# A-Kokolis/Hermes

Measured on AMD Instinct MI355X. Metric: replicated KVS ops/s (reads+writes committed), higher is better.
Workload: dtype u8

## Files before the change

### hermes_amd/csrc/hkv_batch.hip

```cpp
#include <hip/hip_runtime.h>

#include <algorithm>
#include <cstdio>
#include <cstdlib>
#include <cstring>

#include "hkv_exec.h"
#include "hkv_internal.h"

namespace hkv {

constexpr uint32_t kNone = 0xFFFFFFFFu;
enum : uint8_t { kStDone = 0, kStCommit = 1, kStPend = 2 };
enum { kCtrFbM = 1, kCtrFbL = 2 };

struct BatchArgs {
    uint8_t *elems;
    const int32_t *counts;
    const int32_t *offsets;
    const uint8_t *index;
    uint8_t *log;
    uint8_t *rw;
    int32_t *ns_idx;
    unsigned long long *fw;
// ... 14 lines not shown
    int32_t stride;
    int32_t esz;
    int32_t type;
    uint32_t rtag0;
    uint8_t ltag;
    int32_t rounds;
    int32_t inv_direct;
    int32_t ack_direct;
    uint8_t g_membership;
    uint8_t w_ack_init;
    int32_t *node_suspected;
    int32_t n_batches;
    const uint8_t *host_src;
    uint8_t *host_dst;
    uint8_t *dev_region;
    uint64_t region_bytes;
    uint32_t *done_flag;
    uint32_t done_value;
    unsigned long long *prof;
    const SmallBatch *hdr;
    uint8_t *state_out;
    const uint8_t *opc;
    const uint8_t *patch;
    uint16_t *fk;
    uint64_t *hx;
    uint8_t *rws;
    const uint8_t *rwo;
    int32_t n_rows, skip_row;
    int64_t row_stride;
    int32_t dbg;
    int32_t check_unique;
    uint8_t *ack_out;
    uint32_t ack_out_size;
};

__host__ __device__ constexpr int rounds_for(int type, bool rmw)
{
    return type == kVals || (type == kLocal && !rmw) ? 0 : 2;
}

template <int TYPE>
__device__ __forceinline__ uint8_t absorbing_state()
{
    return TYPE == kVals ? kValid : kWrite;
}

template <int TYPE>
__device__ __forceinline__ Meta after_first(const BatchArgs &a, const Meta &m0, uint32_t f, int f_is_put)
{
    Meta m1 = m0;
    m_set_state(m1, absorbing_state<TYPE>());
    if (TYPE != kLocal || a.g.skew == 0) return m1;
    uint8_t foc = f_is_put ? (uint8_t)kOpPut : a.elems[(int64_t)f * a.esz + 8];
    if (a.hx && !f_is_put) {
        const uint64_t pb = *reinterpret_cast<const uint64_t *>(a.patch + (int64_t)f * 16 + 8);
        if ((pb >> 48) & 0xFFu) foc = (uint8_t)pb;
    }
    if (foc != kOpGet) {
        m1.ver += 2;
        m_set_cid(m1, (uint8_t)a.g.machine_id);
    } else {
        m_set_state(m1, kReplay);
    }
    return m1;
}

// ... 31 lines not shown
    }
    int lo = 0, hi = a.n_batches - 1;
    while (lo < hi) {
        const int mid = (lo + hi + 1) >> 1;
        if (a.offsets[mid] <= i) lo = mid; else hi = mid - 1;
    }
    start = a.offsets[lo];
    return lo;
}

__device__ __forceinline__ void elem_at(const BatchArgs &a, uint32_t i, uint8_t *&x, uint8_t &idx, Ctx &c)
{
    c.rw = nullptr;
    c.rws = nullptr;
    idx = 0;
    if (a.rw || !a.offsets) {
        int64_t start;
        const int32_t b = batch_of(a, i, start);
        idx = (uint8_t)(i - start);
        c.rw = a.rw ? a.rw + (int64_t)b * a.rw_stride : nullptr;
        c.rws = a.rws ? a.rws + (int64_t)b * (a.rw_stride / a.g.op_size) : nullptr;
        c.rwo = a.rwo ? a.rwo + (int64_t)b * (a.rw_stride / a.g.op_size) : nullptr;
    }
    x = a.elems + (int64_t)i * a.esz;
}

__device__ __forceinline__ void note_state(const BatchArgs &a, int64_t i, const uint8_t *x)
{
    if (a.state_out) a.state_out[i] = x[9];
}

__device__ __forceinline__ uint64_t phys_of(const BatchArgs &a, uint32_t e) { return (uint64_t)e * a.g.entry_unit; }
__device__ __forceinline__ uint8_t *entry_of(const BatchArgs &a, uint32_t e) { return a.log + phys_of(a, e); }
__device__ __forceinline__ uint32_t fw_index(const BatchArgs &a, uint64_t phys)
{
    return (uint32_t)(((phys >> 6) * 0x9E3779B1ull) & a.fw_mask);
}
__device__ __forceinline__ unsigned long long *fw_of(const BatchArgs &a, uint32_t e) { return a.fw + fw_index(a, phys_of(a, e)); }

__device__ __forceinline__ uint32_t first_cand(unsigned long long f, uint32_t rtag)
{
    return (uint32_t)(f >> 32) == ~rtag ? (uint32_t)f : kNone;
}

__device__ __forceinline__ void offer(unsigned long long *f, uint32_t rtag, uint32_t i)
{
    const unsigned long long v = ((unsigned long long)(~rtag) << 32) | i;
    if (v < __hip_atomic_load(f, __ATOMIC_RELAXED, __HIP_MEMORY_SCOPE_AGENT)) atomicMin(f, v);
}

__device__ __forceinline__ uint32_t agg_ticket(uint32_t *arr, uint32_t j, bool active)
{
    const int lane = threadIdx.x & 63;
    uint32_t ticket = 0;
    unsigned long long left = __ballot(active);
    while (left) {
        const int leader = __ffsll((long long)left) - 1;
        const uint32_t jl = __shfl(j, leader, 64);
        const unsigned long long m = left & __ballot(active && j == jl);
        uint32_t base = 0;
        if (lane == leader) base = atomicAdd(&arr[jl], (uint32_t)__popcll(m));
        base = __shfl(base, leader, 64);
        if ((m >> lane) & 1ull) ticket = base + (uint32_t)__popcll(m & ((1ull << lane) - 1ull));
        left &= ~m;
    }
    return ticket;
// ... 104 lines not shown
    if (oc == kOpPut) k = kFkWrite;
    else if (oc == kOpGet) k = kFkReplay;
    else if (oc == kOpRmw && st != kInProgressRmw) k = m_state(m0) == kValid ? kFkWrite : kFkReplay;
    return (uint16_t)(k | (oc == kOpRmw ? 4u : 0u) | (((h >> 16) & 0xFFu) << 8));
}
__device__ __forceinline__ Meta after_first_rmw(const BatchArgs &a, const Meta &m0, uint16_t fk, uint8_t idx)
{
    Meta m = m0;
    if ((fk & 3u) == kFkWrite) {
        const uint8_t rmw_flag = (fk >> 2) & 1u;
        m_set_val_len(m, (uint8_t)(((uint8_t)(fk >> 8) >> a.g.shift) + kOpMetaSize));
        m_set_rmw(m, rmw_flag);
        m_set_state(m, kWrite);
        m_set_obi(m, idx);
        const uint32_t step = (!a.g.rmw_enabled || rmw_flag == 1) ? 2u : 4u;
        const uint8_t node = (uint8_t)a.g.machine_id;
        m.llw_ver = m.ver + step;
        m.llw_cid = node;
        m_set_ack_bv(m, a.w_ack_init);
        m.ver += step;
        m_set_cid(m, node);
    } else {
        m_set_state(m, kReplay);
        m_set_obi(m, idx);
        m.llw_ver = m.ver;
        m.llw_cid = m_cid(m);
        m_set_ack_bv(m, a.w_ack_init);
    }
    return m;
}

constexpr int64_t kLookupHead = 8192;
constexpr int kLookupPair = 2;
template <int P = kLookupPair>
__device__ __forceinline__ void lookup_pair(const BatchArgs &a, const uint64_t *key, const bool *probe, int q,
                                            int gbase, bool *ok, uint64_t *phys, uint4 *ln)
{
    uint4 v[P];
#pragma unroll
    for (int k = 0; k < P; ++k)
        v[k] = probe[k] ? reinterpret_cast<const uint4 *>(a.index + ((key[k] & 0xFFFFFFFFFFFFULL) & a.g.bkt_mask) * 64u)[q]
                        : make_uint4(0u, 0u, 0u, 0u);
#pragma unroll
    for (int k = 0; k < P; ++k) {
        const uint64_t s0 = (uint64_t)v[k].x | ((uint64_t)v[k].y << 32);
        const uint64_t s1 = (uint64_t)v[k].z | ((uint64_t)v[k].w << 32);
        const uint32_t tag = (uint32_t)(key[k] >> 48);
        const bool mt0 = probe[k] && (s0 & 1u) && ((uint32_t)(s0 >> 1) & 0x7FFFFFu) == tag;
        const bool mt1 = probe[k] && (s1 & 1u) && ((uint32_t)(s1 >> 1) & 0x7FFFFFu) == tag;
        const uint32_t g0 = (uint32_t)(__ballot(mt0) >> gbase) & 0xFu;
        const uint32_t g1 = (uint32_t)(__ballot(mt1) >> gbase) & 0xFu;
        uint32_t o = 0;
#pragma unroll
        for (int l = 0; l < 4; ++l) o |= ((g0 >> l) & 1u) << (2 * l) | ((g1 >> l) & 1u) << (2 * l + 1);
        const int first = o ? __ffs(o) - 1 : 0;
        const uint64_t off = __shfl((first & 1) ? (s1 >> 24) : (s0 >> 24), first >> 1, 4);
        ok[k] = probe[k] && o && a.g.log_head - off < a.g.log_cap;
        phys[k] = off & a.g.log_mask;
    }
#pragma unroll
    for (int k = 0; k < P; ++k)
        ln[k] = ok[k] ? reinterpret_cast<const uint4 *>(a.log + phys[k])[q] : make_uint4(0u, 0u, 0u, 0u);
}

template <int P>
__device__ __forceinline__ void lookup_pair_f(const BatchArgs &a, const uint64_t *key, const bool *probe, int q,
                                              int gbase, bool *ok, uint64_t *phys, uint4 *ln, unsigned long long *fwv)
{
    uint4 v[P];
#pragma unroll
    for (int k = 0; k < P; ++k)
        v[k] = probe[k] ? reinterpret_cast<const uint4 *>(a.index + ((key[k] & 0xFFFFFFFFFFFFULL) & a.g.bkt_mask) * 64u)[q]
                        : make_uint4(0u, 0u, 0u, 0u);
#pragma unroll
    for (int k = 0; k < P; ++k) {
        const uint64_t s0 = (uint64_t)v[k].x | ((uint64_t)v[k].y << 32);
        const uint64_t s1 = (uint64_t)v[k].z | ((uint64_t)v[k].w << 32);
        const uint32_t tag = (uint32_t)(key[k] >> 48);
        const bool mt0 = probe[k] && (s0 & 1u) && ((uint32_t)(s0 >> 1) & 0x7FFFFFu) == tag;
        const bool mt1 = probe[k] && (s1 & 1u) && ((uint32_t)(s1 >> 1) & 0x7FFFFFu) == tag;
        const uint32_t g0 = (uint32_t)(__ballot(mt0) >> gbase) & 0xFu;
        const uint32_t g1 = (uint32_t)(__ballot(mt1) >> gbase) & 0xFu;
        uint32_t o = 0;
#pragma unroll
        for (int l = 0; l < 4; ++l) o |= ((g0 >> l) & 1u) << (2 * l) | ((g1 >> l) & 1u) << (2 * l + 1);
        const int first = o ? __ffs(o) - 1 : 0;
        const uint64_t off = __shfl((first & 1) ? (s1 >> 24) : (s0 >> 24), first >> 1, 4);
        ok[k] = probe[k] && o && a.g.log_head - off < a.g.log_cap;
        phys[k] = off & a.g.log_mask;
    }
#pragma unroll
    for (int k = 0; k < P; ++k) {
        ln[k] = ok[k] ? reinterpret_cast<const uint4 *>(a.log + phys[k])[q] : make_uint4(0u, 0u, 0u, 0u);
        fwv[k] = ok[k] && q == 0 ? a.fw[fw_index(a, phys[k])] : ~0ull;
    }
}


template <int P = kLookupPair>
__global__ __launch_bounds__(256) void k_lookup(BatchArgs a, int64_t i_begin, int64_t i_end)
{
    const int q = threadIdx.x & 3;
    const int lane = threadIdx.x & 63;
    const int gbase = lane & ~3;
    if (i_begin == 0 && blockIdx.x == 0 && threadIdx.x == 0) {
        a.ctr[kCtrFbM] = 0;
        a.ctr[kCtrFbL] = 0;
    }
    const bool vals_direct = a.type == kVals;
    int64_t gi[P];
    uint64_t key[P], hdr[P], tail[P];
    int probe[P];
    bool patched[P];
#pragma unroll
    for (int k = 0; k < P; ++k) {
        gi[k] = i_begin + ((int64_t)blockIdx.x * P + k) * 64 + (threadIdx.x >> 2);
        uint64_t kk = 0, hh = 0;
        int p = 0;
        patched[k] = false;
        tail[k] = 0;
        if (gi[k] < i_end && q == 0) {
            const int32_t b = (int32_t)(gi[k] / a.stride);
            const int32_t idx = (int32_t)(gi[k] - (int64_t)b * a.stride);
            const bool counted = a.counts == nullptr || idx < a.counts[b];
            if (a.hx) {
                const uint8_t *x = a.elems + gi[k] * a.esz;
                const U64x2 h = *reinterpret_cast<const U64x2 *>(x);
                const U64x2 pt = *reinterpret_cast<const U64x2 *>(a.patch + gi[k] * 16);
                tail[k] = *reinterpret_cast<const uint64_t *>(x + a.esz - 8);
                patched[k] = patch_valid(pt.b);
                kk = patched[k] ? pt.a : h.a;
                hh = patched[k] ? patched_hdr(h.b, pt.b) : h.b;
            }
            if (counted) {
                if (!a.hx) {
                    const U64x2 h = *reinterpret_cast<const U64x2 *>(a.elems + gi[k] * a.esz);
                    kk = h.a;
                    hh = h.b;
                }
                if (skip_elem_os(a.type, (uint8_t)hh, (uint8_t)(hh >> 8))) {
                    if (a.type == kInvs && a.ns_idx) {
                        int64_t start;
                        const int32_t bb = a.offsets ? batch_of(a, gi[k], start) : b;
                        atomicMax(&a.ns_idx[bb], a.offsets ? (int32_t)(gi[k] - start) : idx);
                    }
                } else {
                    p = 1;
                }
            }
        }
        key[k] = kk;
        hdr[k] = hh;
        probe[k] = p;
    }
#pragma unroll
    for (int k = 0; k < P; ++k) {
        const int p = __shfl(probe[k], 0, 4);
        const uint64_t kk = __shfl(key[k], 0, 4);
        probe[k] = p;
        key[k] = kk;
    }
    bool ok[P];
    uint64_t phys[P], ekey[P];
    Meta m0[P];
    U64x2 ln[P];
    {
        bool pr[P];
        uint4 l4[P];
#pragma unroll
        for (int k = 0; k < P; ++k) pr[k] = probe[k] != 0;
        lookup_pair<P>(a, key, pr, q, gbase, ok, phys, l4);
#pragma unroll
        for (int k = 0; k < P; ++k)
            ln[k] = U64x2{(uint64_t)l4[k].x | ((uint64_t)l4[k].y << 32), (uint64_t)l4[k].z | ((uint64_t)l4[k].w << 32)};
    }
#pragma unroll
    for (int k = 0; k < P; ++k) {
        ekey[k] = __shfl(ln[k].b, 0, 4);
        const uint64_t w45 = __shfl(ln[k].a, 1, 4), w67 = __shfl(ln[k].b, 1, 4);
        const uint32_t b32 = (uint32_t)__shfl(ln[k].a, 2, 4) & 0xFFu;
        m0[k].w4 = (uint32_t)w45;
        m0[k].w5 = (uint32_t)(w45 >> 32);
        m0[k].ver = (uint32_t)w67;
        m0[k].llw_cid = (uint8_t)(w67 >> 32);
        m0[k].llw_ver = (uint32_t)(w67 >> 40) | (b32 << 24);
    }
    if (q != 0) return;
#pragma unroll
    for (int k = 0; k < P; ++k) {
        if (gi[k] >= i_end) continue;
        uint8_t *x = a.elems + gi[k] * a.esz;
        uint32_t e = kNone;
        uint8_t ifl = 0;
        if (ok[k] && ekey[k] == key[k]) {
            e = (uint32_t)(phys[k] / a.g.entry_unit);
            uint8_t *entry = a.log + phys[k];
            if (vals_direct) {
                const uint64_t its = pack_ts((uint32_t)(hdr[k] >> 32), (uint8_t)(hdr[k] >> 24));
                if (its == pack_ts(m0[k].ver, m_cid(m0[k])) && m_state(m0[k]) != kValid) entry[kEntryMetaOff] = kValid;
                x[8] = kValSuccess;
            } else if (a.ack_direct) {
                const uint64_t ats = pack_ts((uint32_t)(hdr[k] >> 32), (uint8_t)(hdr[k] >> 24));
                if (ats != pack_ts(m0[k].llw_ver, m0[k].llw_cid) || m_obi(m0[k]) == kObiEmpty) {
                    x[8] = ack_opcode((uint8_t)hdr[k]);
                } else {
                    ifl = kAkMatch;
                    const uint32_t w = fw_index(a, phys[k]);
                    const uint8_t snd = (uint8_t)(hdr[k] >> 8);
                    if (snd >= 8 || (uint8_t)(a.g_membership & ~m_ack_bv(m0[k])) == 0)
                        offer(a.fw + w, a.rtag0, (uint32_t)gi[k]);
                    if (snd < 8) {
                        unsigned long long *t = a.ft + (size_t)w * 8 + snd;
                        const unsigned long long tv = ((unsigned long long)(a.rtag0 >> 3) << 32) | (0xFFFFFFFFu - (uint32_t)gi[k]);
                        if (tv > __hip_atomic_load(t, __ATOMIC_RELAXED, __HIP_MEMORY_SCOPE_AGENT)) atomicMax(t, tv);
                    }
                    a.pf[gi[k]] = (uint32_t)m_ack_bv(m0[k]) | ((uint32_t)m_state(m0[k]) << 8) | ((uint32_t)m_obi(m0[k]) << 16);
                }
            } else if (a.inv_direct) {
                const uint64_t its = pack_ts((uint32_t)(hdr[k] >> 32), (uint8_t)(hdr[k] >> 24));
                const uint64_t cur = pack_ts(m0[k].ver, m_cid(m0[k]));
                if (its < cur) {
                    x[8] = inv_opcode((uint8_t)hdr[k], false);
                } else if (its == cur) {
                    ifl = kIvEq | (m_state(m0[k]) == kWrite ? kIvWrite : 0);
                } else {
                    ifl = kIvRaise;
                    a.pf[gi[k]] = 0;
                    const uint32_t w = fw_index(a, phys[k]);
                    const unsigned long long xv = (its << 24) | (0x7FFFFFull - (uint64_t)gi[k]);
// ... 801 lines not shown
            slot = sl;
            return true;
        }
        sl = (sl + 1) & (kPreHash - 1);
    }
    return false;
}

__device__ __forceinline__ void pre_insert_key(uint64_t *hk, uint64_t key)
{
    if (key == ~0ull) return;
    uint32_t sl = pre_slot(key);
    for (int n = 0; n < kPreHash; ++n) {
        const unsigned long long old = atomicCAS((unsigned long long *)&hk[sl], ~0ull, key);
        if (old == ~0ull || old == key) return;
        sl = (sl + 1) & (kPreHash - 1);
    }
}

#ifndef HKV_PRE_PAIR
#define HKV_PRE_PAIR 4
#endif
constexpr int kPrePair = HKV_PRE_PAIR;
#ifdef HKV_PRE_WAVES
#define HKV_PRE_ATTR __attribute__((amdgpu_waves_per_eu(HKV_PRE_WAVES)))
#else
#define HKV_PRE_ATTR
#endif
#ifdef HKV_PRE_NUM_SGPR
#define HKV_PRE_SGPR_ATTR __attribute__((amdgpu_num_sgpr(HKV_PRE_NUM_SGPR)))
#else
#define HKV_PRE_SGPR_ATTR
#endif
template <int HEAD = kPreHead>
__global__ __launch_bounds__(kPreThreads) HKV_PRE_ATTR HKV_PRE_SGPR_ATTR void k_local_pre(BatchArgs a)
{
    __shared__ uint64_t hk[kPreHash], gk[kPreHash];
    __shared__ uint32_t hv[kPreHash];
    __shared__ uint32_t dl[kPreElems];
    __shared__ uint32_t nd;
    const int tid = threadIdx.x, q = tid & 3, gbase = (tid & 63) & ~3;
    if (tid == 0) {
        nd = 0;
        if (blockIdx.x == 0) a.ctr[kCtrDefer] = 0;
    }
    for (int j = tid; j < kPreHash; j += kPreThreads) {
        hk[j] = ~0ull;
        gk[j] = ~0ull;
        hv[j] = kNone;
    }
    if (HKV_DBG_ON(a, 8)) return;
    const int64_t i0 = (int64_t)blockIdx.x * kPreElems;
    const int64_t head_end = HKV_DBG_ON(a, 4) ? 0 : i0 < HEAD ? i0 : HEAD;
    constexpr int kOwnK = kPreElems / kPreThreads, kAllK = kOwnK + (HEAD + kPreThreads - 1) / kPreThreads;
    U64x2 h[kAllK];
    bool in[kAllK];
    uint8_t opm[kAllK];
    U64x2 pt[kAllK];
#pragma unroll
    for (int k = 0; k < kAllK; ++k) {
        const bool own = k < kOwnK;
        const int64_t i = own ? i0 + k * kPreThreads + tid : (int64_t)(k - kOwnK) * kPreThreads + tid;
        in[k] = i < a.n && (own || i < head_end);
        opm[k] = a.opc ? a.opc[in[k] ? i : 0] : (uint8_t)kOpPut;
    }
    if (a.patch) {
#pragma unroll
// ... 54 lines not shown
            pre_insert_key(gk, key);
        }
    }
    __syncthreads();
    const Ctx c = make_ctx(a);
    const uint64_t hput[2] = {0, (uint64_t)kOpPut};
    const uint32_t cnt = HKV_DBG_ON(a, 2) ? 0 : nd;
    for (uint32_t base = 0; base < cnt; base += (kPreThreads / 4) * kPrePair) {
        uint64_t key[kPrePair];
        bool probe[kPrePair], ok[kPrePair];
        uint32_t idx[kPrePair];
        uint64_t phys[kPrePair];
        uint4 ln[kPrePair];
#pragma unroll
        for (int k = 0; k < kPrePair; ++k) {
            const uint32_t j = base + k * (kPreThreads / 4) + (tid >> 2);
            probe[k] = j < cnt;
            const uint32_t d = probe[k] ? dl[j] : 0u;
            idx[k] = !probe[k] ? kNone : d < (uint32_t)kPreHash ? hv[d] : ~d;
            key[k] = !probe[k] ? 0 : d < (uint32_t)kPreHash ? hk[d] : elem_key(a, (int64_t)idx[k]);
            if (probe[k] && head_end > 0 && key[k] != ~0ull) {
                uint32_t sl = pre_slot(key[k]);
                for (int n = 0; n < kPreHash; ++n) {
                    const uint64_t g = gk[sl];
                    if (g == ~0ull) break;
                    if (g == key[k]) {
                        probe[k] = false;
                        break;
                    }
                    sl = (sl + 1) & (kPreHash - 1);
                }
            }
        }
        lookup_pair<kPrePair>(a, key, probe, q, gbase, ok, phys, ln);
#pragma unroll
        for (int k = 0; k < kPrePair; ++k) {
            Meta m0;
            const uint64_t ek = line_key_meta(ln[k], m0);
            if (q != 0 || !ok[k] || ek != key[k]) continue;
            if (!would_mutate(kLocal, reinterpret_cast<const uint8_t *>(hput), m0, c) || HKV_DBG_ON(a, 1)) continue;
            atomicMin(a.fw + fw_index(a, phys[k]), ((unsigned long long)(~a.rtag0) << 32) | idx[k]);
        }
    }
}

__device__ __forceinline__ void local_resolve_nm(const BatchArgs &a, uint8_t *x, const uint8_t *ent, const Meta &m)
{
    const uint8_t oc = x[8], st = m_state(m);
    const bool obi_empty = m_obi(m) == kObiEmpty;
    bool mut = false;
    if (oc == kOpGet) {
        if (st == kValid) {
            copy_value<31>(x + kOpValueOff, ent + kEntryValueOff, 31);
            x[9] = kGetComplete;
            x[10] = (uint8_t)((m_val_len(m) >> a.g.shift) - kOpMetaSize);
        } else if (st == kInvalidWrite || st == kWrite || st == kReplay) {
            x[9] = kGetStall;
        } else {
            x[9] = kEmpty;
            if (st == kInvalid) {
                const uint8_t lw = m_lwid(m);
                if (lw < 8 && ((a.g_membership >> lw) & 1u)) x[9] = kGetStall;
                else mut = obi_empty;
            }
        }
        if (a.g.skew & kSkewReadComplete) hot_read_complete(x, m.ver, m_cid(m));
    } else if (oc == kOpPut) {
        mut = (st == kValid || st == kInvalid) && obi_empty;
        x[9] = kPutStall;
        if (a.g.skew & kSkewWriteCoalesce) {
            const uint32_t cv = m.ver & 0xFFFFu;
            uint32_t over = ld32(x + 12);
            if (st != kReplay && over == 0) {
                st32(x + 12, cv);
                over = cv;
            }
            if (over > 0 && over + 1u < cv) x[9] = kPutComplete;
        }
    }
    if (mut && a.error_flags) atomicOr(a.error_flags, 1u);
}

#ifndef HKV_LOCAL_NUM_SGPR
#define HKV_LOCAL_NUM_SGPR 80
#endif
#if HKV_LOCAL_NUM_SGPR > 0
#define HKV_LOCAL_SGPR_ATTR __attribute__((amdgpu_num_sgpr(HKV_LOCAL_NUM_SGPR)))
#else
#define HKV_LOCAL_SGPR_ATTR
#endif
#ifndef HKV_LF_WAVES
#define HKV_LF_WAVES 2
#endif
constexpr int kLfWaves = HKV_LF_WAVES;
template <int P, int NW>
__global__ __launch_bounds__(64 * NW) HKV_LOCAL_SGPR_ATTR void k_local_fused(BatchArgs a)
{
    constexpr int E = 16 * P;
    constexpr int EB = E * NW;
    __shared__ uint4 sops_b[NW][E * 4];
    __shared__ uint4 sln_b[NW][E * 4];
    __shared__ unsigned long long sfw_b[NW][E];
    __shared__ uint32_t sent_b[NW][E];
    __shared__ uint8_t sprb_b[NW][E];
    __shared__ uint32_t sst[EB / 4], sstate[EB / 4];
    __shared__ uint32_t sdef[EB];
    __shared__ uint32_t ndef;
    const int w = threadIdx.x >> 6, tid = threadIdx.x & 63, q = tid & 3, gbase = tid & ~3;
    uint4 *sops = sops_b[w], *sln = sln_b[w];
    unsigned long long *sfw = sfw_b[w];
    uint32_t *sent = sent_b[w];
    uint8_t *sprb = sprb_b[w];
    const int64_t ib = (int64_t)blockIdx.x * EB, i0 = ib + (int64_t)w * E;
    if (threadIdx.x == 0) ndef = 0;
    uint64_t key[P];
    bool probe[P], ok[P], live[P];
    uint64_t phys[P];
    uint4 ln[P], op[P];
    int te[P];
#pragma unroll
    for (int k = 0; k < P; ++k) {
        te[k] = k * 16 + (tid >> 2);
        const int64_t i = i0 + te[k];
        live[k] = i < a.n;
        op[k] = make_uint4(0u, 0u, 0u, 0u);
        if (live[k]) {
            const uint8_t *xg = a.elems + i * 56 + 16 * q;
            U64x2 p{0, 0};
            if (a.patch) p = *reinterpret_cast<const U64x2 *>(a.patch + i * 16);
            if (q < 3) {
                op[k] = *reinterpret_cast<const uint4 *>(xg);
            } else {
                const uint64_t t = *reinterpret_cast<const uint64_t *>(xg);
                op[k].x = (uint32_t)t;
                op[k].y = (uint32_t)(t >> 32);
            }
            if (patch_valid(p.b)) op[k] = patch_chunk(op[k], q, p.a, p.b);
        }
        sops[te[k] * 4 + q] = op[k];
    }
#pragma unroll
    for (int k = 0; k < P; ++k) {
        key[k] = (uint64_t)(uint32_t)__shfl((int)op[k].x, 0, 4) | ((uint64_t)(uint32_t)__shfl((int)op[k].y, 0, 4) << 32);
        const uint32_t h0 = (uint32_t)__shfl((int)op[k].z, 0, 4);
        probe[k] = false;
        if (live[k] && !HKV_DBG_ON(a, 128))
            probe[k] = in_count(a, (uint32_t)(i0 + te[k])) && !skip_elem_os(kLocal, (uint8_t)h0, (uint8_t)(h0 >> 8));
    }
    unsigned long long fwv[P];
    if (HKV_DBG_ON(a, 512)) {
        lookup_pair<P>(a, key, probe, q, gbase, ok, phys, ln);
#pragma unroll
        for (int k = 0; k < P; ++k) fwv[k] = ~0ull;
    } else {
        lookup_pair_f<P>(a, key, probe, q, gbase, ok, phys, ln, fwv);
    }
#pragma unroll
    for (int k = 0; k < P; ++k) {
        Meta m;
        const uint64_t ek = line_key_meta(ln[k], m);
        const bool hit = ok[k] && ek == key[k];
        const unsigned long long f = hit && m_state(m) != kInvalid && q == 0 ? fwv[k] : ~0ull;
        if (hit) sln[te[k] * 4 + q] = ln[k];
        if (q == 0) {
            sfw[te[k]] = f;
            sent[te[k]] = hit ? (uint32_t)(phys[k] / a.g.entry_unit) : kNone;
            sprb[te[k]] = probe[k];
        }
    }
    __syncthreads();
    if (tid < E && i0 + tid < a.n && !HKV_DBG_ON(a, 64)) {
        const int64_t i = i0 + tid;
        uint8_t *x = reinterpret_cast<uint8_t *>(&sops[tid * 4]);
        uint8_t *ent = reinterpret_cast<uint8_t *>(&sln[tid * 4]);
        const uint32_t e = sent[tid];
        uint8_t st = kStDone;
        if (e != kNone) {
            Ctx c = make_ctx(a);
            Meta m;
            meta_load(ent, m);
            const bool wm = would_mutate(kLocal, x, m, c);
            if (m_state(m) == kInvalid) {
                if (wm) {
                    const uint64_t ph = phys_of(a, e);
                    offer(a.fw + fw_index(a, ph), a.rtag0, (uint32_t)i);
                    if ((uint8_t)(m.w5 >> 16) != a.ltag) a.log[ph + kEntryMetaOff + 4] = a.ltag;
                }
                st = kStDefer;
                sdef[atomicAdd(&ndef, 1u)] = (uint32_t)i;
            } else {
                const uint32_t f = first_cand(sfw[tid], a.rtag0);
                if (wm && (f == kNone || f > (uint32_t)i) && a.error_flags) atomicOr(a.error_flags, 4u);
                if ((uint32_t)i == f) {
                    apply_to_shadow<kLocal, 31>(a, x, (uint32_t)i, ent);
                    st = kStCommit;
                } else {
                    local_resolve_nm(a, x, ent, f != kNone && (uint32_t)i > f ? after_first<kLocal>(a, m, f, 1) : m);
                }
            }
        } else if (sprb[tid]) {
            x[9] = kMiss;
        }
        if (a.opc && sprb[tid] && x[8] == kOpPut && a.opc[i] != kOpPut && a.error_flags) atomicOr(a.error_flags, 8u);
        if (!HKV_DBG_ON(a, 1024)) a.ent[i] = e;
        reinterpret_cast<uint8_t *>(sst)[w * E + tid] = st;
        reinterpret_cast<uint8_t *>(sstate)[w * E + tid] = x[9];
    }
    __syncthreads();
    if (!HKV_DBG_ON(a, 1024) && !HKV_DBG_ON(a, 64)) {
        if (ib + EB <= a.n && ((uintptr_t)a.state_out & 3) == 0) {
            if ((int)threadIdx.x < EB / 4) {
                reinterpret_cast<uint32_t *>(a.st + ib)[threadIdx.x] = sst[threadIdx.x];
                if (a.state_out) reinterpret_cast<uint32_t *>(a.state_out + ib)[threadIdx.x] = sstate[threadIdx.x];
            }
        } else if ((int)threadIdx.x < EB && ib + threadIdx.x < a.n) {
            a.st[ib + threadIdx.x] = reinterpret_cast<const uint8_t *>(sst)[threadIdx.x];
            if (a.state_out) a.state_out[ib + threadIdx.x] = reinterpret_cast<const uint8_t *>(sstate)[threadIdx.x];
        }
    }
// ... 70 lines not shown
        if (a.check_unique) {
            const unsigned long long v = ((unsigned long long)(~a.rtag0) << 32) | (uint32_t)gi[k];
            const unsigned long long old = atomicExch(a.fw + fw_index(a, phys[k]), v);
            if ((uint32_t)(old >> 32) == ~a.rtag0 && a.error_flags) atomicOr(a.error_flags, 16u);
        }
        uint8_t *entry = a.log + phys[k];
        Ctx c = make_ctx(a);
        uint8_t idx = 0;
        if (TYPE == kAcks) {
            uint8_t *xx;
            elem_at(a, (uint32_t)gi[k], xx, idx, c);
        }
        Meta t = m[k];
        dispatch<SV>(TYPE, x, entry, idx, t, c);
        if (!meta_equal(t, m[k])) meta_store(entry, t);
    }
}

__device__ __forceinline__ uint4 load_chunk(const uint8_t *x, int q, int32_t esz)
{
    if (16 * q + 16 <= esz) return *reinterpret_cast<const uint4 *>(x + 16 * q);
    if (16 * q + 8 <= esz) {
        const uint64_t t = *reinterpret_cast<const uint64_t *>(x + 16 * q);
        return make_uint4((uint32_t)t, (uint32_t)(t >> 32), 0u, 0u);
    }
    return make_uint4(0u, 0u, 0u, 0u);
}

__device__ __forceinline__ bool chunk_equal(const uint4 &a, const uint4 &b)
{
    return a.x == b.x && a.y == b.y && a.z == b.z && a.w == b.w;
}

template <int TYPE, int P = kLookupPair>
__global__ __launch_bounds__(64) void k_unique_lds(BatchArgs a)
{
    constexpr int E = 16 * P;
    __shared__ uint4 sops[E * 4];
    __shared__ uint4 sln[E * 4];
    __shared__ uint32_t sent[E];
    __shared__ uint8_t sprb[E];
    const int tid = threadIdx.x, q = tid & 3, gbase = tid & ~3;
    const int64_t i0 = (int64_t)blockIdx.x * E;
    const int64_t n_live = a.offsets ? (int64_t)a.offsets[a.n_batches] : a.n;
    uint64_t key[P];
    bool probe[P], ok[P], live[P];
    uint64_t phys[P];
    uint4 ln[P], op[P];
    int te[P];
#pragma unroll
    for (int k = 0; k < P; ++k) {
        te[k] = k * 16 + (tid >> 2);
        const int64_t i = i0 + te[k];
        live[k] = i < a.n && i < n_live;
        op[k] = live[k] ? load_chunk(a.elems + i * a.esz, q, a.esz) : make_uint4(0u, 0u, 0u, 0u);
        sops[te[k] * 4 + q] = op[k];
    }
#pragma unroll
    for (int k = 0; k < P; ++k) {
        key[k] = (uint64_t)(uint32_t)__shfl((int)op[k].x, 0, 4) | ((uint64_t)(uint32_t)__shfl((int)op[k].y, 0, 4) << 32);
        const uint32_t h0 = (uint32_t)__shfl((int)op[k].z, 0, 4);
        probe[k] = false;
        const int64_t i = i0 + te[k];
        if (live[k] && (a.offsets || in_count(a, (uint32_t)i))) {
            if (!skip_elem_os(TYPE, (uint8_t)h0, (uint8_t)(h0 >> 8))) {
                probe[k] = true;
            } else if (TYPE == kInvs && a.ns_idx && q == 0) {
                int64_t start;
                const int32_t b = batch_of(a, i, start);
                atomicMax(&a.ns_idx[b], (int32_t)(i - start));
            }
        }
    }
    lookup_pair<P>(a, key, probe, q, gbase, ok, phys, ln);
#pragma unroll
    for (int k = 0; k < P; ++k) {
        Meta m;
        const uint64_t ek = line_key_meta(ln[k], m);
        const bool hit = ok[k] && ek == key[k];
        sln[te[k] * 4 + q] = ln[k];
        if (q == 0) {
            sent[te[k]] = hit ? (uint32_t)(phys[k] / a.g.entry_unit) : kNone;
            sprb[te[k]] = probe[k];
        }
    }
    __syncthreads();
    if (tid < E && i0 + tid < n_live) {
        const int64_t i = i0 + tid;
        uint8_t *x = reinterpret_cast<uint8_t *>(&sops[tid * 4]);
        uint8_t *ent = reinterpret_cast<uint8_t *>(&sln[tid * 4]);
        const uint32_t e = sent[tid];
        if (e != kNone) {
            if (a.check_unique) {
                const unsigned long long v = ((unsigned long long)(~a.rtag0) << 32) | (uint32_t)i;
                const unsigned long long old = atomicExch(a.fw + fw_index(a, phys_of(a, e)), v);
                if ((uint32_t)(old >> 32) == ~a.rtag0 && a.error_flags) atomicOr(a.error_flags, 16u);
            }
            Ctx c = make_ctx(a);
            int done = -1;
            if (TYPE == kAcks) c.rw_done = &done;
            Meta m;
            meta_load(ent, m);
            Meta t = m;
            dispatch<31>(TYPE, x, ent, 0, t, c);
            if (!meta_equal(t, m)) meta_store(ent, t);
            if (TYPE == kAcks && done >= 0 && a.rw) {
                uint8_t *xx;
// ... 7 lines not shown
    }
    __syncthreads();
#pragma unroll
    for (int k = 0; k < P; ++k) {
        if (!live[k]) continue;
        uint4 w = sops[te[k] * 4 + q];
        if (TYPE == kInvs && a.ack_out) {
            uint8_t *y = a.ack_out + (i0 + te[k]) * a.ack_out_size;
            const uint32_t hz = sops[te[k] * 4].z;
            const uint8_t oc = (uint8_t)hz;
            const bool full = oc == kOpInvAbort && a.ack_out_size >= (uint32_t)a.esz;
            if (oc == kInvSuccess || full) {
                uint4 c = w;
                if (q == 0)
                    c.z = (hz & ~0xFFFFu) | (oc == kInvSuccess ? kOpAck : kOpInvAbort) |
                          ((uint32_t)(uint8_t)a.g.machine_id << 8);
                if (q == 0 || (full && 16 * q < a.esz)) {
                    if (16 * q + 16 <= a.esz || q == 0) *reinterpret_cast<uint4 *>(y + 16 * q) = c;
                    else *reinterpret_cast<uint64_t *>(y + 16 * q) = (uint64_t)c.x | ((uint64_t)c.y << 32);
                }
            } else if (q == 0) {
                y[8] = kEmpty;
            }
            if (q == 0 && (oc == kInvSuccess || oc == kOpInvAbort || oc == kOpMembChange))
                w.z = (w.z & ~0xFFu) | kEmpty;
        }
        if (!chunk_equal(w, op[k])) {
            uint8_t *xg = a.elems + (i0 + te[k]) * a.esz + 16 * q;
            if (16 * q + 16 <= a.esz) *reinterpret_cast<uint4 *>(xg) = w;
            else *reinterpret_cast<uint64_t *>(xg) = (uint64_t)w.x | ((uint64_t)w.y << 32);
        }
        if (ok[k] && q > 0) {
            const uint4 l = sln[te[k] * 4 + q];
            if (!chunk_equal(l, ln[k])) reinterpret_cast<uint4 *>(a.log + phys[k])[q] = l;
        }
    }
}

#ifdef HKV_ROWS_NUM_SGPR
#define HKV_ROWS_SGPR_ATTR __attribute__((amdgpu_num_sgpr(HKV_ROWS_NUM_SGPR)))
#else
#define HKV_ROWS_SGPR_ATTR
#endif
template <int TYPE, int RMAX, int CH, int P = kLookupPair>
#ifdef HKV_ROWS_WAVES
#define HKV_ROWS_WAVES_ATTR __attribute__((amdgpu_waves_per_eu(HKV_ROWS_WAVES, 8)))
#else
#define HKV_ROWS_WAVES_ATTR
#endif
__global__ __launch_bounds__(64) HKV_ROWS_SGPR_ATTR HKV_ROWS_WAVES_ATTR void k_unique_rows(BatchArgs a)
{
    constexpr int E = 16 * P;
    __shared__ uint4 sops[RMAX][E * CH];
    __shared__ uint4 sln[E * 4];
    __shared__ uint32_t sent[E];
    __shared__ uint8_t spart[E];
    const int tid = threadIdx.x, q = tid & 3, gbase = tid & ~3;
    const int64_t i0 = (int64_t)blockIdx.x * E;
    const int R = a.n_rows < RMAX ? a.n_rows : RMAX;
    const int64_t n_live = a.offsets ? (int64_t)a.offsets[a.n_batches] : a.n;
    uint64_t key[P];
    bool probe[P], ok[P], live[P];
    uint64_t phys[P];
    uint4 ln[P], op[RMAX][P];
    uint32_t part[P];
    int te[P];
#pragma unroll
    for (int k = 0; k < P; ++k) {
        te[k] = k * 16 + (tid >> 2);
        const int64_t i = i0 + te[k];
        live[k] = i < a.n && i < n_live && (a.offsets || in_count(a, (uint32_t)i));
#pragma unroll
        for (int r = 0; r < RMAX; ++r) {
            const bool on = live[k] && r < R && r != a.skip_row;
            op[r][k] = on && q < CH ? load_chunk(a.elems + (r * a.row_stride + i) * a.esz, q, a.esz)
                                    : make_uint4(0u, 0u, 0u, 0u);
            if (q < CH) sops[r][te[k] * CH + q] = op[r][k];
        }
    }
#pragma unroll
    for (int k = 0; k < P; ++k) {
        uint64_t kk = 0;
        uint32_t p = 0;
        bool mismatch = false;
#pragma unroll
        for (int r = 0; r < RMAX; ++r) {
            const uint64_t kr = (uint64_t)(uint32_t)__shfl((int)op[r][k].x, 0, 4) |
                                ((uint64_t)(uint32_t)__shfl((int)op[r][k].y, 0, 4) << 32);
            const uint32_t h0 = (uint32_t)__shfl((int)op[r][k].z, 0, 4);
            if (!live[k] || r >= R || r == a.skip_row || (uint8_t)h0 == 0) continue;
            if (skip_elem_os(TYPE, (uint8_t)h0, (uint8_t)(h0 >> 8))) continue;
            if (p && kr != kk) mismatch = true;
            if (!p) kk = kr;
            p |= 1u << r;
        }
        if (mismatch && q == 0 && a.error_flags) atomicOr(a.error_flags, 16u);
        key[k] = kk;
        part[k] = mismatch ? 0u : p;
        probe[k] = part[k] != 0;
    }
    lookup_pair<P>(a, key, probe, q, gbase, ok, phys, ln);
#pragma unroll
    for (int k = 0; k < P; ++k) {
        Meta m;
        const uint64_t ek = line_key_meta(ln[k], m);
        const bool hit = ok[k] && ek == key[k];
        sln[te[k] * 4 + q] = ln[k];
        if (q == 0) {
            sent[te[k]] = hit ? (uint32_t)(phys[k] / a.g.entry_unit) : kNone;
            spart[te[k]] = (uint8_t)part[k];
        }
    }
    __syncthreads();
    if (tid < E && i0 + tid < n_live) {
        const int64_t i = i0 + tid;
        uint8_t *ent = reinterpret_cast<uint8_t *>(&sln[tid * 4]);
        const uint32_t e = sent[tid];
        const uint32_t p = spart[tid];
        if (e != kNone && p) {
            if (a.check_unique) {
                const unsigned long long v = ((unsigned long long)(~a.rtag0) << 32) | (uint32_t)i;
                const unsigned long long old = atomicExch(a.fw + fw_index(a, phys_of(a, e)), v);
                if ((uint32_t)(old >> 32) == ~a.rtag0 && a.error_flags) atomicOr(a.error_flags, 16u);
            }
            Ctx c = make_ctx(a);
            int done = -1;
            if (TYPE == kAcks) c.rw_done = &done;
            Meta m;
            meta_load(ent, m);
            Meta t = m;
#pragma unroll
            for (int r = 0; r < RMAX; ++r)
                if ((p >> r) & 1u) dispatch<31>(TYPE, reinterpret_cast<uint8_t *>(&sops[r][tid * CH]), ent, 0, t, c);
            if (!meta_equal(t, m)) meta_store(ent, t);
// ... 3 lines not shown
                elem_at(a, (uint32_t)i, xx, idx, c);
                complete_rw_slot(c, done);
            }
        } else {
#pragma unroll
            for (int r = 0; r < RMAX; ++r)
                if ((p >> r) & 1u) reinterpret_cast<uint8_t *>(&sops[r][tid * CH])[9] = kMiss;
        }
    }
    __syncthreads();
#pragma unroll
    for (int k = 0; k < P; ++k) {
        if (!live[k]) continue;
#pragma unroll
        for (int r = 0; r < RMAX; ++r) {
            if (r >= R || r == a.skip_row || q >= CH) continue;
            uint4 w = sops[r][te[k] * CH + q];
            if (TYPE == kAcks && CH == 1 && a.ack_out) {
                const uint8_t oc = (uint8_t)w.z;
                uint4 v = make_uint4(0u, 0u, (uint32_t)kEmpty, 0u);
                if (oc != 0 && oc != kAckSuccess && oc != kOpMembChange && oc != kEmpty)
                    v = make_uint4(w.x, w.y, (w.z & ~0xFFFFu) | (uint32_t)kOpVal | ((uint32_t)(uint8_t)a.g.machine_id << 8), w.w);
                *reinterpret_cast<uint4 *>(a.ack_out + (r * a.row_stride + i0 + te[k]) * 16) = v;
                if (oc != 0 && oc != kEmpty) w.z = (w.z & ~0xFFu) | (uint32_t)kEmpty;
            }
            if (!chunk_equal(w, op[r][k])) {
                uint8_t *xg = a.elems + (r * a.row_stride + i0 + te[k]) * a.esz + 16 * q;
                if (16 * q + 16 <= a.esz) *reinterpret_cast<uint4 *>(xg) = w;
                else *reinterpret_cast<uint64_t *>(xg) = (uint64_t)w.x | ((uint64_t)w.y << 32);
            }
        }
        if (ok[k] && q > 0) {
            const uint4 l = sln[te[k] * 4 + q];
            if (!chunk_equal(l, ln[k])) reinterpret_cast<uint4 *>(a.log + phys[k])[q] = l;
        }
    }
}

constexpr int kUbElems = 16;
constexpr int kUbChunks = 20;
template <int TYPE>
__global__ __launch_bounds__(64) void k_unique_big(BatchArgs a)
{
    __shared__ uint4 sx[kUbElems * kUbChunks];
    __shared__ uint4 se[kUbElems * kUbChunks];
    constexpr int kPerLane = (kUbChunks + 3) / 4;
    uint4 x0[kPerLane], e0[kPerLane];
    const int tid = threadIdx.x, q = tid & 3, el = tid >> 2, gbase = tid & ~3;
    const int64_t i = (int64_t)blockIdx.x * kUbElems + el;
    const bool live = i < a.n;
    const int nch = (a.esz + 15) / 16;
    uint8_t *xg = a.elems + i * a.esz;
#pragma unroll
    for (int u = 0; u < kPerLane; ++u) {
        const int c = q + 4 * u;
        const uint4 v = live && c < nch ? load_chunk(xg, c, a.esz) : make_uint4(0u, 0u, 0u, 0u);
        if (c < nch) sx[el * kUbChunks + c] = v;
        x0[u] = v;
    }
    const uint4 c0 = sx[el * kUbChunks];
    const uint64_t key = (uint64_t)c0.x | ((uint64_t)c0.y << 32);
    bool probe = false;
    if (live && (a.offsets || in_count(a, (uint32_t)i))) {
        if (!skip_elem_os(TYPE, (uint8_t)c0.z, (uint8_t)(c0.z >> 8))) {
            probe = true;
        } else if (TYPE == kInvs && a.ns_idx && q == 0) {
            int64_t start;
// ... 63 lines not shown
                        w.z = (hz & ~0xFFFFu) | (oc == kInvSuccess ? kOpAck : kOpInvAbort) |
                              ((uint32_t)(uint8_t)a.g.machine_id << 8);
                    if (16 * c + 16 <= a.esz || c == 0) *reinterpret_cast<uint4 *>(y + 16 * c) = w;
                    else *reinterpret_cast<uint64_t *>(y + 16 * c) = (uint64_t)w.x | ((uint64_t)w.y << 32);
                }
            } else if (q == 0) {
                y[8] = kEmpty;
            }
        }
#pragma unroll
        for (int u = 0; u < kPerLane; ++u) {
            const int c = q + 4 * u;
            if (c >= nch) continue;
            uint4 w = sx[el * kUbChunks + c];
            if (TYPE == kInvs && a.ack_out && c == 0 && (oc == kInvSuccess || oc == kOpInvAbort || oc == kOpMembChange))
                w.z = (w.z & ~0xFFu) | kEmpty;
            if (chunk_equal(w, x0[u])) continue;
            if (16 * c + 16 <= a.esz) *reinterpret_cast<uint4 *>(xg + 16 * c) = w;
            else *reinterpret_cast<uint64_t *>(xg + 16 * c) = (uint64_t)w.x | ((uint64_t)w.y << 32);
        }
    }
    if (hit) {
        uint4 *eg = reinterpret_cast<uint4 *>(a.log + phys);
#pragma unroll
        for (int u = 0; u < kPerLane; ++u) {
            const int c = q + 4 * u;
            if (c >= kUbChunks) continue;
            const uint4 w = se[el * kUbChunks + c];
            if (c > 0 && !chunk_equal(w, e0[u])) eg[c] = w;
        }
    }
}

__global__ __launch_bounds__(256) void k_local_deferred(BatchArgs a)
{
    const uint32_t nd = a.ctr[kCtrDefer];
    for (uint32_t j = blockIdx.x * 256u + threadIdx.x; j < nd; j += gridDim.x * 256u) {
        const uint32_t i = a.fbl[j];
        const uint32_t e = a.ent[i];
        uint8_t *xg;
        uint8_t idx;
        Ctx c = make_ctx(a);
        elem_at(a, i, xg, idx, c);
        Meta m;
        meta_load(entry_of(a, e), m);
        const uint32_t f = first_cand(*fw_of(a, e), a.rtag0);
        uint8_t st = kStDone;
        if (f == kNone || i < f) {
            Meta tm = m;
            dispatch<31>(kLocal, xg, entry_of(a, e), idx, tm, c);
            if (a.error_flags && !meta_equal(tm, m)) atomicOr(a.error_flags, 1u);
        } else if (i == f) {
            apply_to_shadow<kLocal, 31>(a, nullptr, i, entry_of(a, e));
            st = kStCommit;
        } else {
            const Meta m1 = after_first<kLocal>(a, m, f, 0);
            Meta tm = m1;
            dispatch<31>(kLocal, xg, entry_of(a, e), idx, tm, c);
            if (a.error_flags && !meta_equal(tm, m1)) atomicOr(a.error_flags, 1u);
        }
        a.st[i] = st;
        note_state(a, i, xg);
    }
}

template <int TYPE, int SV>
__global__ __launch_bounds__(256) void k_resolve(BatchArgs a, int r)
{
    extern __shared__ uint64_t sx[];
    const bool kStage = SV == 31 && a.esz <= 16;
    const int64_t i = (int64_t)blockIdx.x * 256 + threadIdx.x;
    bool left = false;
    VCopy vc{nullptr, nullptr};
    VCopy *vcp = SV != 31 && a.g.st_value <= 320 ? &vc : nullptr;
    const bool wave_shadow = SV != 31 && vcp;
    bool cand = false;
    uint32_t prev = 0;
    if (i < a.n && a.st[i] == kStPend) {
        const uint32_t e = a.ent[i];
        const uint32_t f = first_cand(*fw_of(a, e), a.rtag0 + (uint32_t)r);
        prev = a.pf[i];
        if (f == kNone || (uint32_t)i <= f) {
            uint8_t *xg = a.elems + i * a.esz;
            uint8_t *xl = reinterpret_cast<uint8_t *>(sx) + threadIdx.x * (uint32_t)a.esz;
            if (kStage) copy_elem(xl, xg, a.esz);
            if ((uint32_t)i != f) {
                if (kStage) resolve_elem<TYPE, SV>(a, (uint32_t)i, xl, shadow_of(a, prev));
                else resolve_elem<TYPE, SV>(a, (uint32_t)i, xg, shadow_of(a, prev), vcp);
                a.st[i] = kStDone;
            } else {
                if (wave_shadow) cand = true;
// ... 19 lines not shown
    }
}

__device__ __forceinline__ uint32_t pow2ceil(uint32_t c) { return c <= 1 ? 1u : 1u << (32 - __clz(c - 1)); }

template <int SV>
__global__ __launch_bounds__(256) void k_commit(BatchArgs a)
{
    const int64_t i = (int64_t)blockIdx.x * 256 + threadIdx.x;
    if (SV != 31) {
        const bool mine = i < a.n && a.st[i] == kStCommit;
        const uint32_t e = mine ? a.ent[i] : 0u;
        wave_block_copies(mine ? entry_of(a, e) : nullptr, mine ? shadow_of(a, (uint32_t)i) : nullptr,
                          a.g.entry_size);
        return;
    }
    if (i >= a.n || a.st[i] != kStCommit) return;
    uint8_t *dst = entry_of(a, a.ent[i]);
    const uint8_t *src = shadow_of(a, (uint32_t)i);
    if (SV == 31) {
        const uint4 *s4 = reinterpret_cast<const uint4 *>(src);
        uint4 *d4 = reinterpret_cast<uint4 *>(dst);
        const uint4 w0 = s4[0], w1 = s4[1], w2 = s4[2], w3 = s4[3];
        d4[0] = w0;
        d4[1] = w1;
        d4[2] = w2;
        d4[3] = w3;
    } else {
        copy_entry(dst, src, a.g.entry_size);
    }
}

constexpr int kCwElems = 1024;
__global__ __launch_bounds__(256) void k_commit_w(BatchArgs a)
{
    __shared__ uint32_t lst[4][kCwElems];
    const int lane = threadIdx.x & 63, w = threadIdx.x >> 6;
    const int64_t e0 = ((int64_t)blockIdx.x * 4 + w) * kCwElems + 16 * lane;
    uint32_t m = 0;
    if (e0 + 16 <= a.n) {
        const uint4 s4 = *reinterpret_cast<const uint4 *>(a.st + e0);
        const uint32_t sw[4] = {s4.x, s4.y, s4.z, s4.w};
#pragma unroll
        for (int b = 0; b < 16; ++b)
            if (((sw[b >> 2] >> (8 * (b & 3))) & 0xFFu) == kStCommit) m |= 1u << b;
    } else {
        for (int b = 0; b < 16; ++b)
            if (e0 + b < a.n && a.st[e0 + b] == kStCommit) m |= 1u << b;
    }
    const uint32_t c = __popc(m);
    uint32_t incl = c;
#pragma unroll
    for (int d = 1; d < 64; d <<= 1) {
        const uint32_t v = (uint32_t)__shfl_up((int)incl, d, 64);
        if (lane >= d) incl += v;
    }
    const uint32_t total = (uint32_t)__shfl((int)incl, 63, 64);
    for (uint32_t pos = incl - c; m; m &= m - 1) lst[w][pos++] = (uint32_t)e0 + (uint32_t)(__ffs(m) - 1);
    __syncthreads();
    const int q = lane & 3;
    for (uint32_t j = (uint32_t)(lane >> 2); j < total; j += 16) {
        const uint32_t i = lst[w][j];
        const uint4 v = reinterpret_cast<const uint4 *>(shadow_of(a, i))[q];
        reinterpret_cast<uint4 *>(entry_of(a, a.ent[i]))[q] = v;
    }
}

constexpr int kFbThreads = 1024;
constexpr int kFbPerThread = 8;
constexpr int kFbChunk = kFbThreads * kFbPerThread;
constexpr int kFbLds = 8192;
constexpr int kFbSerial = 32;

__device__ __forceinline__ int block_min(int v, int *lds)
{
    for (int o = 32; o > 0; o >>= 1) {
        const int u = __shfl_xor(v, o, 64);
        v = u < v ? u : v;
    }
    if ((threadIdx.x & 63) == 0) lds[threadIdx.x >> 6] = v;
    __syncthreads();
    int r = lds[0];
#pragma unroll
    for (int w = 1; w < kFbThreads / 64; ++w) r = lds[w] < r ? lds[w] : r;
    return r;
}

__device__ void bitonic_sort(unsigned long long *s, uint32_t n)
{
    for (uint32_t k = 2; k <= n; k <<= 1) {
        for (uint32_t j = k >> 1; j > 0; j >>= 1) {
            for (uint32_t t = threadIdx.x; t < n; t += blockDim.x) {
                const uint32_t u = t ^ j;
                if (u > t) {
                    const unsigned long long x = s[t], y = s[u];
                    if ((x > y) == ((t & k) == 0)) {
                        s[t] = y;
// ... 914 lines not shown
    if (pl.n_batches <= 0 || pl.n_batches > kPartMaxB || pl.c.g.entry_size != 64 || pl.c.g.st_value != 31) return -1;
    static const int prof_every = getenv("HKV_PART_PROF") ? atoi(getenv("HKV_PART_PROF")) : 0;
    static unsigned long long *prof = nullptr;
    static long prof_n = 0, k = 0;
    static double sum[4] = {0, 0, 0, 0};
    HostPartLaunch p = pl;
    p.c.prof = nullptr;
    const bool sample = prof_every > 0 && (++prof_n % prof_every) == 0;
    if (sample) {
        if (!prof && hipHostMalloc((void **)&prof, 64, hipHostMallocMapped | hipHostMallocCoherent) != hipSuccess) return -3;
        p.c.prof = prof;
    }
    hipLaunchKernelGGL(k_hpart, dim3(kPartG), dim3(kHpThreads), 0, s, p);
    if (sample) {
        hipStreamSynchronize(s);
        ++k;
        for (int i = 0; i < 4; ++i) sum[i] += (double)(prof[i + 1] - prof[i]) * 10.0 / 1000.0;
        fprintf(stderr, "[hkv] k_hpart phases (us, avg of %ld): headers %.2f load+lookup %.2f rounds %.2f store %.2f\n", k,
                sum[0] / k, sum[1] / k, sum[2] / k, sum[3] / k);
    }
    return hipGetLastError() == hipSuccess ? 0 : -3;
}

__global__ void k_node_suspected(const uint8_t *elems, const int32_t *ns_idx, int32_t *out, int32_t n_batches,
                                 int32_t stride, int32_t esz, const int32_t *offsets)
{
    const int32_t b = blockIdx.x * blockDim.x + threadIdx.x;
    if (b >= n_batches) return;
    const int32_t i = ns_idx[b];
    const int64_t base = offsets ? (int64_t)offsets[b] : (int64_t)b * stride;
    if (i >= 0) out[b] = elems[(base + i) * esz + kOpValueOff];
}

static inline size_t align256(size_t x) { return (x + 255) & ~(size_t)255; }

size_t batch_scratch_bytes(int64_t cap, uint32_t entry_size)
{
    return align256(4 * (size_t)cap) * 3 + align256((size_t)cap) + align256(16 * (size_t)cap) * 2 + 256 +
           align256(2 * (size_t)cap) +
           align256((size_t)entry_size * (size_t)cap);
}

void batch_carve(BatchLaunch &bl, uint8_t *base, int64_t cap, uint32_t entry_size)
{
    uint8_t *p = base;
    auto take = [&](size_t bytes) {
        uint8_t *r = p;
        p += align256(bytes);
        return r;
    };
    bl.ent = reinterpret_cast<uint32_t *>(take(4 * (size_t)cap));
    bl.st = take((size_t)cap);
    bl.mem = reinterpret_cast<unsigned long long *>(take(16 * (size_t)cap));
    bl.fbl = reinterpret_cast<uint32_t *>(take(4 * (size_t)cap));
    bl.pf = reinterpret_cast<uint32_t *>(take(4 * (size_t)cap));
    bl.shadow = take((size_t)entry_size * (size_t)cap);
    bl.ctr = reinterpret_cast<uint32_t *>(take(256));
    bl.hx = reinterpret_cast<uint64_t *>(take(16 * (size_t)cap));
    bl.fk = reinterpret_cast<uint16_t *>(take(2 * (size_t)cap));
    bl.cap = (uint32_t)cap;
}

size_t batch_fw_words(uint64_t log_cap) { return (size_t)(log_cap >> 6); }

uint32_t batch_max_epoch() { return (1u << 29) - 1; }

int launch_batch(BatchLaunch &bl, hipStream_t s)
{
    const int64_t n = bl.n;
    if (n <= 0) return 0;
    BatchArgs a;
    a.elems = bl.elems;
    a.counts = bl.counts;
    a.offsets = bl.offsets;
    a.state_out = (bl.type == kLocal || bl.type == kLocalAfterMemb) ? bl.state_out : nullptr;
    a.opc = bl.type == kLocal ? bl.opcode_in : nullptr;
    a.patch = nullptr;
    a.hx = nullptr;
    a.fk = bl.type == kLocal && bl.g.rmw_enabled && bl.esz > 64 ? bl.fk : nullptr;
    a.ack_out = bl.type == kInvs || (bl.type == kAcks && bl.n_rows > 0) ? bl.ack_out : nullptr;
    a.ack_out_size = bl.ack_out_size;
    a.n_rows = bl.n_rows;
    a.skip_row = bl.skip_row;
    a.row_stride = bl.row_stride;
    a.rws = bl.type == kAcks ? bl.rw_state : nullptr;
    a.rwo = bl.type == kAcks ? bl.opcode_in : nullptr;
#ifdef HKV_DEBUG_MODES
    static const int dbg_env = getenv("HKV_DBG") ? atoi(getenv("HKV_DBG")) : 0;
#else
    constexpr int dbg_env = 0;
#endif
    a.dbg = dbg_env;
    static const int check_unique_env = getenv("HKV_CHECK_UNIQUE") ? atoi(getenv("HKV_CHECK_UNIQUE")) : 0;
    a.check_unique = check_unique_env;
    a.index = bl.index;
    a.log = bl.log;
    a.rw = bl.rw;
    a.ns_idx = bl.ns_idx;
    a.fw = bl.fw;
    a.fw_mask = (uint32_t)((bl.g.log_cap >> 6) - 1);
    a.ent = bl.ent;
    a.st = bl.st;
    a.mem = bl.mem;
    a.fbl = bl.fbl;
    a.pf = bl.pf;
    a.shadow = bl.shadow;
    a.ctr = bl.ctr;
    a.error_flags = bl.error_flags;
    a.g = bl.g;
    a.n = n;
    a.rw_stride = bl.rw_stride;
    a.stride = bl.stride;
    a.esz = bl.esz;
    a.type = bl.type;
    a.rtag0 = bl.epoch << 3;
    a.ltag = (uint8_t)(bl.epoch % 255u + 1u);
    a.rounds = rounds_for(bl.type, bl.g.rmw_enabled != 0);
    a.fx = bl.fx;
    a.fy = bl.fy;
    a.inv_direct = bl.type == kInvs && !bl.g.rmw_enabled && n < kInvDirectMax;
    a.ft = bl.ft;
    a.ack_direct = bl.type == kAcks && !bl.g.rmw_enabled && n < (int64_t)kNone;
    a.g_membership = bl.g_membership;
    a.w_ack_init = bl.w_ack_init;
    a.node_suspected = bl.node_suspected;
    a.n_batches = bl.n_batches;
    a.host_src = bl.host_src;
    a.host_dst = bl.host_dst;
    a.dev_region = bl.dev_region;
    a.region_bytes = bl.region_bytes;
    a.done_flag = bl.done_flag;
    a.done_value = bl.done_value;
    a.hdr = bl.hdr;
    const unsigned grid = (unsigned)((n + 255) / 256);
    const unsigned cgrid = (unsigned)((n + 256 * kCandPer - 1) / (256 * kCandPer));
    const bool big = bl.esz > 64;
    const bool big_direct = bl.type != kInvs;
    const unsigned rgrid = (unsigned)(big ? (n + 127) / 128 : grid);
    const size_t rlds = (size_t)(big ? 128 : 256) * (size_t)bl.esz;
    const bool small = (bl.path == kPathSmall || (bl.path == kPathAuto && n <= kSmallMax)) && n <= kSmallMax;
    if (bl.region_bytes && !small) return -1;
    const bool local_direct = bl.type == kLocal && !bl.g.rmw_enabled && bl.esz == 56 && bl.g.st_value == 31 &&
                              bl.g.entry_size == 64 && !bl.offsets;
    const uint32_t vend = (uint32_t)kOpValueOff + bl.g.st_value;
    const bool patch_in_resolve = bl.patch && !small && !local_direct && bl.type == kLocal && big && big_direct &&
                                  !bl.offsets && bl.g.st_value != 31 && bl.g.st_value <= 320 && bl.esz % 8 == 0 &&
                                  (uint32_t)bl.esz >= vend && (uint32_t)bl.esz <= vend + 8;
    if (patch_in_resolve) {
        a.patch = bl.patch;
        a.hx = bl.hx;
    } else if (bl.patch && (small || !local_direct)) {
        hipLaunchKernelGGL(k_apply_patch, dim3(grid), dim3(256), 0, s, bl.elems, bl.patch, n, bl.esz, bl.g.st_value);
    } else if (bl.patch) {
        a.patch = bl.patch;
    }
    if (small) {
        if (launch_small(a, s)) return -3;
        return 0;
    } else if (local_direct) {
        hipLaunchKernelGGL(k_local_pre<kPreHead>, dim3((unsigned)((n + kPreElems - 1) / kPreElems)), dim3(kPreThreads),
                           0, s, a);
        hipLaunchKernelGGL((k_local_fused<2, kLfWaves>), dim3((unsigned)((n + 32 * kLfWaves - 1) / (32 * kLfWaves))),
                           dim3(64 * kLfWaves), 0, s, a);
        hipLaunchKernelGGL(k_local_deferred, dim3(128u), dim3(256), 0, s, a);
        hipLaunchKernelGGL(k_commit_w, dim3((unsigned)((n + 4 * kCwElems - 1) / (4 * kCwElems))), dim3(256), 0, s, a);
    } else if (bl.n_rows > 0 && bl.unique) {
        const unsigned lgrid = (unsigned)((n + kLfElems - 1) / kLfElems);
        if (bl.type == kInvs) {
            if (bl.n_rows <= 2) hipLaunchKernelGGL((k_unique_rows<kInvs, 2, 4>), dim3(lgrid), dim3(64), 0, s, a);
            else hipLaunchKernelGGL((k_unique_rows<kInvs, 8, 4>), dim3(lgrid), dim3(64), 0, s, a);
        } else if (bl.esz <= 16) {
            if (bl.n_rows <= 2) hipLaunchKernelGGL((k_unique_rows<kAcks, 2, 1>), dim3(lgrid), dim3(64), 0, s, a);
            else hipLaunchKernelGGL((k_unique_rows<kAcks, 8, 1>), dim3(lgrid), dim3(64), 0, s, a);
        } else {
            if (bl.n_rows <= 2) hipLaunchKernelGGL((k_unique_rows<kAcks, 2, 4>), dim3(lgrid), dim3(64), 0, s, a);
            else hipLaunchKernelGGL((k_unique_rows<kAcks, 8, 4>), dim3(lgrid), dim3(64), 0, s, a);
        }
    } else if (bl.unique && (bl.type == kInvs || bl.type == kAcks)) {
        const unsigned ugrid1 = (unsigned)((n + 63) / 64);
#define HKV_UNIQUE(T)                                                                                  \
    do {                                                                                               \
        if (bl.g.st_value == 31) hipLaunchKernelGGL((k_unique<T, 31, 1>), dim3(ugrid1), dim3(256), 0, s, a); \
        else if (bl.g.st_value == 287) hipLaunchKernelGGL((k_unique<T, 287, 1>), dim3(ugrid1), dim3(256), 0, s, a); \
        else hipLaunchKernelGGL((k_unique<T, 0, 1>), dim3(ugrid1), dim3(256), 0, s, a);             \
    } while (0)
        const bool lds64 = bl.g.st_value == 31 && bl.g.entry_size == 64 && bl.esz <= 64;
        const bool lds_big = bl.type == kInvs && bl.g.st_value == 287 && bl.g.entry_size == 320 && bl.esz <= 320;
        if (a.ack_out && !(lds64 || lds_big)) return -1;
        if (lds64) {
            const unsigned g1 = (unsigned)((n + 15) / 16);
            if (bl.type == kInvs) hipLaunchKernelGGL((k_unique_lds<kInvs, 1>), dim3(g1), dim3(64), 0, s, a);
            else hipLaunchKernelGGL((k_unique_lds<kAcks, 1>), dim3(g1), dim3(64), 0, s, a);
        } else if (lds_big) {
            hipLaunchKernelGGL(k_unique_big<kInvs>, dim3((unsigned)((n + kUbElems - 1) / kUbElems)), dim3(64), 0, s, a);
        } else if (bl.type == kInvs) HKV_UNIQUE(kInvs);
        else HKV_UNIQUE(kAcks);
#undef HKV_UNIQUE
    } else if (bl.type == kVals) {
        hipLaunchKernelGGL(k_lookup<1>, dim3((unsigned)((n + 63) / 64)), dim3(256), 0, s, a, (int64_t)0, n);
        return hipGetLastError() == hipSuccess ? 0 : -3;
    } else {
    const bool split = bl.type == kLocal || bl.type == kLocalAfterMemb;
    const int64_t head = split && n > kLookupHead ? kLookupHead : n;
    hipLaunchKernelGGL(k_lookup<1>, dim3((unsigned)((head + 63) / 64)), dim3(256), 0, s, a, (int64_t)0, head);
    if (n > head) hipLaunchKernelGGL(k_lookup<1>, dim3((unsigned)((n - head + 63) / 64)), dim3(256), 0, s, a, head, n);
    if (a.ack_direct) {
        hipLaunchKernelGGL(k_ack_resolve, dim3(grid), dim3(256), 0, s, a);
    } else if (a.inv_direct) {
        hipLaunchKernelGGL(k_inv_resolve, dim3(grid), dim3(256), 0, s, a, (int64_t)0, n);
        if (bl.g.st_value == 31) hipLaunchKernelGGL((k_inv_commit<31>), dim3(grid), dim3(256), 0, s, a);
        else if (bl.g.st_value == 287) hipLaunchKernelGGL((k_inv_commit<287>), dim3(grid), dim3(256), 0, s, a);
        else hipLaunchKernelGGL((k_inv_commit<0>), dim3(grid), dim3(256), 0, s, a);
    } else {
#define HKV_ROUNDS(T, V)                                                                          \
    do {                                                                                          \
        if (big && rlds > 64 * 1024 &&                                                            \
            hipFuncSetAttribute((const void *)k_resolve0<T, V, 128>,                              \
                                hipFuncAttributeMaxDynamicSharedMemorySize, (int)rlds) != hipSuccess) \
            return -3;                                                                            \
        if (big && big_direct) hipLaunchKernelGGL((k_resolve0_direct<T, V>), dim3(grid), dim3(256), 0, s, a); \
        else if (big) hipLaunchKernelGGL((k_resolve0<T, V, 128>), dim3(rgrid), dim3(128), rlds, s, a); \
        else hipLaunchKernelGGL((k_resolve0<T, V, 256>), dim3(rgrid), dim3(256), rlds, s, a);     \
        for (int r = 1; r <= a.rounds; ++r) {                                                     \
            hipLaunchKernelGGL((k_cand<T>), dim3(cgrid), dim3(256), 0, s, a, r);                  \
            hipLaunchKernelGGL((k_resolve<T, V>), dim3(grid), dim3(256), V == 31 ? 256 * bl.esz : 0, s, a, r); \
        }                                                                                         \
        hipLaunchKernelGGL((k_commit<V>), dim3(grid), dim3(256), 0, s, a);                         \
        if (a.rounds > 0) hipLaunchKernelGGL((k_fb_exec<T, V>), dim3(256), dim3(kFbThreads), 0, s, a); \
    } while (0)
#define HKV_ROUNDS_SV(T)                                      \
    do {                                                      \
        if (bl.g.st_value == 31) HKV_ROUNDS(T, 31);           \
// ... 25 lines not shown
```

### hermes_amd/csrc/hkv_internal.h

```cpp
#pragma once
#include <hip/hip_runtime.h>
#include <stddef.h>
#include <stdint.h>

#include "hkv_codes.h"

struct hkv_table;

namespace hkv {

struct BatchLaunch {
    Geometry g;
    uint8_t *elems;
    const int32_t *counts;
    const int32_t *offsets;
    uint8_t *state_out;
    const uint8_t *opcode_in;
    const uint8_t *patch;
    uint8_t *rw_state;
    const uint8_t *index;
    uint8_t *log;
    uint8_t *rw;
    int64_t rw_stride;
    int32_t *ns_idx;
    int32_t *node_suspected;
    unsigned long long *fw;
    unsigned long long *fx, *fy;
    unsigned long long *ft;
    unsigned long long *mem;
    uint32_t *ent, *fbl, *pf, *ctr;
    uint64_t *hx;
    uint16_t *fk;
    uint8_t *st, *shadow;
    uint32_t cap;
    uint32_t epoch;
    unsigned int *error_flags;
    int64_t n;
    int32_t n_batches;
    int32_t stride;
    int32_t esz;
    int32_t type;
    uint8_t g_membership;
    uint8_t w_ack_init;
    int32_t path;
    int32_t unique;
    int32_t n_rows, skip_row;
    uint8_t *ack_out;
    uint32_t ack_out_size;
    int64_t row_stride;
    const uint8_t *host_src;
    uint8_t *host_dst;
    uint8_t *dev_region;
    uint64_t region_bytes;
    uint32_t *done_flag;
// ... 56 lines not shown
    const uint32_t *stop;
    uint32_t *exited;
    uint64_t idle_ticks, life_ticks;
    int32_t merge;
    uint32_t start[kPartG];
    int32_t spec;
};
int launch_host_serve(const HostServeLaunch &sl, hipStream_t s);
int launch_host_part(const HostPartLaunch &pl, hipStream_t s);

enum : int32_t { kPathAuto = 0, kPathEngine = 1, kPathSmall = 2 };

struct PopulateLaunch {
    uint64_t *first, *second;
    uint32_t *keys_a, *keys_b, *vals_a, *vals_b;
    void *sort_tmp;
    size_t sort_tmp_bytes;
    uint8_t *index;
    uint8_t *log;
    unsigned long long *evictions;
    int64_t n;
    uint64_t bkt_mask;
    uint64_t log_cap, log_mask;
    uint64_t h0, k, hw;
    uint32_t entry_size;
    int32_t key_bits;
    uint8_t val_len_byte;
};

struct TableView {
    Geometry g;
    const uint8_t *index;
    const uint8_t *log;
};
int table_view(const hkv_table *t, TableView *out);

int launch_batch(BatchLaunch &bl, hipStream_t s);
constexpr int64_t kSmallMaxElems = 4096;
int launch_populate(const PopulateLaunch &pl, hipStream_t s);
int launch_hash_ids(const uint32_t *ids, uint64_t *out, int64_t n, hipStream_t s);
size_t sort_temp_bytes(int64_t n, int key_bits);
size_t batch_scratch_bytes(int64_t cap, uint32_t entry_size);
void batch_carve(BatchLaunch &bl, uint8_t *base, int64_t cap, uint32_t entry_size);
size_t batch_fw_words(uint64_t log_cap);
uint32_t batch_max_epoch();

}
```

### hermes_amd/csrc/hkv_runtime.hip

```cpp
#include <hip/hip_runtime.h>
#include <csetjmp>
#include <csignal>

#include <cstdarg>
#include <cstdio>
#include <cstdlib>
#include <cstring>
#include <sched.h>
#include <unistd.h>
#include <algorithm>
#include <atomic>
#include <condition_variable>
#include <deque>
#include <mutex>
#include <vector>
#include <string>

#define HKV_IMPLEMENTATION 1
#include "../../include/hermeskv.h"
#include "hkv_internal.h"

using namespace hkv;

constexpr int kHostSets = 4;
// ... 38 lines not shown
{
    std::vector<std::pair<uint8_t *, bool>> gy;
    {
        std::lock_guard<std::mutex> g(g_stage_gy_mu);
        gy.swap(g_stage_graveyard);
    }
    for (auto &b : gy) (void)(b.second ? hipFree(b.first) : hipHostFree(b.first));
}
static thread_local CallerStage t_stage;

struct HostReq {
    int type;
    uint8_t *ops;
    int n;
    uint16_t esz;
    uint64_t mb;
    int *ns;
    uint8_t *rw;
    HostSet *set = nullptr;
    size_t ops_off = 0, rw_off = 0, ns_off = 0, rw_bytes = 0;
    std::atomic<bool> launched{false};
    bool part = false;
    uint32_t pseq = 0;
    uint64_t st_elems = 0, st_pos = 0, st_rw = 0, st_out = 0, st_rwo = 0;
    uint16_t poff[kPartG + 1];
};

struct hkv_table {
    hkv_config cfg;
    Geometry geo;
    hipStream_t stream = nullptr;
    uint8_t *d_index = nullptr;
    uint8_t *d_log = nullptr;
    unsigned long long *d_evictions = nullptr;
    int64_t inserted = 0;
    uint32_t skip_key = 0;
    int key_bits = 0;
    uint8_t *d_batch = nullptr;
    int64_t batch_cap = 0;
    unsigned long long *d_fw = nullptr;
    uint32_t epoch = 0;
    uint32_t scratch_gen = 0;
    struct {
        bool valid = false, done = false;
        uint32_t epoch = 0, scratch_gen = 0;
        int64_t n = 0;
        const uint8_t *elems = nullptr;
    } pre;
    unsigned int *d_error_flags = nullptr;
    int32_t *d_ns_idx = nullptr;
    int32_t ns_cap = 0;
    std::mutex hmu;
    std::condition_variable hcv;
    std::deque<HostReq *> hq;
    std::atomic<bool> combining{false};
    HostSet sets[kHostSets];
    uint32_t *pflags = nullptr, *pflags_d = nullptr;
    uint32_t pseq = 0;
    HostRingSlot *ring = nullptr, *ring_d = nullptr;
    uint32_t *srv_words = nullptr, *srv_words_d = nullptr;
    uint32_t *srv_stop = nullptr, *srv_stop_d = nullptr;
    bool ring_vram = false;
    uint32_t srv_epoch = 0;
    bool srv_running = false;
    hipEvent_t srv_ev = nullptr;
    std::mutex mu;
// ... 99 lines not shown
        HIP_TRY(hipMemset(t->d_fw, 0xFF, bytes));
        HIP_TRY(hipMemset(reinterpret_cast<uint8_t *>(t->d_fw) + bytes, 0, 10 * bytes));
        HIP_TRY(hipDeviceSynchronize());
        t->epoch = 0;
    }
    if (n <= t->batch_cap) return 0;
    const int64_t cap = n + n / 4 + 1024;
    hipFree(t->d_batch);
    t->d_batch = nullptr;
    t->batch_cap = 0;
    HIP_TRY(hipMalloc(&t->d_batch, batch_scratch_bytes(cap, t->geo.entry_size)));
    t->batch_cap = cap;
    ++t->scratch_gen;
    return 0;
}

static void plan_log(uint64_t h0, uint64_t cap, uint32_t e, uint32_t maxv, uint64_t n,
                     uint64_t &k, uint64_t &hw, uint64_t &final_head)
{
    const uint64_t T = (uint64_t)maxv + 32, mask = cap - 1;
    k = UINT64_MAX;
    hw = 0;
    if (h0 <= cap) {
        uint64_t lo = cap > T ? cap - T : 0;
        uint64_t kk = (h0 + e >= lo) ? 1 : (lo - h0 + e - 1) / e;
        if (h0 + kk * e <= cap) {
            k = kk;
            hw = (h0 + kk * e + cap) & ~mask;
        }
    }
    final_head = (n < k) ? h0 + n * e : hw + (n - k) * e;
}

namespace hkv {
int table_view(const hkv_table *t, TableView *out)
{
    if (!t || !out) return -1;
    out->g = t->geo;
    out->index = t->d_index;
    out->log = t->d_log;
    return 0;
}
}

extern "C" {

int hkv_abi_version(void) { return HKV_ABI_VERSION; }

int hkv_debug_modes(void)
{
#ifdef HKV_DEBUG_MODES
    return 1;
#else
    return 0;
#endif
}

const char *hkv_last_error(void) { return g_err.c_str(); }

int hkv_table_create(const hkv_config *cfg, hkv_table **out)
{
    if (!cfg || !out) return fail(-1, "null argument");
    if (cfg->abi_version != HKV_ABI_VERSION) return fail(-1, "abi_version %u != %d", cfg->abi_version, HKV_ABI_VERSION);
    if (!is_pow2(cfg->num_bkts) || cfg->num_bkts > (1ull << 31)) return fail(-1, "num_bkts must be a power of two <= 2^31");
    if (!is_pow2(cfg->log_cap) || cfg->log_cap < 4096) return fail(-1, "log_cap must be a power of two >= 4096");
    if (cfg->machine_id > 127) return fail(-1, "machine_id must be < 128");
    if (cfg->skew_flags & ~(HKV_SKEW_READ_COMPLETE | HKV_SKEW_WRITE_COALESCE))
        return fail(-1, "unknown skew_flags %#x", cfg->skew_flags);
    if (cfg->big_objects && (cfg->extra_cache_lines < 1 || cfg->extra_cache_lines > 16))
        return fail(-1, "extra_cache_lines must be 1..16 with big objects");
    hkv_table *t = new hkv_table();
    t->cfg = *cfg;
    if (t->cfg.rw_len == 0) t->cfg.rw_len = 250;
// ... 5 lines not shown
    }
    t->skip_key = (uint32_t)slots;
    t->key_bits = bit_width(slots);
    int rc = 0;
    do {
        if (hipSetDevice(cfg->device) != hipSuccess) { rc = fail(-5, "hipSetDevice(%d) failed", cfg->device); break; }
        if (hipStreamCreateWithFlags(&t->stream, hipStreamNonBlocking) != hipSuccess) { rc = fail(-5, "stream"); break; }
        if (hipMalloc(&t->d_index, t->cfg.num_bkts * 64) != hipSuccess) { rc = fail(-6, "index alloc %llu B", (unsigned long long)(t->cfg.num_bkts * 64)); break; }
        if (hipMalloc(&t->d_log, t->cfg.log_cap + t->geo.entry_size) != hipSuccess) { rc = fail(-6, "log alloc %llu B", (unsigned long long)t->cfg.log_cap); break; }
        if (hipMalloc(&t->d_evictions, sizeof(unsigned long long)) != hipSuccess) { rc = fail(-6, "alloc"); break; }
        if (hipMalloc(&t->d_error_flags, sizeof(unsigned int)) != hipSuccess) { rc = fail(-6, "alloc"); break; }
        if (hipMemsetAsync(t->d_error_flags, 0, sizeof(unsigned int), t->stream) != hipSuccess) { rc = fail(-5, "memset"); break; }
        if (hipMemsetAsync(t->d_index, 0, t->cfg.num_bkts * 64, t->stream) != hipSuccess) { rc = fail(-5, "memset"); break; }
        if (hipMemsetAsync(t->d_log, 0, t->cfg.log_cap + t->geo.entry_size, t->stream) != hipSuccess) { rc = fail(-5, "memset"); break; }
        if (hipMemsetAsync(t->d_evictions, 0, sizeof(unsigned long long), t->stream) != hipSuccess) { rc = fail(-5, "memset"); break; }
        if (hipStreamSynchronize(t->stream) != hipSuccess) { rc = fail(-5, "sync"); break; }
    } while (0);
    if (rc) {
        hkv_table_destroy(t);
        return rc;
    }
    (void)stage_vram_usable();
    *out = t;
    return 0;
}


int hkv_table_destroy(hkv_table *t)
{
    if (!t) return 0;
    if (t->stream) hipStreamSynchronize(t->stream);
    hipFree(t->d_index);
    hipFree(t->d_log);
    hipFree(t->d_evictions);
    hipFree(t->d_batch);
    hipFree(t->d_fw);
    hipFree(t->d_error_flags);
    hipFree(t->d_ns_idx);
    for (HostSet &hs : t->sets) {
        hipFree(hs.d);
        hipHostFree(hs.h);
        hipHostFree(hs.flag);
        if (hs.ev) hipEventDestroy(hs.ev);
    }
    if (t->srv_running) {
        srv_set_stop(t, 1u);
        hipEventSynchronize(t->srv_ev);
    }
    {
        std::lock_guard<std::mutex> lk(g_srv_mu);
        g_srv_tables.erase(std::remove(g_srv_tables.begin(), g_srv_tables.end(), t), g_srv_tables.end());
    }
    if (t->srv_ev) hipEventDestroy(t->srv_ev);
    free_stage_graveyard();
    if (t->ring) (void)(t->ring_vram ? hipFree(t->ring) : hipHostFree(t->ring));
    if (t->ring_vram && t->srv_stop) (void)hipFree(t->srv_stop);
    if (t->srv_words) hipHostFree(t->srv_words);
    if (t->pflags) hipHostFree(t->pflags);
    if (t->stream) hipStreamDestroy(t->stream);
    delete t;
    return 0;
}

int hkv_table_config(const hkv_table *t, hkv_config *out)
{
    if (!t || !out) return fail(-1, "null argument");
    *out = t->cfg;
    return 0;
}

int hkv_table_set_skew(hkv_table *t, uint32_t skew_flags)
{
    if (!t) return fail(-1, "null table");
    if (skew_flags & ~(HKV_SKEW_READ_COMPLETE | HKV_SKEW_WRITE_COALESCE)) return fail(-1, "unknown skew_flags %#x", skew_flags);
    srv_stop(t);
    std::lock_guard<std::mutex> lk(t->mu);
    t->cfg.skew_flags = skew_flags;
    t->geo.skew = skew_flags;
    return 0;
}

int hkv_table_populate(hkv_table *t, int64_t n, int val_len)
{
    if (!t) return fail(-1, "null table");
    if (n <= 0) return fail(-1, "populate: n must be > 0");
    if (val_len <= 0 || (uint32_t)val_len > t->geo.kvs_value) return fail(-1, "populate: bad val_len %d", val_len);
    srv_stop(t);
    if (n > 0x7FFFFFFFll) return fail(-1, "populate: at most 2^31-1 keys (32-bit key ids)");
    std::lock_guard<std::mutex> lk(t->mu);
    HIP_TRY(hipSetDevice(t->cfg.device));
    int bbits = bit_width(t->cfg.num_bkts - 1);
    if (bbits == 0) bbits = 1;
    uint64_t *d_first = nullptr, *d_second = nullptr;
    uint32_t *d_pairs = nullptr;
    void *d_tmp = nullptr;
    const size_t tmp_bytes = sort_temp_bytes(n, bbits);
    auto release = [&]() {
        hipFree(d_first);
        hipFree(d_second);
        hipFree(d_pairs);
        hipFree(d_tmp);
    };
    if (hipMalloc(&d_first, n * 8) != hipSuccess || hipMalloc(&d_second, n * 8) != hipSuccess ||
        hipMalloc(&d_pairs, n * 16) != hipSuccess || hipMalloc(&d_tmp, tmp_bytes) != hipSuccess) {
        release();
        return fail(-6, "populate: temporary allocation of %lld keys failed", (long long)n);
    }
    PopulateLaunch pl;
    memset(&pl, 0, sizeof pl);
    pl.first = d_first;
    pl.second = d_second;
    pl.keys_a = d_pairs;
    pl.keys_b = d_pairs + n;
    pl.vals_a = d_pairs + 2 * n;
    pl.vals_b = d_pairs + 3 * n;
    pl.sort_tmp = d_tmp;
    pl.sort_tmp_bytes = tmp_bytes;
    pl.index = t->d_index;
    pl.log = t->d_log;
    pl.evictions = t->d_evictions;
    pl.n = n;
    pl.bkt_mask = t->geo.bkt_mask;
    pl.log_cap = t->geo.log_cap;
// ... 100 lines not shown
    bl.path = (d->flags & HKV_BATCH_ENGINE) || packed ? kPathEngine
            : (d->flags & HKV_BATCH_SMALL) ? kPathSmall : kPathAuto;
    bl.unique = (d->flags & HKV_BATCH_UNIQUE) && (d->type == kInvs || d->type == kAcks) ? 1 : 0;
    if (d->d_ack_out && d->type == kAcks) {
        if (!(d->flags & HKV_BATCH_ROWS) || !bl.unique || d->elem_size != 16 || d->ack_out_size != 16 ||
            t->geo.entry_size != 64 || t->geo.st_value != 31 || ((uintptr_t)d->d_ack_out & 15))
            return fail(-1, "d_ack_out on an ACK launch: HKV_BATCH_ROWS unique launches of 16-byte ACKs and 64-byte "
                            "entries, 16-byte VALs, 16-byte aligned");
        bl.ack_out = d->d_ack_out;
        bl.ack_out_size = d->ack_out_size;
    } else if (d->d_ack_out) {
        const bool small_geo = t->geo.entry_size == 64 && t->geo.st_value == 31 && d->elem_size <= 64;
        const bool big_geo = t->geo.entry_size == 320 && t->geo.st_value == 287 && d->elem_size <= 320;
        if (d->type != kInvs || !bl.unique || d->n_rows > 1 || !(small_geo || big_geo) || d->ack_out_size < 16 ||
            (d->ack_out_size & 7) || ((uintptr_t)d->d_ack_out & 7))
            return fail(-1, "d_ack_out: unique INV launches of 64-byte entries and elements (or 320-byte big "
                            "objects), 16-byte ACKs or larger");
        bl.ack_out = d->d_ack_out;
        bl.ack_out_size = d->ack_out_size;
        bl.path = kPathEngine;
    }
    if (d->flags & HKV_BATCH_ROWS) {
        if (!bl.unique || t->geo.entry_size != 64 || t->geo.st_value != 31 || d->elem_size > 64)
            return fail(-1, "HKV_BATCH_ROWS: unique INV or ACK launches of 64-byte entries and elements only");
        if (d->n_rows < 1 || d->n_rows > HKV_MAX_ROWS || d->skip_row >= d->n_rows || d->d_node_suspected)
            return fail(-1, "HKV_BATCH_ROWS: 1..%d rows, a skip row among them (or -1), no node_suspected",
                        HKV_MAX_ROWS);
        if (d->n_rows > 1 && d->row_stride < n) return fail(-1, "HKV_BATCH_ROWS: rows overlap");
        bl.n_rows = d->n_rows;
        bl.skip_row = d->skip_row < 0 ? -1 : d->skip_row;
        bl.row_stride = d->row_stride;
        bl.path = kPathEngine;
    }
    TRACE("batch_async type=%d n=%lld", d->type, (long long)n);
    rc = launch_batch(bl, s);
    if (rc) return fail(rc, "batch launch failed (%d): %s", rc, hipGetErrorString(hipGetLastError()));
    return 0;
}

static bool srv_exited(const hkv_table *t);
static void free_stage_graveyard_if_quiet()
{
    {
        std::lock_guard<std::mutex> g(g_stage_gy_mu);
        if (g_stage_graveyard.empty()) return;
    }
    {
        std::lock_guard<std::mutex> lk(g_srv_mu);
        for (hkv_table *u : g_srv_tables)
            if (__atomic_load_n(&u->srv_running, __ATOMIC_ACQUIRE) && !srv_exited(u)) return;
    }
    free_stage_graveyard();
}

int hkv_sync(hkv_table *t, void *stream)
{
    if (!t) return fail(-1, "null table");
    srv_stop(t);
    HIP_TRY(hipStreamSynchronize((hipStream_t)stream));
    HIP_TRY(hipStreamSynchronize(t->stream));
    free_stage_graveyard_if_quiet();
    return 0;
}

int hkv_copy_index(hkv_table *t, void *dst, uint64_t off, uint64_t bytes)
{
    if (!t || !dst) return fail(-1, "null argument");
    if (off + bytes > t->cfg.num_bkts * 64) return fail(-1, "index range out of bounds");
    srv_stop(t);
    HIP_TRY(hipStreamSynchronize(t->stream));
    HIP_TRY(hipMemcpy(dst, t->d_index + off, bytes, hipMemcpyDeviceToHost));
    return 0;
}

int hkv_copy_log(hkv_table *t, void *dst, uint64_t off, uint64_t bytes)
{
    if (!t || !dst) return fail(-1, "null argument");
    if (off + bytes > t->cfg.log_cap + t->geo.entry_size) return fail(-1, "log range out of bounds");
    srv_stop(t);
    HIP_TRY(hipStreamSynchronize(t->stream));
    HIP_TRY(hipMemcpy(dst, t->d_log + off, bytes, hipMemcpyDeviceToHost));
    return 0;
}

uint64_t hkv_log_head(const hkv_table *t) { return t ? t->geo.log_head : 0; }

int64_t hkv_num_index_evictions(const hkv_table *t)
{
    if (!t) return -1;
    unsigned long long v = 0;
    if (hipMemcpy(&v, t->d_evictions, sizeof v, hipMemcpyDeviceToHost) != hipSuccess) return -1;
    return (int64_t)v;
}

void *hkv_device_index(hkv_table *t) { return t ? t->d_index : nullptr; }

int hkv_take_error_flags(hkv_table *t, uint32_t *out)
{
    if (!t || !out) return fail(-1, "null argument");
    srv_stop(t);
    HIP_TRY(hipDeviceSynchronize());
    HIP_TRY(hipMemcpy(out, t->d_error_flags, sizeof(uint32_t), hipMemcpyDeviceToHost));
    HIP_TRY(hipMemset(t->d_error_flags, 0, sizeof(uint32_t)));
    HIP_TRY(hipDeviceSynchronize());
    return 0;
}
void *hkv_device_log(hkv_table *t) { return t ? t->d_log : nullptr; }

int hkv_hash_ids(const uint32_t *d_ids, uint64_t *d_keys_second, int64_t n, void *stream)
{
    if (launch_hash_ids(d_ids, d_keys_second, n, (hipStream_t)stream)) return fail(-5, "hash launch failed");
    return 0;
}

int hkv_set_default_config(const hkv_config *cfg)
{
    std::lock_guard<std::mutex> lk(g_default_mu);
    if (g_default) return fail(-1, "default table already exists");
    g_default_cfg = *cfg;
    g_default_cfg_set = true;
    return 0;
}

hkv_table *hkv_default_table(void) { return g_default; }

[[noreturn]] static void die(const char *where)
{
    fprintf(stderr, "libhermeskv: %s: %s\n", where, g_err.c_str());
    abort();
}

static hkv_table *default_table_locked(int instance_id)
{
    if (!g_default) {
        hkv_config c = g_default_cfg_set ? g_default_cfg : reference_defaults();
        if (!g_default_cfg_set && instance_id >= 0) c.machine_id = (uint32_t)instance_id;
        if (hkv_table_create(&c, &g_default)) die("table create");
        kv.handle = g_default;
    }
    return g_default;
// ... 97 lines not shown
    size_t off = align16(sizeof(SmallBatch) * (size_t)nb);
    for (HostReq *r : take) {
        r->ops_off = off;
        off = align16(off + (size_t)r->n * r->esz);
    }
    for (HostReq *r : take) {
        r->rw_bytes = r->type == acks && r->rw ? rw_bytes : 0;
        r->rw_off = off;
        off = align16(off + r->rw_bytes);
        r->ns_off = off;
        if (r->type == invs && r->ns) off += 4;
    }
    const size_t total = align16(off);
    host_set_reserve(set, total);
    SmallBatch *hdr = reinterpret_cast<SmallBatch *>(set->h);
    for (int b = 0; b < nb; ++b) {
        HostReq *r = take[b];
        SmallBatch &h = hdr[b];
        memset(&h, 0, sizeof h);
        h.type = r->type;
        h.count = r->n;
        h.esz = r->esz;
        h.elem_off = (int32_t)r->ops_off;
        h.rw_off = r->rw_bytes ? (int32_t)r->rw_off : -1;
        h.ns_off = r->type == invs && r->ns ? (int32_t)r->ns_off : -1;
        h.g_membership = (uint8_t)(r->mb >> 8);
        h.w_ack_init = (uint8_t)(r->mb >> 16);
        memcpy(set->h + r->ops_off, r->ops, (size_t)r->n * r->esz);
        if (r->rw_bytes) memcpy(set->h + r->rw_off, r->rw, r->rw_bytes);
        if (h.ns_off >= 0) memcpy(set->h + r->ns_off, r->ns, 4);
    }
    BatchLaunch bl;
    memset(&bl, 0, sizeof bl);
    bl.g = t->geo;
    bl.index = t->d_index;
    bl.log = t->d_log;
    bl.error_flags = t->d_error_flags;
    bl.n = elems;
    bl.n_batches = nb;
    bl.stride = 1;
    bl.esz = 16;
    bl.type = take[0]->type;
    bl.g_membership = hdr[0].g_membership;
    bl.w_ack_init = hdr[0].w_ack_init;
    bl.path = kPathSmall;
    bl.host_src = set->hd;
    bl.host_dst = set->hd;
    bl.dev_region = set->d;
    bl.region_bytes = total;
    bl.done_flag = set->flag_d;
    bl.done_value = ++set->seq;
    bl.hdr = reinterpret_cast<const SmallBatch *>(set->d);
    set->mode = kModeSmall;
    if (g_host_stats) host_stats_note(nb);
    TRACE("mixed launch batches=%d elements=%lld", nb, (long long)elems);
    if (elems == 0) {
        __atomic_store_n(set->flag, bl.done_value, __ATOMIC_RELEASE);
    } else {
        std::lock_guard<std::mutex> tl(t->mu);
        bl.g = t->geo;
        if (launch_batch(bl, t->stream)) die("hermes_batch_ops_to_KVS (small launch)");
    }
    lk.lock();
    set->busy = true;
    set->refs = nb;
    for (HostReq *r : take) {
// ... 25 lines not shown

static void srv_stop(hkv_table *t)
{
    std::lock_guard<std::mutex> lk(t->hmu);
    srv_stop_locked(t);
}

static void srv_atexit()
{
    std::lock_guard<std::mutex> lk(g_srv_mu);
    for (hkv_table *t : g_srv_tables)
        if (t->srv_running) {
            srv_set_stop(t, 1u);
            (void)hipEventSynchronize(t->srv_ev);
            t->srv_running = false;
        }
    g_srv_tables.clear();
}

static void srv_ensure(hkv_table *t)
{
    if (t->srv_running && !srv_exited(t)) return;
    if (t->srv_running) {
        if (hipEventSynchronize(t->srv_ev) != hipSuccess) die("serving kernel");
        t->srv_running = false;
    }
    static const double idle_ms = getenv("HKV_SERVE_IDLE_MS") ? atof(getenv("HKV_SERVE_IDLE_MS")) : 2.0;
    HostServeLaunch sl;
    memset(&sl, 0, sizeof sl);
    {
        std::lock_guard<std::mutex> tl(t->mu);
        sl.c.g = t->geo;
    }
    sl.c.index = t->d_index;
    sl.c.log = t->d_log;
    sl.c.error_flags = t->d_error_flags;
    sl.c.flags = t->pflags_d;
    sl.ring = t->ring_d;
    sl.ring_n = kRingN;
    sl.epoch = ++t->srv_epoch;
    sl.stop = t->srv_stop_d;
    sl.exited = t->srv_words_d + 32;
    sl.idle_ticks = (uint64_t)(idle_ms * 1e5);
    sl.life_ticks = (uint64_t)1e8;
    static const int merge = getenv("HKV_SERVE_MERGE") ? std::max(1, atoi(getenv("HKV_SERVE_MERGE"))) : kServeMerge;
    sl.merge = std::min(merge, kRingN / 2);
    sl.spec = 1;
    for (int g = 0; g < kPartG; ++g) sl.start[g] = __atomic_load_n(t->pflags + g, __ATOMIC_ACQUIRE) + 1;
    srv_set_stop(t, 0u);
    if (!t->srv_ev && hipEventCreateWithFlags(&t->srv_ev, hipEventDisableTiming) != hipSuccess) die("event");
    if (launch_host_serve(sl, t->stream) || hipEventRecord(t->srv_ev, t->stream) != hipSuccess) die("serving kernel launch");
    t->srv_running = true;
    {
        static std::once_flag once;
        std::call_once(once, [] { atexit(srv_atexit); });
        std::lock_guard<std::mutex> lk(g_srv_mu);
        if (std::find(g_srv_tables.begin(), g_srv_tables.end(), t) == g_srv_tables.end()) g_srv_tables.push_back(t);
    }
    TRACE("serving kernel epoch %u", sl.epoch);
}

static uint32_t part_done(const hkv_table *t)
{
    uint32_t m = __atomic_load_n(t->pflags, __ATOMIC_ACQUIRE);
    for (int g = 1; g < kPartG; ++g) {
        const uint32_t v = __atomic_load_n(t->pflags + g, __ATOMIC_ACQUIRE);
// ... 56 lines not shown
    memset(&pl, 0, sizeof pl);
    std::vector<HostReq *> take;
    int tot[kPartG] = {0};
    for (auto it = t->hq.begin(); it != t->hq.end() && (int)take.size() < kPartMaxB;) {
        HostReq *r = *it;
        bool fits = r->part;
        for (int g = 0; fits && g < kPartG; ++g) fits = tot[g] + (r->poff[g + 1] - r->poff[g]) <= kPartCap;
        if (!fits) {
            ++it;
            continue;
        }
        for (int g = 0; g < kPartG; ++g) tot[g] += r->poff[g + 1] - r->poff[g];
        take.push_back(r);
        it = t->hq.erase(it);
    }
    const uint32_t seq = ++t->pseq;
    lk.unlock();
    const int nb = (int)take.size();
    for (int b = 0; b < nb; ++b) {
        const HostReq *r = take[b];
        HostPartHdr &h = pl.hdr[b];
        h.elems = r->st_elems;
        h.pos = r->st_pos;
        h.out = r->st_out;
        h.rw = r->st_rw;
        h.rwo = r->st_rwo;
        h.type = r->type;
        h.count = r->n;
        h.esz = r->esz;
        h.g_membership = (uint8_t)(r->mb >> 8);
        h.w_ack_init = (uint8_t)(r->mb >> 16);
        for (int g = 0; g <= kPartG; ++g) pl.part[g][b] = r->poff[g];
    }
    pl.c.index = t->d_index;
    pl.c.log = t->d_log;
    pl.c.error_flags = t->d_error_flags;
    pl.n_batches = nb;
    pl.c.flags = t->pflags_d;
    pl.seq = seq;
    if (g_host_stats) host_stats_note(nb);
    TRACE("partitioned launch %u batches=%d", seq, nb);
    const long c2 = g_host_timing ? now_ns() : 0;
    if (serve) {
        HostRingSlot &slot = t->ring[seq % kRingN];
        slot.n_batches = nb;
        memcpy(slot.hdr, pl.hdr, sizeof(HostPartHdr) * (size_t)nb);
        memcpy(slot.part, pl.part, sizeof slot.part);
        __builtin_ia32_sfence();
        __atomic_store_n(&slot.seq, seq, __ATOMIC_RELEASE);
        __builtin_ia32_sfence();
        lk.lock();
        srv_ensure(t);
    } else {
        {
            std::lock_guard<std::mutex> tl(t->mu);
            pl.c.g = t->geo;
            if (launch_host_part(pl, t->stream)) {
                die("hermes_batch_ops_to_KVS (partitioned launch)");
            }
        }
        lk.lock();
    }
    if (g_host_timing) {
        const long c3 = now_ns();
        g_hc_n += 1;
        g_hc_inflight += c1 - c0;
// ... 365 lines not shown
```

### hermes_amd/csrc/hkv_workload.hip

```cpp
#include <hip/hip_runtime.h>

#include "../../include/hermeskv.h"
#include "../../include/hermeskv_workload.h"
#include "hkv_codes.h"
#include "hkv_internal.h"

namespace hkv {

__device__ __forceinline__ uint64_t splitmix64(uint64_t x)
{
    x += 0x9e3779b97f4a7c15ULL;
    x = (x ^ (x >> 30)) * 0xbf58476d1ce4e5b9ULL;
    x = (x ^ (x >> 27)) * 0x94d049bb133111ebULL;
    return x ^ (x >> 31);
}

__device__ __forceinline__ double unit_double(uint64_t r) { return (double)(r >> 11) * (1.0 / 9007199254740992.0); }

__device__ __forceinline__ uint64_t zipf_draw(const hkv_zipf &z, double u)
{
    if (z.theta <= 0.0) {
        uint64_t id = (uint64_t)(u * (double)z.n);
        return id < z.n ? id : z.n - 1;
    }
// ... 1175 lines not shown
            const int64_t g = (int64_t)w * row + (int64_t)r * per_peer + j;
            bool keep = false;
            uint32_t id = 0;
            if (j < per_peer) {
                id = ids[g];
                const uint32_t h = dedup_slot(hk, (((uint64_t)r << 32) | id) + 1, mask, false);
                keep = h != 0xFFFFFFFFu && hmin[h] == (uint32_t)w * (uint32_t)per_peer + (uint32_t)j;
            }
            int total;
            const int rank = block_rank(keep, total);
            if (keep) {
                const int64_t o = (int64_t)w * row + base + cnt + rank;
                const uint64_t key = key_of_id(id);
                const uint8_t f = rmw[g];
                const uint64_t h1 = (uint64_t)kOpInv | ((uint64_t)peer << 8) | ((uint64_t)(st_value >> shift) << 16) |
                                    ((uint64_t)peer << 24);
                uint64_t *x = reinterpret_cast<uint64_t *>(invs + o * op_size);
                x[0] = key;
                x[1] = h1;
                const uint64_t vv = 0x0101010101010101ULL * (uint8_t)('a' + peer);
                x[2] = (vv << 16) | f;
                for (uint32_t k = 3; k < op_size / 8; ++k) x[k] = vv;
                uint64_t *v = reinterpret_cast<uint64_t *>(vals + o * kOpMetaSize);
                v[0] = key;
                v[1] = (h1 & ~0xFFull) | kOpVal;
            }
            cnt += total;
        }
        if (threadIdx.x == 0) peer_counts[(int64_t)w * n_peers + r] = cnt;
        base += cnt;
    }
}

__device__ __forceinline__ uint64_t find_entry(const TableView &t, uint64_t key)
{
    const uint64_t *b = reinterpret_cast<const uint64_t *>(t.index + ((key & 0xFFFFFFFFFFFFULL) & t.g.bkt_mask) * 64u);
    const uint32_t tag = (uint32_t)(key >> 48);
    for (int s = 0; s < 8; ++s) {
        const uint64_t slot = b[s];
        if ((slot & 1u) && ((uint32_t)(slot >> 1) & 0x7FFFFFu) == tag) {
            const uint64_t off = slot >> 24;
            if (t.g.log_head - off >= t.g.log_cap) return ~0ull;
            const uint64_t phys = off & t.g.log_mask;
            return *reinterpret_cast<const uint64_t *>(t.log + phys + 8) == key ? phys : ~0ull;
        }
    }
    return ~0ull;
}

__device__ __forceinline__ uint64_t peer_slot(const TableView &t, uint64_t phys) { return phys / t.g.entry_size; }

__device__ __forceinline__ uint32_t peer_round_tag(uint32_t round) { return (round + 1u) & 0x7FFFFFu; }

struct __attribute__((aligned(8))) U64x2w {
    uint64_t a, b;
};
constexpr int kPeerTsPair = 2;
__global__ __launch_bounds__(256) void k_peer_ts(TableView t, uint8_t *invs, uint8_t *vals, const int32_t *counts,
                                                 int32_t stride, uint32_t op_size, unsigned long long *peer_ts,
                                                 uint32_t round, int64_t total)
{
    const int q = threadIdx.x & 3;
    const int gbase = (threadIdx.x & 63) & ~3;
    int64_t g[kPeerTsPair];
    int live[kPeerTsPair];
    uint64_t key[kPeerTsPair], flags[kPeerTsPair];
#pragma unroll
    for (int k = 0; k < kPeerTsPair; ++k) {
        g[k] = ((int64_t)blockIdx.x * kPeerTsPair + k) * 64 + (threadIdx.x >> 2);
        live[k] = 0;
        key[k] = flags[k] = 0;
        if (g[k] < total && q == 0) {
            const int32_t w = (int32_t)(g[k] / stride);
            if ((int32_t)(g[k] - (int64_t)w * stride) < counts[w]) {
                live[k] = 1;
                const uint8_t *x = invs + g[k] * op_size;
                key[k] = *reinterpret_cast<const uint64_t *>(x);
                flags[k] = *reinterpret_cast<const uint64_t *>(x + 8) >> 8 & 0xFFu;
                flags[k] |= (uint64_t)(x[16] & 1u) << 8;
            }
// ... 226 lines not shown
        uint8_t *x = aq + ((int64_t)w * q_stride + j) * ack_size;
        const uint8_t oc = j < applied ? x[8] : 0;
        const bool send = j < applied && val_sends(oc);
        int cnt;
        const int rank = block_rank(send, cnt);
        if (send && total + rank < kMaxVq) {
            const W16 h = *reinterpret_cast<const W16 *>(x);
            buf[total + rank] = W16{h.a, (h.b & ~0xFFFFull) | kOpVal | ((uint64_t)(machine_id & 0xFF) << 8)};
        } else if (send && overflow) {
            atomicAdd(overflow, 1ull);
        }
        if (j < applied && oc != kEmpty) x[8] = kEmpty;
        total = min(total + cnt, kMaxVq);
    }
    __syncthreads();
    const int send = min(total, min(v_credits, out_stride));
    W16 *orow = reinterpret_cast<W16 *>(out + (int64_t)w * out_stride * kOpMetaSize);
    for (int j = threadIdx.x; j < send; j += 256) orow[j] = buf[j];
    const int keep = min(total - send, vq_stride);
    for (int j = threadIdx.x; j < keep; j += 256) vrow[j] = buf[send + j];
    if (threadIdx.x == 0) {
        out_count[w] = send;
        vq_n[w] = keep;
        if (applied) aq_n[w] = 0;
        if (total - send > keep && overflow) atomicAdd(overflow, (unsigned long long)(total - send - keep));
    }
}

__global__ __launch_bounds__(256) void k_peer_locate(TableView t, const uint8_t *invs, uint32_t op_size,
                                                     int64_t total, uint64_t *phys_out)
{
    const int64_t g = (int64_t)blockIdx.x * 256 + threadIdx.x;
    if (g >= total) return;
    phys_out[g] = find_entry(t, *reinterpret_cast<const uint64_t *>(invs + g * op_size));
}

struct PeerTsArgs {
    TableView t;
    uint8_t *invs, *vals;
    const uint64_t *phys_in;
    int64_t total;
    uint32_t op_size;
    unsigned long long *peer_ts;
    uint32_t round;
};
__device__ __forceinline__ void peer_ts_at_body(const PeerTsArgs &pt, int bx)
{
    const TableView &t = pt.t;
    uint8_t *invs = pt.invs, *vals = pt.vals;
    const uint64_t *phys_in = pt.phys_in;
    const int64_t total = pt.total;
    const uint32_t op_size = pt.op_size, round = pt.round;
    unsigned long long *peer_ts = pt.peer_ts;
    const int64_t g = (int64_t)bx * 256 + threadIdx.x;
    if (g >= total) return;
    uint8_t *x = invs + g * op_size;
    uint8_t *vv = vals + g * kOpMetaSize;
    const uint64_t key = *reinterpret_cast<const uint64_t *>(x);
    const uint64_t h8 = *reinterpret_cast<const uint64_t *>(x + 8);
    const uint64_t vh = *reinterpret_cast<const uint64_t *>(vv + 8);
    const uint8_t peer = (uint8_t)(h8 >> 8);
    const bool rmw = x[16] & 1u;
    uint64_t phys = phys_in[g];
    uint32_t cur = 0;
    bool ok = false;
    if (phys != ~0ull) {
        const U64x2w *e = reinterpret_cast<const U64x2w *>(t.log + phys);
        const U64x2w l0 = e[0], l1 = e[1];
        if (l0.b == key) {
            ok = true;
            cur = (uint32_t)l1.b;
        }
    }
    if (!ok) {
        phys = find_entry(t, key);
        if (phys != ~0ull) {
            ok = true;
            cur = *reinterpret_cast<const uint32_t *>(t.log + phys + 24);
        }
    }
    uint32_t ver = 2;
    if (ok) {
        ver = cur + ((!t.g.rmw_enabled || rmw) ? 2u : 4u);
        if (peer_ts && peer < 8)
            atomicMax(peer_ts + peer_slot(t, phys) * 8 + peer,
                      ((unsigned long long)peer_round_tag(round) << 41) | ((unsigned long long)rmw << 40) |
                          ((unsigned long long)ver << 8) | peer);
    }
    const uint64_t nh = (h8 & 0xFFFFFF00ull & 0xFFFFFFFFull) | kOpInv | ((uint64_t)ver << 32);
    *reinterpret_cast<uint64_t *>(x + 8) = nh;
    *reinterpret_cast<uint64_t *>(vv + 8) = (vh & 0xFFFFFF00ull & 0xFFFFFFFFull) | kOpVal | ((uint64_t)ver << 32);
}

__global__ __launch_bounds__(256) void k_peer_ts_at(PeerTsArgs pt) { peer_ts_at_body(pt, blockIdx.x); }

__global__ __launch_bounds__(256) HKV_PLAN_SGPR_ATTR void k_plan_peer_ts(PlanArgs pa, PeerTsArgs pt, int plan_blocks)
{
    if ((int)blockIdx.x < plan_blocks) refill_plan_body<2>(pa, blockIdx.x);
    else peer_ts_at_body(pt, (int)blockIdx.x - plan_blocks);
}

}

using namespace hkv;

static inline unsigned blocks_for(int64_t n) { return (unsigned)((n + 255) / 256); }
static inline int ok() { return hipGetLastError() == hipSuccess ? 0 : -5; }

extern "C" {

int hkv_wl_gen_trace(uint64_t *tkey, uint8_t *top, uint32_t *tid, int32_t n_workers, int32_t len, const hkv_zipf *z,
                     uint32_t write_pm, uint32_t rmw_pm, uint64_t seed, void *stream)
{
    int64_t n = (int64_t)n_workers * len;
    if (n <= 0) return 0;
    hipLaunchKernelGGL(k_gen_trace, dim3(blocks_for(n)), dim3(256), 0, (hipStream_t)stream, tkey, top, tid, n_workers,
                       len, *z, write_pm, rmw_pm, seed);
    return ok();
}

int hkv_wl_refill(uint8_t *ops, int32_t n_workers, int32_t stride, uint32_t op_size, uint32_t st_value, uint32_t shift,
                  const uint64_t *tkey, const uint8_t *top, const uint32_t *tid, int32_t tlen, uint32_t *cursor,
                  uint32_t machine_id, int32_t first_iter, uint32_t flags, unsigned long long *counters,
                  uint8_t *opc_out, uint8_t *hot, void *stream)
{
    if (stride > 256 || n_workers <= 0 || op_size % 8 || tlen <= 0) return -1;
    if (flags & ~(uint32_t)(HKV_WL_REFILL_ALL | HKV_WL_READ_TS_RESET | HKV_WL_COALESCE_HOT)) return -1;
    const size_t lds = (size_t)stride * op_size;
    if (flags & HKV_WL_COALESCE_HOT) {
        if (!tid || !hot || stride > 255 || lds > 56 * 1024) return -1;
        hipLaunchKernelGGL(k_refill_hot, dim3(n_workers), dim3(256), lds, (hipStream_t)stream, ops, stride, op_size,
                           st_value, shift, tkey, top, tid, tlen, cursor, machine_id, first_iter, flags, counters,
// ... 58 lines not shown
{
    if (stride > 256 || n_workers <= 0) return -1;
    hipLaunchKernelGGL(k_marshal_invs, dim3(n_workers), dim3(256), 0, (hipStream_t)stream, ops, stride, op_size, out,
                       stride, count, machine_id, (unsigned long long *)nullptr, (const int32_t *)nullptr, 1,
                       (uint8_t *)nullptr);
    return ok();
}

int hkv_wl_marshal_acks(uint8_t *invs, int64_t n, uint32_t op_size, uint8_t *out, uint32_t ack_size,
                        uint32_t machine_id, void *stream)
{
    if (n <= 0) return 0;
    hipLaunchKernelGGL(k_marshal_acks, dim3(blocks_for(n)), dim3(256), 0, (hipStream_t)stream, invs, n, op_size, out,
                       ack_size, machine_id);
    return ok();
}

int hkv_wl_marshal_vals(uint8_t *acks, int64_t n, uint32_t ack_size, uint8_t *out, uint32_t machine_id, void *stream)
{
    if (n <= 0) return 0;
    hipLaunchKernelGGL(k_marshal_vals, dim3(blocks_for(n)), dim3(256), 0, (hipStream_t)stream, acks, n, ack_size, out,
                       machine_id);
    return ok();
}

int hkv_wl_peer_acks_pm(hkv_table *t, const uint8_t *inv_out, const int32_t *inv_count, int32_t n_workers,
                        int32_t inv_stride, uint32_t op_size, uint8_t *acks, uint32_t ack_size, int32_t max_invs,
                        int32_t *ack_count, const uint8_t *peer_ids, int32_t n_peers,
                        const unsigned long long *peer_ts, uint32_t round, const int32_t *inv_off, void *stream)
{
    if (n_peers <= 0 || n_workers <= 0 || ack_size < kOpMetaSize || ack_size % 8 || !inv_off) return -1;
    if (max_invs <= 0 || max_invs > inv_stride) return -1;
    TableView tv{};
    if (peer_ts && table_view(t, &tv)) return -1;
    const int32_t out_stride = max_invs * n_peers;
    int64_t total = (int64_t)n_workers * out_stride;
    hipLaunchKernelGGL(k_peer_acks, dim3(blocks_for(total)), dim3(256), 0, (hipStream_t)stream, inv_out, inv_count,
                       inv_stride, op_size, acks, ack_size, out_stride, ack_count, peer_ids, n_peers, total, tv,
                       peer_ts, round, inv_off, n_workers);
    return ok();
}

int hkv_wl_peer_acks(hkv_table *t, const uint8_t *inv_out, const int32_t *inv_count, int32_t n_workers,
                     int32_t inv_stride, uint32_t op_size, uint8_t *acks, uint32_t ack_size, int32_t out_stride,
                     int32_t *ack_count, const uint8_t *peer_ids, int32_t n_peers,
                     const unsigned long long *peer_ts, uint32_t round, const int32_t *out_off, void *stream)
{
    if (n_peers <= 0 || n_workers <= 0 || ack_size < kOpMetaSize || ack_size % 8) return -1;
    if (out_stride % n_peers || out_stride > inv_stride * n_peers || out_stride <= 0) return -1;
    TableView tv{};
    if (peer_ts && table_view(t, &tv)) return -1;
    int64_t total = (int64_t)n_workers * out_stride;
    hipLaunchKernelGGL(k_peer_acks, dim3(blocks_for(total)), dim3(256), 0, (hipStream_t)stream, inv_out, inv_count,
                       inv_stride, op_size, acks, ack_size, out_stride, ack_count, peer_ids, n_peers, total, tv,
                       peer_ts, round, out_off, 0);
    return ok();
}

static size_t peer_slots(int64_t total)
{
    size_t s = 1024;
    while (s < 2 * (size_t)total) s <<= 1;
    return s;
}

static size_t align_up(size_t x) { return (x + 255) & ~(size_t)255; }

size_t hkv_wl_peer_round_scratch(int32_t n_workers, int32_t per_peer, int32_t n_peers)
{
    const int64_t total = (int64_t)n_workers * per_peer * n_peers;
    const size_t slots = peer_slots(total);
    return align_up(8 * slots) + align_up(4 * slots) + align_up(4 * (size_t)total) + align_up((size_t)total);
}

int hkv_wl_gen_peer_round(uint8_t *invs, uint8_t *vals, int32_t *peer_counts, int32_t n_workers, int32_t per_peer,
                          const uint8_t *peer_ids, int32_t n_peers, uint32_t op_size, uint32_t st_value,
                          uint32_t shift, const hkv_zipf *z, uint32_t rmw_pm, uint32_t round, uint64_t seed,
                          void *scratch, void *stream)
{
    const int64_t total = (int64_t)n_workers * per_peer * n_peers;
    if (total <= 0) return 0;
    if (op_size % 8 || op_size < kOpValueOff + st_value || total > 0x7FFFFFFFll) return -1;
    hipStream_t s = (hipStream_t)stream;
    const size_t slots = peer_slots(total);
    uint8_t *p = static_cast<uint8_t *>(scratch);
    unsigned long long *hk = reinterpret_cast<unsigned long long *>(p);
    p += align_up(8 * slots);
    uint32_t *hmin = reinterpret_cast<uint32_t *>(p);
    p += align_up(4 * slots);
    uint32_t *ids = reinterpret_cast<uint32_t *>(p);
    p += align_up(4 * (size_t)total);
    uint8_t *rmw = p;
    if (hipMemsetAsync(hk, 0, 8 * slots, s) != hipSuccess || hipMemsetAsync(hmin, 0xFF, 4 * slots, s) != hipSuccess)
        return -5;
    hipLaunchKernelGGL(k_peer_draw, dim3(blocks_for(total)), dim3(256), 0, s, ids, rmw, hk, hmin,
                       (uint32_t)(slots - 1), per_peer, n_peers, *z, rmw_pm, round, seed, total);
    hipLaunchKernelGGL(k_peer_compact, dim3(n_workers), dim3(256), 0, s, ids, rmw, hk, hmin, (uint32_t)(slots - 1), invs,
                       vals, peer_counts, per_peer, peer_ids, n_peers, op_size, st_value, shift);
    return ok();
}

int hkv_wl_peer_ts(hkv_table *t, uint8_t *invs, uint8_t *vals, const int32_t *counts, int32_t n_workers,
                   int32_t stride, uint32_t op_size, unsigned long long *peer_ts, uint32_t round, void *stream)
{
    TableView tv;
    if (table_view(t, &tv) || n_workers <= 0 || stride <= 0 || op_size % 8) return -1;
    const int64_t total = (int64_t)n_workers * stride;
    const int64_t per_block = 64 * kPeerTsPair;
    hipLaunchKernelGGL(k_peer_ts, dim3((unsigned)((total + per_block - 1) / per_block)), dim3(256), 0,
                       (hipStream_t)stream, tv, invs, vals, counts, stride, op_size, peer_ts, round, total);
    return ok();
}

uint64_t hkv_wl_peer_ts_words(const hkv_table *t)
{
    TableView tv;
    if (table_view(t, &tv)) return 0;
    return (tv.g.log_cap / tv.g.entry_size + 1) * 8;
}

int hkv_wl_marshal_invs_cap(uint8_t *ops, int32_t n_workers, int32_t stride, uint32_t op_size, uint8_t *out,
                            int32_t out_stride, int32_t *count, uint32_t machine_id, unsigned long long *held,
                            uint8_t *states, void *stream)
{
    if (stride > 256 || n_workers <= 0 || out_stride <= 0 || op_size % 8) return -1;
    const bool mwave = marshal_wave();
    if (op_size <= 64)
        if (wl_wpw() == 2 && mwave)
            hipLaunchKernelGGL((k_marshal_invs_w<2, true>), dim3((unsigned)((n_workers + 7) / 8)), dim3(256), 0,
                               (hipStream_t)stream, ops, n_workers, stride, op_size, out, out_stride, count, machine_id,
                               held, (const int32_t *)nullptr, 1, states);
        else if (wl_wpw() == 2)
            hipLaunchKernelGGL(k_marshal_invs_w<2>, dim3((unsigned)((n_workers + 7) / 8)), dim3(256), 0, (hipStream_t)stream,
                               ops, n_workers, stride, op_size, out, out_stride, count, machine_id, held,
                               (const int32_t *)nullptr, 1, states);
        else
            hipLaunchKernelGGL(k_marshal_invs_w<1>, dim3((unsigned)((n_workers + 3) / 4)), dim3(256), 0, (hipStream_t)stream,
                               ops, n_workers, stride, op_size, out, out_stride, count, machine_id, held,
                               (const int32_t *)nullptr, 1, states);
    else
        hipLaunchKernelGGL(k_marshal_invs, dim3(n_workers), dim3(256), 0, (hipStream_t)stream, ops, stride, op_size,
                           out, out_stride, count, machine_id, held, (const int32_t *)nullptr, 1, states);
    return ok();
}

int hkv_wl_marshal_invs_credits(uint8_t *ops, int32_t n_workers, int32_t stride, uint32_t op_size, uint8_t *out,
                                int32_t out_stride, int32_t *count, uint32_t machine_id, unsigned long long *held,
                                const int32_t *aq_n, int32_t r_alive, void *stream)
{
    if (stride > 256 || n_workers <= 0 || out_stride <= 0 || op_size % 8) return -1;
// ... 114 lines not shown
int hkv_wl_marshal_acks_aligned(uint8_t *invs, const int32_t *counts, int32_t rows, int32_t width, uint32_t op_size,
                                uint8_t *out, uint32_t ack_size, uint32_t machine_id, void *stream)
{
    const int64_t n = (int64_t)rows * width;
    if (n <= 0) return 0;
    if (op_size % 8 || ack_size % 8) return -1;
    hipLaunchKernelGGL(k_marshal_acks_aligned, dim3(blocks_for(n)), dim3(256), 0, (hipStream_t)stream, invs, counts,
                       width, n, op_size, out, ack_size, machine_id);
    return ok();
}

int hkv_wl_regroup_aligned(const uint8_t *in, int32_t n_peers, int32_t width, const int32_t *offsets,
                           const int32_t *counts, int32_t n_workers, uint32_t elem_size, uint8_t *out,
                           int32_t out_stride, int32_t *out_count, void *stream)
{
    if (n_workers <= 0) return 0;
    if (n_peers <= 0 || width <= 0 || elem_size % 8) return -1;
    hipLaunchKernelGGL(k_regroup_aligned, dim3(n_workers), dim3(256), 0, (hipStream_t)stream, in, n_peers, width,
                       offsets, counts, elem_size, out, out_stride, out_count);
    return ok();
}

}

extern "C" {

int hkv_wl_peer_acks_queue(hkv_table *t, const uint8_t *inv_out, const int32_t *inv_count, int32_t n_workers,
                           int32_t inv_stride, uint32_t op_size, uint8_t *aq, uint32_t ack_size, int32_t q_stride,
                           int32_t *aq_n, const int32_t *vq_n, int32_t *acnt, const uint8_t *peer_ids, int32_t n_peers,
                           const unsigned long long *peer_ts, uint32_t round, void *stream)
{
    if (n_peers <= 0 || n_workers <= 0 || ack_size < kOpMetaSize || ack_size % 8 || q_stride <= 0) return -1;
    TableView tv{};
    if (peer_ts && table_view(t, &tv)) return -1;
    hipLaunchKernelGGL(k_peer_acks_q, dim3(n_workers), dim3(256), 0, (hipStream_t)stream, inv_out, inv_count, inv_stride,
                       op_size, aq, ack_size, q_stride, aq_n, vq_n, acnt, peer_ids, n_peers, tv, peer_ts, round);
    return ok();
}

int hkv_wl_vals_credit(uint8_t *aq, int32_t *aq_n, const int32_t *acnt, int32_t n_workers, int32_t q_stride,
                       uint32_t ack_size, uint8_t *vq, int32_t *vq_n, int32_t vq_stride, uint8_t *out,
                       int32_t *out_count, int32_t out_stride, int32_t v_credits, uint32_t machine_id,
                       unsigned long long *overflow, void *stream)
{
    if (n_workers <= 0 || ack_size % 8 || vq_stride <= 0 || out_stride <= 0 || v_credits < 0) return -1;
    hipLaunchKernelGGL(k_vals_credit, dim3(n_workers), dim3(256), 0, (hipStream_t)stream, aq, aq_n, acnt, q_stride,
                       ack_size, vq, vq_n, vq_stride, out, out_count, out_stride, v_credits, machine_id, overflow);
    return ok();
}

}

extern "C" {

int hkv_wl_peer_locate(hkv_table *t, const uint8_t *invs, int64_t n, uint32_t op_size, uint64_t *phys_out, void *stream)
{
    TableView tv;
    if (table_view(t, &tv) || n < 0 || op_size % 8) return -1;
    if (n == 0) return 0;
    hipLaunchKernelGGL(k_peer_locate, dim3(blocks_for(n)), dim3(256), 0, (hipStream_t)stream, tv, invs, op_size, n,
                       phys_out);
    return ok();
}

int hkv_wl_peer_ts_at(hkv_table *t, uint8_t *invs, uint8_t *vals, const uint64_t *phys, int64_t n, uint32_t op_size,
                      unsigned long long *peer_ts, uint32_t round, void *stream)
{
    TableView tv;
    if (table_view(t, &tv) || n < 0 || op_size % 8) return -1;
    if (n == 0) return 0;
    const PeerTsArgs pt{tv, invs, vals, phys, n, op_size, peer_ts, round};
    hipLaunchKernelGGL(k_peer_ts_at, dim3(blocks_for(n)), dim3(256), 0, (hipStream_t)stream, pt);
    return ok();
}

int hkv_wl_refill_plan_peer_ts(uint8_t *states, int32_t n_workers, int32_t stride, uint32_t st_value, uint32_t shift,
                               const uint64_t *tkey, const uint8_t *top, int32_t tlen, uint32_t *cursor,
                               uint32_t machine_id, uint32_t flags, unsigned long long *counters, uint8_t *opc,
                               uint8_t *patch, hkv_table *t, uint8_t *invs, uint8_t *vals, const uint64_t *phys, int64_t n,
                               uint32_t op_size, unsigned long long *peer_ts, uint32_t round, void *stream)
{
    if (stride > 256 || n_workers <= 0 || tlen <= 0 || !states || !opc || !patch) return -1;
    if (flags & ~(uint32_t)(HKV_WL_REFILL_ALL | HKV_WL_READ_TS_RESET)) return -1;
    if (((uintptr_t)patch & 15) || (st_value >> shift) > 255) return -1;
    TableView tv;
    if (table_view(t, &tv) || n < 0 || op_size % 8) return -1;
    const PlanArgs pa{states, n_workers, stride, st_value, shift, tkey, top, tlen, cursor, machine_id, flags, counters, opc,
                      patch};
    const PeerTsArgs pt{tv, invs, vals, phys, n, op_size, peer_ts, round};
    const int plan_blocks = (n_workers + 7) / 8;
#ifdef HKV_PLAN_PTS_SPLIT
    hipLaunchKernelGGL(k_refill_plan_w<2>, dim3((unsigned)plan_blocks), dim3(256), 0, (hipStream_t)stream, pa);
    if (n) hipLaunchKernelGGL(k_peer_ts_at, dim3(blocks_for(n)), dim3(256), 0, (hipStream_t)stream, pt);
#else
    hipLaunchKernelGGL(k_plan_peer_ts, dim3((unsigned)plan_blocks + blocks_for(n)), dim3(256), 0, (hipStream_t)stream, pa,
                       pt, plan_blocks);
#endif
    return ok();
}

}
```

### hermes_amd/kvs.py

```python
from __future__ import annotations

import ctypes

import numpy as np
import torch

from . import layout as L
from .lib import ABI_VERSION, HkvBatchDesc, HkvConfig, Membership, check, raw

_L = raw()


def _membership_struct(mb: bytes) -> Membership:
    return Membership(int.from_bytes(bytes(mb[:8]).ljust(8, b"\0"), "little"))


def set_default_config(**kw) -> None:
    cfg = make_config(**kw)
    check(_L.hkv_set_default_config(ctypes.byref(cfg)), "hkv_set_default_config")


def spacetime_init(instance_id: int) -> None:
    _L.spacetime_init(int(instance_id))


def spacetime_populate_fixed_len(n: int, val_len: int) -> None:
    _L.spacetime_populate_fixed_len(None, int(n), int(val_len))


def hermes_batch_ops_to_KVS(btype: int, op_array: np.ndarray, op_num: int, sizeof_op_elem: int,
                            curr_membership: bytes, node_suspected: list | None,
                            read_write_ops: np.ndarray | None, thread_id: int = 0) -> None:
    assert op_array.flags["C_CONTIGUOUS"]
    ns = ctypes.c_int(node_suspected[0] if node_suspected else -1)
    _L.hermes_batch_ops_to_KVS(int(btype), op_array.ctypes.data_as(ctypes.c_void_p), int(op_num),
                               int(sizeof_op_elem), _membership_struct(curr_membership),
                               ctypes.byref(ns) if node_suspected is not None else None,
                               read_write_ops.ctypes.data_as(ctypes.c_void_p) if read_write_ops is not None else None,
                               int(thread_id))
    if node_suspected is not None:
        node_suspected[0] = ns.value


def make_config(num_keys: int = 1_000_000, num_bkts: int = 2 * 1024 * 1024, log_cap: int = 1 << 30,
                machine_id: int = 0, rmw: bool = False, big_objects: bool = False,
                extra_cache_lines: int = 0, device: int = 0, rw_len: int = 250, skew: int = 0) -> HkvConfig:
    return HkvConfig(ABI_VERSION, machine_id, int(rmw), int(big_objects), int(extra_cache_lines), device, rw_len,
                     int(skew), num_keys, num_bkts, log_cap)


SKEW_READ_COMPLETE = 1
SKEW_WRITE_COALESCE = 2


def sized_geometry(num_keys: int, sizes: L.Sizes = L.DEFAULT) -> tuple[int, int]:
    bkts = 1 << max(4, (2 * num_keys - 1).bit_length())
    need = num_keys * sizes.entry + sizes.kvs_value + 64
    cap = 1 << max(16, (need - 1).bit_length())
    return min(bkts, 1 << (27 if num_keys <= 1 << 28 else 29)), cap


BATCH_ENGINE = 1
BATCH_SMALL = 2
BATCH_PACKED = 4
BATCH_UNIQUE = 8
BATCH_ROWS = 16


class HermesKV:

    default_flags = 0

    def __init__(self, num_keys: int | None = 1_000_000, num_bkts: int | None = None,
                 log_cap: int | None = None, machine_id: int = 0, rmw: bool = False,
                 big_objects: bool = False, extra_cache_lines: int = 0, device: int = 0,
                 rw_len: int = 250, populate: bool = True, skew: int = 0):
        self.sizes = L.Sizes(big_objects, extra_cache_lines if big_objects else 0)
        nk = num_keys or 0
        if num_bkts is None or log_cap is None:
            b, c = sized_geometry(max(nk, 1), self.sizes)
            num_bkts = num_bkts or b
            log_cap = log_cap or c
        self.cfg = make_config(nk, num_bkts, log_cap, machine_id, rmw, big_objects,
                               extra_cache_lines, device, rw_len, skew)
        self.skew = int(skew)
        self.device = device
        self.machine_id = machine_id
        self.rmw = rmw
        self.num_keys = nk
        h = ctypes.c_void_p()
        check(_L.hkv_table_create(ctypes.byref(self.cfg), ctypes.byref(h)), "hkv_table_create")
        self.h = h
        self._owned = True
# ... 163 lines not shown
        nbytes = self.cfg.num_bkts * 64 - offset if nbytes is None else nbytes
        out = np.empty(nbytes, dtype=np.uint8)
        check(_L.hkv_copy_index(self.h, out.ctypes.data_as(ctypes.c_void_p), offset, nbytes), "hkv_copy_index")
        return out

    def log_bytes(self, offset: int = 0, nbytes: int | None = None) -> np.ndarray:
        nbytes = self.cfg.log_cap - offset if nbytes is None else nbytes
        out = np.empty(nbytes, dtype=np.uint8)
        check(_L.hkv_copy_log(self.h, out.ctypes.data_as(ctypes.c_void_p), offset, nbytes), "hkv_copy_log")
        return out

    def lookup_offset(self, key: int) -> int | None:
        key = int(key)
        bkt = (key & 0xFFFFFFFFFFFF) & (self.cfg.num_bkts - 1)
        slots = self.index_bytes(bkt * 64, 64).view("<u8")
        tag = key >> 48
        for s in slots:
            s = int(s)
            if (s & 1) and ((s >> 1) & 0x7FFFFF) == tag:
                off = s >> 24
                if self.log_head - off >= self.cfg.log_cap:
                    return None
                phys = off & (self.cfg.log_cap - 1)
                e = self.log_bytes(phys, 16).view("<u8")
                return phys if int(e[1]) == key else None
        return None

    def entry(self, key: int):
        off = self.lookup_offset(key)
        if off is None:
            return None
        return self.log_bytes(off, self.sizes.entry).view(L.entry_dtype(self.sizes))[0]

    def device_index(self) -> int:
        return _L.hkv_device_index(self.h)

    def device_log(self) -> int:
        return _L.hkv_device_log(self.h)


def hash_ids(ids: torch.Tensor, stream: torch.cuda.Stream | None = None) -> torch.Tensor:
    assert ids.is_cuda and ids.dtype == torch.int32
    out = torch.empty(ids.numel(), dtype=torch.int64, device=ids.device)
    s = (stream or torch.cuda.current_stream(ids.device)).cuda_stream
    check(_L.hkv_hash_ids(ctypes.c_void_p(ids.data_ptr()), ctypes.c_void_p(out.data_ptr()), ids.numel(),
                          ctypes.c_void_p(s)), "hkv_hash_ids")
    return out
```

### hermes_amd/lib.py

```python
from __future__ import annotations

import ctypes
import os

import torch

HERE = os.path.dirname(os.path.abspath(__file__))
LIB_PATH = os.environ.get("HKV_LIB") or os.path.join(HERE, "libhermeskv.so")
ABI_VERSION = 8

if not os.path.exists(LIB_PATH):
    raise ImportError(f"{LIB_PATH} is missing: run __graft_entry__.build() (hipcc --offload-arch=gfx950)")

_L = ctypes.CDLL(LIB_PATH, mode=ctypes.RTLD_GLOBAL)


class HkvConfig(ctypes.Structure):
    _fields_ = [("abi_version", ctypes.c_uint32), ("machine_id", ctypes.c_uint32),
                ("rmw_enabled", ctypes.c_uint32), ("big_objects", ctypes.c_uint32),
                ("extra_cache_lines", ctypes.c_uint32), ("device", ctypes.c_int32),
                ("rw_len", ctypes.c_uint32), ("skew_flags", ctypes.c_uint32),
                ("num_keys", ctypes.c_uint64), ("num_bkts", ctypes.c_uint64),
                ("log_cap", ctypes.c_uint64)]


class HkvBatchDesc(ctypes.Structure):
    _fields_ = [("type", ctypes.c_int32), ("n_batches", ctypes.c_int32), ("stride", ctypes.c_int32),
                ("elem_size", ctypes.c_uint16), ("flags", ctypes.c_uint16),
                ("d_elems", ctypes.c_void_p), ("d_counts", ctypes.c_void_p), ("d_rw", ctypes.c_void_p),
                ("rw_stride_bytes", ctypes.c_int64), ("d_node_suspected", ctypes.c_void_p),
                ("membership", ctypes.c_uint8 * 8), ("d_state_out", ctypes.c_void_p),
                ("d_opcode_in", ctypes.c_void_p), ("d_patch", ctypes.c_void_p), ("d_rw_state", ctypes.c_void_p),
                ("d_put_keys", ctypes.c_void_p), ("n_rows", ctypes.c_int32), ("skip_row", ctypes.c_int32),
                ("row_stride", ctypes.c_int64), ("d_ack_out", ctypes.c_void_p), ("ack_out_size", ctypes.c_uint32),
                ("d_phys", ctypes.c_void_p)]


class Membership(ctypes.Structure):
    _fields_ = [("bits", ctypes.c_uint64)]


_P = ctypes.c_void_p
_L.hkv_abi_version.restype = ctypes.c_int
_L.hkv_debug_modes.restype = ctypes.c_int
_L.hkv_last_error.restype = ctypes.c_char_p
_L.hkv_table_create.argtypes = [ctypes.POINTER(HkvConfig), ctypes.POINTER(_P)]
_L.hkv_table_destroy.argtypes = [_P]
_L.hkv_table_populate.argtypes = [_P, ctypes.c_int64, ctypes.c_int]
_L.hkv_table_config.argtypes = [_P, ctypes.POINTER(HkvConfig)]
_L.hkv_table_set_skew.argtypes = [_P, ctypes.c_uint32]
_L.hkv_batch_async.argtypes = [_P, ctypes.POINTER(HkvBatchDesc), _P]
_L.hkv_sync.argtypes = [_P, _P]
_L.hkv_copy_index.argtypes = [_P, _P, ctypes.c_uint64, ctypes.c_uint64]
_L.hkv_copy_log.argtypes = [_P, _P, ctypes.c_uint64, ctypes.c_uint64]
_L.hkv_log_head.restype = ctypes.c_uint64
_L.hkv_log_head.argtypes = [_P]
_L.hkv_num_index_evictions.restype = ctypes.c_int64
_L.hkv_num_index_evictions.argtypes = [_P]
_L.hkv_device_index.restype = _P
_L.hkv_device_index.argtypes = [_P]
_L.hkv_take_error_flags.argtypes = [_P, ctypes.POINTER(ctypes.c_uint32)]
_L.hkv_device_log.restype = _P
_L.hkv_device_log.argtypes = [_P]
_L.hkv_set_default_config.argtypes = [ctypes.POINTER(HkvConfig)]
_L.hkv_default_table.restype = _P
_L.hkv_hash_ids.argtypes = [_P, _P, ctypes.c_int64, _P]
_L.spacetime_init.argtypes = [ctypes.c_int]
_L.spacetime_populate_fixed_len.argtypes = [_P, ctypes.c_int, ctypes.c_int]
_L.hermes_batch_ops_to_KVS.argtypes = [ctypes.c_int, _P, ctypes.c_int, ctypes.c_uint16, Membership,
                                       ctypes.POINTER(ctypes.c_int), _P, ctypes.c_uint8]

if _L.hkv_abi_version() != ABI_VERSION:
    raise ImportError(f"libhermeskv ABI {_L.hkv_abi_version()} != {ABI_VERSION}")


class HkvError(RuntimeError):
    pass


def check(rc: int, what: str) -> None:
    if rc != 0:
        raise HkvError(f"{what}: rc={rc}: {_L.hkv_last_error().decode(errors='replace')}")


def raw() -> ctypes.CDLL:
    return _L


def loaded_path() -> str:
    return LIB_PATH
```

### hermes_amd/workload.py

```python
from __future__ import annotations

import ctypes
import math

import numpy as np
import torch

from . import layout as L
from .kvs import HermesKV
from .lib import check, raw

_L = raw()
_P = ctypes.c_void_p


class HkvZipf(ctypes.Structure):
    _fields_ = [("theta", ctypes.c_double), ("zetan", ctypes.c_double), ("alpha", ctypes.c_double),
                ("eta", ctypes.c_double), ("half_pow", ctypes.c_double), ("n", ctypes.c_uint64)]


_L.hkv_wl_gen_trace.argtypes = [_P, _P, _P, ctypes.c_int32, ctypes.c_int32, ctypes.POINTER(HkvZipf),
                                ctypes.c_uint32, ctypes.c_uint32, ctypes.c_uint64, _P]
_L.hkv_wl_refill.argtypes = [_P, ctypes.c_int32, ctypes.c_int32, ctypes.c_uint32, ctypes.c_uint32, ctypes.c_uint32,
                             _P, _P, _P, ctypes.c_int32, _P, ctypes.c_uint32, ctypes.c_int32, ctypes.c_uint32, _P, _P,
                             _P, _P]
_L.hkv_wl_fold_counters.argtypes = [_P, _P]
_L.hkv_wl_refill_st.argtypes = [_P, ctypes.c_int32, ctypes.c_int32, ctypes.c_uint32, ctypes.c_uint32, ctypes.c_uint32,
                                _P, _P, ctypes.c_int32, _P, ctypes.c_uint32, ctypes.c_uint32, _P, _P, _P, _P]
_L.hkv_wl_refill_plan.argtypes = [_P, ctypes.c_int32, ctypes.c_int32, ctypes.c_uint32, ctypes.c_uint32, _P, _P,
                                  ctypes.c_int32, _P, ctypes.c_uint32, ctypes.c_uint32, _P, _P, _P, _P]
_L.hkv_wl_marshal_invs.argtypes = [_P, ctypes.c_int32, ctypes.c_int32, ctypes.c_uint32, _P, _P, ctypes.c_uint32, _P]
_L.hkv_wl_marshal_invs_cap.argtypes = [_P, ctypes.c_int32, ctypes.c_int32, ctypes.c_uint32, _P, ctypes.c_int32, _P,
                                       ctypes.c_uint32, _P, _P, _P]
_L.hkv_wl_marshal_acks.argtypes = [_P, ctypes.c_int64, ctypes.c_uint32, _P, ctypes.c_uint32, ctypes.c_uint32, _P]
_L.hkv_wl_marshal_memb_vals.argtypes = [_P, ctypes.c_int32, ctypes.c_int32, ctypes.c_uint32, _P, ctypes.c_int32, _P,
                                        ctypes.c_uint32, _P, _P]
_L.hkv_wl_max_to_host.argtypes = [_P, ctypes.c_int32, _P, _P]
_L.hkv_wl_marshal_vals.argtypes = [_P, ctypes.c_int64, ctypes.c_uint32, _P, ctypes.c_uint32, _P]
_L.hkv_wl_collect_vals.argtypes = [_P, _P, ctypes.c_int32, ctypes.c_int32, ctypes.c_uint32, _P, ctypes.c_int32,
                                   _P, ctypes.c_uint32, _P, _P, _P]
_L.hkv_wl_peer_acks_pm.argtypes = [_P, _P, _P, ctypes.c_int32, ctypes.c_int32, ctypes.c_uint32, _P, ctypes.c_uint32,
                                   ctypes.c_int32, _P, _P, ctypes.c_int32, _P, ctypes.c_uint32, _P, _P]
# ... 216 lines not shown
        self.ack_count = torch.zeros(W, dtype=torch.int32, device=dev)
        self.val_out = torch.zeros(W * self.ack_stride * L.OP_META_SIZE, **u8)
        self.val_count = torch.zeros(W, dtype=torch.int32, device=dev)
        self.rstride = self.rpp * max(self.R, 1)
        self.ack_out = torch.zeros(W * self.rstride * self.ack_size, **u8)
        self.cursor = torch.zeros(W, dtype=torch.int32, device=dev)
        self.counters = torch.zeros(4096, dtype=torch.int64, device=dev)
        self.inv_total = torch.zeros(1, dtype=torch.int64, device=dev)
        self.elem_totals = torch.zeros(3, dtype=torch.int64, device=dev)
        self.count_elems = True
        self.peer_t = torch.tensor(self.peers or [0], dtype=torch.uint8, device=dev)
        self.trace_len = trace_len
        self.seed = seed
        self.trace_key = torch.empty(W * trace_len, dtype=torch.int64, device=dev)
        self.trace_op = torch.empty(W * trace_len, dtype=torch.uint8, device=dev)
        self.trace_id = torch.empty(W * trace_len, dtype=torch.int32, device=dev) if coalesce_hot else None
        self.hot = torch.full((W * 2 * HOT_KEYS,), 0xFF, dtype=torch.uint8, device=dev) if coalesce_hot else None
        check(_L.hkv_wl_gen_trace(_ptr(self.trace_key), _ptr(self.trace_op), _ptr(self.trace_id), W, trace_len,
                                  ctypes.byref(zipf), write_permille, rmw_permille,
                                  ctypes.c_uint64(seed ^ (self.machine_id << 48)), _s()), "gen_trace")
        self.clock = 0
        self.max_steps = max_steps
        self.rmw_pm = rmw_permille
        self.remote_inv = []
        self.remote_val = []
        self.remote_counts = []
        self.peer_ts = None
        if virtual_peers and self.R and kvs.rmw:
            self.peer_ts = torch.zeros(int(_L.hkv_wl_peer_ts_words(kvs.h)), dtype=torch.int64, device=dev)
        self.pack_remote = virtual_peers and self.R > 0 and pack_remote
        self.remote_packed = []
        self.fused_acks = (self.pack_remote and ((kvs.sizes.entry == 64 and self.op <= 64) or
                                                 (kvs.sizes.entry == 320 and self.op <= 320)))
        self.drops = []
        self.alive = self.R
        self._counts = {}
        self.hades = None
        if hades:
            self._hades_start()
        self._gen_remote()
        self.audit: CommitAudit | None = None
        self._pts_done = None
        self.refill(first=True)

    def _gen_remote(self):
        if not (self.virtual and self.R):
            return
        W, R, dev = self.W, self.R, torch.device("cuda", self.kvs.device)
        u8 = dict(dtype=torch.uint8, device=dev)
        scratch = torch.empty(int(_L.hkv_wl_peer_round_scratch(W, self.rpp, R)), **u8)
        pc = torch.empty(W * R, dtype=torch.int32, device=dev)
        for k in range(self.max_steps):
            ri = torch.zeros(W * self.rstride * self.op, **u8)
            rv = torch.zeros(W * self.rstride * L.OP_META_SIZE, **u8)
            check(_L.hkv_wl_gen_peer_round(_ptr(ri), _ptr(rv), _ptr(pc), W, self.rpp, _ptr(self.peer_t), R, self.op,
                                           self.sizes.st_value, self.sizes.shift, ctypes.byref(self.zipf),
                                           self.rmw_pm, k, ctypes.c_uint64(self.seed * 7919 + self.machine_id),
                                           _ptr(scratch), _s()), "gen_peer_round")
            cum = torch.cumsum(pc.view(W, R), dim=1, dtype=torch.int32)
            self.remote_counts.append([None] + [cum[:, n - 1].contiguous() for n in range(1, R + 1)])
            self.remote_inv.append(ri)
            self.remote_val.append(rv)
            if self.pack_remote:
                pcw = pc.view(W, R).long()
                start = torch.cumsum(pcw, dim=1) - pcw
                cnt = pcw.t().reshape(-1)
# ... 364 lines not shown
```

### include/hermeskv.h

```cpp
#ifndef HERMESKV_H
#define HERMESKV_H

#include <stddef.h>
#include <stdint.h>

#ifdef __cplusplus
extern "C" {
#endif

#define HKV_ABI_VERSION 8

#ifndef HERMES_SPACETIME_H
enum hermes_batch_type_t {
    local_ops,
    local_ops_after_membership_change,
    invs,
    acks,
    vals
};
typedef struct { uint8_t bit_array[1]; } bit_vector_t;
typedef struct { uint8_t lock; uint32_t version; } __attribute__((packed)) seqlock_t;
typedef struct {
    volatile uint8_t num_of_alive_remotes;
    volatile bit_vector_t g_membership;
    volatile bit_vector_t w_ack_init;
    seqlock_t lock;
} spacetime_group_membership;
typedef struct hkv_spacetime_op spacetime_op_t;
struct spacetime_kv;
#endif


#ifndef HKV_IMPLEMENTATION
void hermes_batch_ops_to_KVS(enum hermes_batch_type_t type, uint8_t *op_array, int op_num,
                             uint16_t sizeof_op_elem, spacetime_group_membership curr_membership,
                             int *node_suspected, spacetime_op_t *read_write_ops, uint8_t thread_id);
#endif

void spacetime_init(int instance_id);

void spacetime_populate_fixed_len(struct spacetime_kv *kv, int n, int val_len);


// ... 41 lines not shown
    const uint64_t *d_phys;
} hkv_batch_desc;

#define HKV_PATCH_BYTES 16

#define HKV_BATCH_ENGINE 1u
#define HKV_BATCH_SMALL  2u
#define HKV_BATCH_PACKED 4u
#define HKV_BATCH_UNIQUE 8u
#define HKV_BATCH_ROWS 16u
#define HKV_BATCH_RESERVED_FLAGS 0xE0u
#define HKV_MAX_ROWS 8
int  hkv_abi_version(void);
int  hkv_debug_modes(void);
const char *hkv_last_error(void);

int  hkv_table_create(const hkv_config *cfg, hkv_table **out);
int  hkv_table_destroy(hkv_table *t);
int  hkv_table_populate(hkv_table *t, int64_t n, int val_len);
int  hkv_table_config(const hkv_table *t, hkv_config *out);
int  hkv_table_set_skew(hkv_table *t, uint32_t skew_flags);

int  hkv_batch_async(hkv_table *t, const hkv_batch_desc *desc, void *stream);
int  hkv_sync(hkv_table *t, void *stream);

int  hkv_copy_index(hkv_table *t, void *host_dst, uint64_t offset, uint64_t bytes);
int  hkv_copy_log(hkv_table *t, void *host_dst, uint64_t offset, uint64_t bytes);
uint64_t hkv_log_head(const hkv_table *t);
int64_t  hkv_num_index_evictions(const hkv_table *t);
void *hkv_device_index(hkv_table *t);
int  hkv_take_error_flags(hkv_table *t, uint32_t *out);
void *hkv_device_log(hkv_table *t);

int  hkv_set_default_config(const hkv_config *cfg);
hkv_table *hkv_default_table(void);

int  hkv_debug_host_hold(int n_batches);
int  hkv_debug_host_queued(void);

int  hkv_hash_ids(const uint32_t *d_ids, uint64_t *d_keys_second, int64_t n, void *stream);

#ifdef __cplusplus
}
#endif
#endif
```

Baseline: 4.532 billion.

## Add inline bucket-line layout co-locating index bucket and 64B entry

Adds an optional table layout where each hash bucket is stored as a 128-byte line holding the 64-byte index bucket followed by the first matching 64-byte entry, so a lookup can fetch index and value with one contiguous access instead of two dependent loads. Lookup, commit, deferred and peer kernels are templated on the inline flag, and entry references carry a high bit marking inline homes. A conversion kernel migrates between layouts, and the workload enables inline mode by default when entry and op sizes match. This adds memory for the line array, conversion cost and extra branching on every entry access.

Result: faster. 4.914 billion (median of 6 runs) (+8.4%).

```diff
diff --git a/hermes_amd/csrc/hkv_batch.hip b/hermes_amd/csrc/hkv_batch.hip
--- a/hermes_amd/csrc/hkv_batch.hip
+++ b/hermes_amd/csrc/hkv_batch.hip
@@ -70,6 +70,7 @@
     int32_t check_unique;
     uint8_t *ack_out;
     uint32_t ack_out_size;
+    uint8_t *line;
 };
 
 __host__ __device__ constexpr int rounds_for(int type, bool rmw)
@@ -167,6 +168,19 @@
 
 __device__ __forceinline__ uint64_t phys_of(const BatchArgs &a, uint32_t e) { return (uint64_t)e * a.g.entry_unit; }
 __device__ __forceinline__ uint8_t *entry_of(const BatchArgs &a, uint32_t e) { return a.log + phys_of(a, e); }
+constexpr uint32_t kEntInline = 0x80000000u;
+__device__ __forceinline__ uint8_t *line_entry(const BatchArgs &a, uint64_t key)
+{
+    return a.line + ((key & 0xFFFFFFFFFFFFULL) & a.g.bkt_mask) * 128u + 64u;
+}
+template <bool IL>
+__device__ __forceinline__ uint32_t ent_id(uint32_t e) { return IL ? e & ~kEntInline : e; }
+template <bool IL>
+__device__ __forceinline__ uint8_t *entry_home(const BatchArgs &a, uint32_t e, uint64_t key)
+{
+    if (IL && (e & kEntInline)) return line_entry(a, key);
+    return entry_of(a, ent_id<IL>(e));
+}
 __device__ __forceinline__ uint32_t fw_index(const BatchArgs &a, uint64_t phys)
 {
     return (uint32_t)(((phys >> 6) * 0x9E3779B1ull) & a.fw_mask);
@@ -337,15 +351,24 @@
 
 constexpr int64_t kLookupHead = 8192;
 constexpr int kLookupPair = 2;
-template <int P = kLookupPair>
-__device__ __forceinline__ void lookup_pair(const BatchArgs &a, const uint64_t *key, const bool *probe, int q,
-                                            int gbase, bool *ok, uint64_t *phys, uint4 *ln)
-{
-    uint4 v[P];
-#pragma unroll
-    for (int k = 0; k < P; ++k)
-        v[k] = probe[k] ? reinterpret_cast<const uint4 *>(a.index + ((key[k] & 0xFFFFFFFFFFFFULL) & a.g.bkt_mask) * 64u)[q]
-                        : make_uint4(0u, 0u, 0u, 0u);
+template <int P = kLookupPair, bool IL = false, bool F = false>
+__device__ __forceinline__ void lookup_core(const BatchArgs &a, const uint64_t *key, const bool *probe, int q,
+                                            int gbase, bool *ok, uint64_t *phys, uint4 *ln, unsigned long long *fwv,
+                                            uint8_t **home, bool *inl)
+{
+    uint4 v[P], ev[P];
+#pragma unroll
+    for (int k = 0; k < P; ++k) {
+        if (IL) {
+            const uint4 *l = reinterpret_cast<const uint4 *>(a.line + ((key[k] & 0xFFFFFFFFFFFFULL) & a.g.bkt_mask) * 128u);
+            v[k] = probe[k] ? l[q] : make_uint4(0u, 0u, 0u, 0u);
+            ev[k] = probe[k] ? l[4 + q] : make_uint4(0u, 0u, 0u, 0u);
+        } else {
+            v[k] = probe[k] ? reinterpret_cast<const uint4 *>(a.index + ((key[k] & 0xFFFFFFFFFFFFULL) & a.g.bkt_mask) * 64u)[q]
+                            : make_uint4(0u, 0u, 0u, 0u);
+        }
+    }
+    bool il[P];
 #pragma unroll
     for (int k = 0; k < P; ++k) {
         const uint64_t s0 = (uint64_t)v[k].x | ((uint64_t)v[k].y << 32);
@@ -359,50 +382,50 @@
 #pragma unroll
         for (int l = 0; l < 4; ++l) o |= ((g0 >> l) & 1u) << (2 * l) | ((g1 >> l) & 1u) << (2 * l + 1);
         const int first = o ? __ffs(o) - 1 : 0;
-        const uint64_t off = __shfl((first & 1) ? (s1 >> 24) : (s0 >> 24), first >> 1, 4);
+        uint64_t off = __shfl((first & 1) ? (s1 >> 24) : (s0 >> 24), first >> 1, 4);
+        il[k] = false;
+        if (IL) {
+            il[k] = (off & kInlineOffBit) != 0;
+            off &= ~kInlineOffBit;
+        }
         ok[k] = probe[k] && o && a.g.log_head - off < a.g.log_cap;
         phys[k] = off & a.g.log_mask;
-    }
-#pragma unroll
-    for (int k = 0; k < P; ++k)
-        ln[k] = ok[k] ? reinterpret_cast<const uint4 *>(a.log + phys[k])[q] : make_uint4(0u, 0u, 0u, 0u);
-}
-
-template <int P>
+        if (IL) il[k] = il[k] && ok[k];
+    }
+#pragma unroll
+    for (int k = 0; k < P; ++k) {
+        if (IL) {
+            ln[k] = ev[k];
+            if (!il[k]) ln[k] = ok[k] ? reinterpret_cast<const uint4 *>(a.log + phys[k])[q] : make_uint4(0u, 0u, 0u, 0u);
+            if (home) home[k] = il[k] ? line_entry(a, key[k]) : a.log + phys[k];
+            if (inl) inl[k] = il[k];
+        } else {
+            ln[k] = ok[k] ? reinterpret_cast<const uint4 *>(a.log + phys[k])[q] : make_uint4(0u, 0u, 0u, 0u);
+            if (home) home[k] = a.log + phys[k];
+            if (inl) inl[k] = false;
+        }
+        if (F) fwv[k] = ok[k] && q == 0 ? a.fw[fw_index(a, phys[k])] : ~0ull;
+    }
+}
+
+template <int P = kLookupPair, bool IL = false>
+__device__ __forceinline__ void lookup_pair(const BatchArgs &a, const uint64_t *key, const bool *probe, int q,
+                                            int gbase, bool *ok, uint64_t *phys, uint4 *ln, uint8_t **home = nullptr,
+                                            bool *inl = nullptr)
+{
+    lookup_core<P, IL, false>(a, key, probe, q, gbase, ok, phys, ln, nullptr, home, inl);
+}
+
+template <int P, bool IL = false>
 __device__ __forceinline__ void lookup_pair_f(const BatchArgs &a, const uint64_t *key, const bool *probe, int q,
-                                              int gbase, bool *ok, uint64_t *phys, uint4 *ln, unsigned long long *fwv)
-{
-    uint4 v[P];
-#pragma unroll
-    for (int k = 0; k < P; ++k)
-        v[k] = probe[k] ? reinterpret_cast<const uint4 *>(a.index + ((key[k] & 0xFFFFFFFFFFFFULL) & a.g.bkt_mask) * 64u)[q]
-                        : make_uint4(0u, 0u, 0u, 0u);
-#pragma unroll
-    for (int k = 0; k < P; ++k) {
-        const uint64_t s0 = (uint64_t)v[k].x | ((uint64_t)v[k].y << 32);
-        const uint64_t s1 = (uint64_t)v[k].z | ((uint64_t)v[k].w << 32);
-        const uint32_t tag = (uint32_t)(key[k] >> 48);
-        const bool mt0 = probe[k] && (s0 & 1u) && ((uint32_t)(s0 >> 1) & 0x7FFFFFu) == tag;
-        const bool mt1 = probe[k] && (s1 & 1u) && ((uint32_t)(s1 >> 1) & 0x7FFFFFu) == tag;
-        const uint32_t g0 = (uint32_t)(__ballot(mt0) >> gbase) & 0xFu;
-        const uint32_t g1 = (uint32_t)(__ballot(mt1) >> gbase) & 0xFu;
-        uint32_t o = 0;
-#pragma unroll
-        for (int l = 0; l < 4; ++l) o |= ((g0 >> l) & 1u) << (2 * l) | ((g1 >> l) & 1u) << (2 * l + 1);
-        const int first = o ? __ffs(o) - 1 : 0;
-        const uint64_t off = __shfl((first & 1) ? (s1 >> 24) : (s0 >> 24), first >> 1, 4);
-        ok[k] = probe[k] && o && a.g.log_head - off < a.g.log_cap;
-        phys[k] = off & a.g.log_mask;
-    }
-#pragma unroll
-    for (int k = 0; k < P; ++k) {
-        ln[k] = ok[k] ? reinterpret_cast<const uint4 *>(a.log + phys[k])[q] : make_uint4(0u, 0u, 0u, 0u);
-        fwv[k] = ok[k] && q == 0 ? a.fw[fw_index(a, phys[k])] : ~0ull;
-    }
-}
-
-
-template <int P = kLookupPair>
+                                              int gbase, bool *ok, uint64_t *phys, uint4 *ln, unsigned long long *fwv,
+                                              uint8_t **home = nullptr, bool *inl = nullptr)
+{
+    lookup_core<P, IL, true>(a, key, probe, q, gbase, ok, phys, ln, fwv, home, inl);
+}
+
+
+template <int P = kLookupPair, bool IL = false>
 __global__ __launch_bounds__(256) void k_lookup(BatchArgs a, int64_t i_begin, int64_t i_end)
 {
     const int q = threadIdx.x & 3;
@@ -469,12 +492,13 @@
     uint64_t phys[P], ekey[P];
     Meta m0[P];
     U64x2 ln[P];
+    uint8_t *home[P];
     {
         bool pr[P];
         uint4 l4[P];
 #pragma unroll
         for (int k = 0; k < P; ++k) pr[k] = probe[k] != 0;
-        lookup_pair<P>(a, key, pr, q, gbase, ok, phys, l4);
+        lookup_pair<P, IL>(a, key, pr, q, gbase, ok, phys, l4, home);
 #pragma unroll
         for (int k = 0; k < P; ++k)
             ln[k] = U64x2{(uint64_t)l4[k].x | ((uint64_t)l4[k].y << 32), (uint64_t)l4[k].z | ((uint64_t)l4[k].w << 32)};
@@ -499,7 +523,7 @@
         uint8_t ifl = 0;
         if (ok[k] && ekey[k] == key[k]) {
             e = (uint32_t)(phys[k] / a.g.entry_unit);
-            uint8_t *entry = a.log + phys[k];
+            uint8_t *entry = IL ? home[k] : a.log + phys[k];
             if (vals_direct) {
                 const uint64_t its = pack_ts((uint32_t)(hdr[k] >> 32), (uint8_t)(hdr[k] >> 24));
                 if (its == pack_ts(m0[k].ver, m_cid(m0[k])) && m_state(m0[k]) != kValid) entry[kEntryMetaOff] = kValid;
@@ -1367,7 +1391,7 @@
 #else
 #define HKV_PRE_SGPR_ATTR
 #endif
-template <int HEAD = kPreHead>
+template <int HEAD = kPreHead, bool IL = false>
 __global__ __launch_bounds__(kPreThreads) HKV_PRE_ATTR HKV_PRE_SGPR_ATTR void k_local_pre(BatchArgs a)
 {
     __shared__ uint64_t hk[kPreHash], gk[kPreHash];
@@ -1488,7 +1512,7 @@
                 }
             }
         }
-        lookup_pair<kPrePair>(a, key, probe, q, gbase, ok, phys, ln);
+        lookup_pair<kPrePair, IL>(a, key, probe, q, gbase, ok, phys, ln);
 #pragma unroll
         for (int k = 0; k < kPrePair; ++k) {
             Meta m0;
@@ -1549,7 +1573,7 @@
 #define HKV_LF_WAVES 2
 #endif
 constexpr int kLfWaves = HKV_LF_WAVES;
-template <int P, int NW>
+template <int P, int NW, bool IL = false>
 __global__ __launch_bounds__(64 * NW) HKV_LOCAL_SGPR_ATTR void k_local_fused(BatchArgs a)
 {
     constexpr int E = 16 * P;
@@ -1604,12 +1628,13 @@
             probe[k] = in_count(a, (uint32_t)(i0 + te[k])) && !skip_elem_os(kLocal, (uint8_t)h0, (uint8_t)(h0 >> 8));
     }
     unsigned long long fwv[P];
+    bool inl[P];
     if (HKV_DBG_ON(a, 512)) {
-        lookup_pair<P>(a, key, probe, q, gbase, ok, phys, ln);
+        lookup_pair<P, IL>(a, key, probe, q, gbase, ok, phys, ln, nullptr, inl);
 #pragma unroll
         for (int k = 0; k < P; ++k) fwv[k] = ~0ull;
     } else {
-        lookup_pair_f<P>(a, key, probe, q, gbase, ok, phys, ln, fwv);
+        lookup_pair_f<P, IL>(a, key, probe, q, gbase, ok, phys, ln, fwv, nullptr, inl);
     }
 #pragma unroll
     for (int k = 0; k < P; ++k) {
@@ -1620,7 +1645,7 @@
         if (hit) sln[te[k] * 4 + q] = ln[k];
         if (q == 0) {
             sfw[te[k]] = f;
-            sent[te[k]] = hit ? (uint32_t)(phys[k] / a.g.entry_unit) : kNone;
+            sent[te[k]] = hit ? (uint32_t)(phys[k] / a.g.entry_unit) | (IL && inl[k] ? kEntInline : 0u) : kNone;
             sprb[te[k]] = probe[k];
         }
     }
@@ -1638,9 +1663,10 @@
             const bool wm = would_mutate(kLocal, x, m, c);
             if (m_state(m) == kInvalid) {
                 if (wm) {
-                    const uint64_t ph = phys_of(a, e);
+                    const uint64_t ph = phys_of(a, ent_id<IL>(e));
                     offer(a.fw + fw_index(a, ph), a.rtag0, (uint32_t)i);
-                    if ((uint8_t)(m.w5 >> 16) != a.ltag) a.log[ph + kEntryMetaOff + 4] = a.ltag;
+                    if ((uint8_t)(m.w5 >> 16) != a.ltag)
+                        entry_home<IL>(a, e, *reinterpret_cast<const uint64_t *>(x))[kEntryMetaOff + 4] = a.ltag;
                 }
                 st = kStDefer;
                 sdef[atomicAdd(&ndef, 1u)] = (uint32_t)i;
@@ -1777,7 +1803,7 @@
     return a.x == b.x && a.y == b.y && a.z == b.z && a.w == b.w;
 }
 
-template <int TYPE, int P = kLookupPair>
+template <int TYPE, int P = kLookupPair, bool IL = false>
 __global__ __launch_bounds__(64) void k_unique_lds(BatchArgs a)
 {
     constexpr int E = 16 * P;
@@ -1817,7 +1843,8 @@
             }
         }
     }
-    lookup_pair<P>(a, key, probe, q, gbase, ok, phys, ln);
+    uint8_t *home[P];
+    lookup_pair<P, IL>(a, key, probe, q, gbase, ok, phys, ln, home);
 #pragma unroll
     for (int k = 0; k < P; ++k) {
         Meta m;
@@ -1891,7 +1918,7 @@
         }
         if (ok[k] && q > 0) {
             const uint4 l = sln[te[k] * 4 + q];
-            if (!chunk_equal(l, ln[k])) reinterpret_cast<uint4 *>(a.log + phys[k])[q] = l;
+            if (!chunk_equal(l, ln[k])) reinterpret_cast<uint4 *>(IL ? home[k] : a.log + phys[k])[q] = l;
         }
     }
 }
@@ -1901,7 +1928,7 @@
 #else
 #define HKV_ROWS_SGPR_ATTR
 #endif
-template <int TYPE, int RMAX, int CH, int P = kLookupPair>
+template <int TYPE, int RMAX, int CH, int P = kLookupPair, bool IL = false>
 #ifdef HKV_ROWS_WAVES
 #define HKV_ROWS_WAVES_ATTR __attribute__((amdgpu_waves_per_eu(HKV_ROWS_WAVES, 8)))
 #else
@@ -1958,7 +1985,8 @@
         part[k] = mismatch ? 0u : p;
         probe[k] = part[k] != 0;
     }
-    lookup_pair<P>(a, key, probe, q, gbase, ok, phys, ln);
+    uint8_t *home[P];
+    lookup_pair<P, IL>(a, key, probe, q, gbase, ok, phys, ln, home);
 #pragma unroll
     for (int k = 0; k < P; ++k) {
         Meta m;
@@ -2028,7 +2056,7 @@
         }
         if (ok[k] && q > 0) {
             const uint4 l = sln[te[k] * 4 + q];
-            if (!chunk_equal(l, ln[k])) reinterpret_cast<uint4 *>(a.log + phys[k])[q] = l;
+            if (!chunk_equal(l, ln[k])) reinterpret_cast<uint4 *>(IL ? home[k] : a.log + phys[k])[q] = l;
         }
     }
 }
@@ -2158,6 +2186,7 @@
     }
 }
 
+template <bool IL = false>
 __global__ __launch_bounds__(256) void k_local_deferred(BatchArgs a)
 {
     const uint32_t nd = a.ctr[kCtrDefer];
@@ -2168,21 +2197,22 @@
         uint8_t idx;
         Ctx c = make_ctx(a);
         elem_at(a, i, xg, idx, c);
+        uint8_t *entry = IL ? entry_home<IL>(a, e, *reinterpret_cast<const uint64_t *>(xg)) : entry_of(a, e);
         Meta m;
-        meta_load(entry_of(a, e), m);
-        const uint32_t f = first_cand(*fw_of(a, e), a.rtag0);
+        meta_load(entry, m);
+        const uint32_t f = first_cand(*fw_of(a, ent_id<IL>(e)), a.rtag0);
         uint8_t st = kStDone;
         if (f == kNone || i < f) {
             Meta tm = m;
-            dispatch<31>(kLocal, xg, entry_of(a, e), idx, tm, c);
+            dispatch<31>(kLocal, xg, entry, idx, tm, c);
             if (a.error_flags && !meta_equal(tm, m)) atomicOr(a.error_flags, 1u);
         } else if (i == f) {
-            apply_to_shadow<kLocal, 31>(a, nullptr, i, entry_of(a, e));
+            apply_to_shadow<kLocal, 31>(a, nullptr, i, entry);
             st = kStCommit;
         } else {
             const Meta m1 = after_first<kLocal>(a, m, f, 0);
             Meta tm = m1;
-            dispatch<31>(kLocal, xg, entry_of(a, e), idx, tm, c);
+            dispatch<31>(kLocal, xg, entry, idx, tm, c);
             if (a.error_flags && !meta_equal(tm, m1)) atomicOr(a.error_flags, 1u);
         }
         a.st[i] = st;
@@ -2268,6 +2298,7 @@
 }
 
 constexpr int kCwElems = 1024;
+template <bool IL = false>
 __global__ __launch_bounds__(256) void k_commit_w(BatchArgs a)
 {
     __shared__ uint32_t lst[4][kCwElems];
@@ -2298,7 +2329,12 @@
     for (uint32_t j = (uint32_t)(lane >> 2); j < total; j += 16) {
         const uint32_t i = lst[w][j];
         const uint4 v = reinterpret_cast<const uint4 *>(shadow_of(a, i))[q];
-        reinterpret_cast<uint4 *>(entry_of(a, a.ent[i]))[q] = v;
+        if (IL) {
+            const uint64_t key = (uint64_t)(uint32_t)__shfl((int)v.z, 0, 4) | ((uint64_t)(uint32_t)__shfl((int)v.w, 0, 4) << 32);
+            reinterpret_cast<uint4 *>(entry_home<IL>(a, a.ent[i], key))[q] = v;
+        } else {
+            reinterpret_cast<uint4 *>(entry_of(a, a.ent[i]))[q] = v;
+        }
     }
 }
 
@@ -3279,6 +3315,47 @@
     if (i >= 0) out[b] = elems[(base + i) * esz + kOpValueOff];
 }
 
+template <bool TO_INLINE>
+__global__ __launch_bounds__(256) void k_layout_convert(const uint8_t *index, uint8_t *log, uint8_t *line,
+                                                        uint64_t num_bkts, uint64_t log_mask)
+{
+    const int q = threadIdx.x & 3, gbase = (threadIdx.x & 63) & ~3;
+    const uint64_t b = (uint64_t)blockIdx.x * 64 + (threadIdx.x >> 2);
+    const bool live = b < num_bkts;
+    uint4 v = make_uint4(0u, 0u, 0u, 0u);
+    if (live) v = reinterpret_cast<const uint4 *>(index + b * 64u)[q];
+    const uint64_t s0 = (uint64_t)v.x | ((uint64_t)v.y << 32), s1 = (uint64_t)v.z | ((uint64_t)v.w << 32);
+    const uint32_t g0 = (uint32_t)(__ballot(live && (s0 & 1u)) >> gbase) & 0xFu;
+    const uint32_t g1 = (uint32_t)(__ballot(live && (s1 & 1u)) >> gbase) & 0xFu;
+    uint32_t o = 0;
+#pragma unroll
+    for (int l = 0; l < 4; ++l) o |= ((g0 >> l) & 1u) << (2 * l) | ((g1 >> l) & 1u) << (2 * l + 1);
+    const int first = o ? __ffs(o) - 1 : 0;
+    const uint64_t off = __shfl((first & 1) ? (s1 >> 24) : (s0 >> 24), first >> 1, 4);
+    if (!live) return;
+    uint4 *ln = reinterpret_cast<uint4 *>(line + b * 128u);
+    uint4 *ent = reinterpret_cast<uint4 *>(log + (off & log_mask));
+    if (TO_INLINE) {
+        if (o && (first >> 1) == q) {
+            if (first & 1) v.w |= (uint32_t)(kInlineSlotBit >> 32);
+            else v.y |= (uint32_t)(kInlineSlotBit >> 32);
+        }
+        ln[q] = v;
+        ln[4 + q] = o ? ent[q] : make_uint4(0u, 0u, 0u, 0u);
+    } else if (o) {
+        ent[q] = ln[4 + q];
+    }
+}
+
+int launch_layout_convert(const uint8_t *index, uint8_t *log, uint8_t *line, uint64_t num_bkts, uint64_t log_mask,
+                          bool to_inline, hipStream_t s)
+{
+    const unsigned grid = (unsigned)((num_bkts + 63) / 64);
+    if (to_inline) hipLaunchKernelGGL(k_layout_convert<true>, dim3(grid), dim3(256), 0, s, index, log, line, num_bkts, log_mask);
+    else hipLaunchKernelGGL(k_layout_convert<false>, dim3(grid), dim3(256), 0, s, index, log, line, num_bkts, log_mask);
+    return hipGetLastError() == hipSuccess ? 0 : -3;
+}
+
 static inline size_t align256(size_t x) { return (x + 255) & ~(size_t)255; }
 
 size_t batch_scratch_bytes(int64_t cap, uint32_t entry_size)
@@ -3312,10 +3389,40 @@
 
 uint32_t batch_max_epoch() { return (1u << 29) - 1; }
 
+struct BatchPath {
+    bool small, local_direct, rows, unique_lds64, vals;
+};
+static BatchPath batch_path(const BatchLaunch &bl)
+{
+    BatchPath p{};
+    const int64_t n = bl.n;
+    p.small = (bl.path == kPathSmall || (bl.path == kPathAuto && n <= kSmallMaxElems)) && n <= kSmallMaxElems;
+    p.local_direct = bl.type == kLocal && !bl.g.rmw_enabled && bl.esz == 56 && bl.g.st_value == 31 &&
+                     bl.g.entry_size == 64 && !bl.offsets;
+    const bool uniq = bl.unique && (bl.type == kInvs || bl.type == kAcks);
+    p.rows = bl.n_rows > 0 && bl.unique;
+    p.unique_lds64 = uniq && bl.g.st_value == 31 && bl.g.entry_size == 64 && bl.esz <= 64;
+    p.vals = bl.type == kVals;
+    return p;
+}
+
+bool batch_inline_capable(const BatchLaunch &bl)
+{
+    if (bl.n <= 0 || bl.g.entry_size != 64 || bl.g.st_value != 31) return false;
+    const BatchPath p = batch_path(bl);
+    if (p.small) return false;
+    if (p.local_direct) return true;
+    if (bl.type == kLocal || bl.type == kLocalAfterMemb) return false;
+    if (p.rows) return bl.n_rows <= 8;
+    if (bl.unique && (bl.type == kInvs || bl.type == kAcks)) return p.unique_lds64;
+    return p.vals;
+}
+
 int launch_batch(BatchLaunch &bl, hipStream_t s)
 {
     const int64_t n = bl.n;
     if (n <= 0) return 0;
+    if (bl.line && !batch_inline_capable(bl)) return -1;
     BatchArgs a;
     a.elems = bl.elems;
     a.counts = bl.counts;
@@ -3342,6 +3449,7 @@
     a.check_unique = check_unique_env;
     a.index = bl.index;
     a.log = bl.log;
+    a.line = bl.line;
     a.rw = bl.rw;
     a.ns_idx = bl.ns_idx;
     a.fw = bl.fw;
@@ -3385,10 +3493,11 @@
     const bool big_direct = bl.type != kInvs;
     const unsigned rgrid = (unsigned)(big ? (n + 127) / 128 : grid);
     const size_t rlds = (size_t)(big ? 128 : 256) * (size_t)bl.esz;
-    const bool small = (bl.path == kPathSmall || (bl.path == kPathAuto && n <= kSmallMax)) && n <= kSmallMax;
+    const BatchPath bp = batch_path(bl);
+    const bool small = bp.small;
     if (bl.region_bytes && !small) return -1;
-    const bool local_direct = bl.type == kLocal && !bl.g.rmw_enabled && bl.esz == 56 && bl.g.st_value == 31 &&
-                              bl.g.entry_size == 64 && !bl.offsets;
+    const bool local_direct = bp.local_direct;
+    const bool il = bl.line != nullptr;
     const uint32_t vend = (uint32_t)kOpValueOff + bl.g.st_value;
     const bool patch_in_resolve = bl.patch && !small && !local_direct && bl.type == kLocal && big && big_direct &&
                                   !bl.offsets && bl.g.st_value != 31 && bl.g.st_value <= 320 && bl.esz % 8 == 0 &&
@@ -3405,24 +3514,32 @@
         if (launch_small(a, s)) return -3;
         return 0;
     } else if (local_direct) {
-        hipLaunchKernelGGL(k_local_pre<kPreHead>, dim3((unsigned)((n + kPreElems - 1) / kPreElems)), dim3(kPreThreads),
-                           0, s, a);
-        hipLaunchKernelGGL((k_local_fused<2, kLfWaves>), dim3((unsigned)((n + 32 * kLfWaves - 1) / (32 * kLfWaves))),
-                           dim3(64 * kLfWaves), 0, s, a);
-        hipLaunchKernelGGL(k_local_deferred, dim3(128u), dim3(256), 0, s, a);
-        hipLaunchKernelGGL(k_commit_w, dim3((unsigned)((n + 4 * kCwElems - 1) / (4 * kCwElems))), dim3(256), 0, s, a);
+        const dim3 pgrid((unsigned)((n + kPreElems - 1) / kPreElems));
+        const dim3 fgrid((unsigned)((n + 32 * kLfWaves - 1) / (32 * kLfWaves)));
+        if (il) {
+            hipLaunchKernelGGL((k_local_pre<kPreHead, true>), pgrid, dim3(kPreThreads), 0, s, a);
+            hipLaunchKernelGGL((k_local_fused<2, kLfWaves, true>), fgrid, dim3(64 * kLfWaves), 0, s, a);
+            hipLaunchKernelGGL(k_local_deferred<true>, dim3(128u), dim3(256), 0, s, a);
+            hipLaunchKernelGGL(k_commit_w<true>, dim3((unsigned)((n + 4 * kCwElems - 1) / (4 * kCwElems))), dim3(256), 0, s, a);
+            return hipGetLastError() == hipSuccess ? 0 : -3;
+        }
+        hipLaunchKernelGGL(k_local_pre<kPreHead>, pgrid, dim3(kPreThreads), 0, s, a);
+        hipLaunchKernelGGL((k_local_fused<2, kLfWaves>), fgrid, dim3(64 * kLfWaves), 0, s, a);
+        hipLaunchKernelGGL(k_local_deferred<false>, dim3(128u), dim3(256), 0, s, a);
+        hipLaunchKernelGGL(k_commit_w<false>, dim3((unsigned)((n + 4 * kCwElems - 1) / (4 * kCwElems))), dim3(256), 0, s, a);
     } else if (bl.n_rows > 0 && bl.unique) {
         const unsigned lgrid = (unsigned)((n + kLfElems - 1) / kLfElems);
-        if (bl.type == kInvs) {
-            if (bl.n_rows <= 2) hipLaunchKernelGGL((k_unique_rows<kInvs, 2, 4>), dim3(lgrid), dim3(64), 0, s, a);
-            else hipLaunchKernelGGL((k_unique_rows<kInvs, 8, 4>), dim3(lgrid), dim3(64), 0, s, a);
-        } else if (bl.esz <= 16) {
-            if (bl.n_rows <= 2) hipLaunchKernelGGL((k_unique_rows<kAcks, 2, 1>), dim3(lgrid), dim3(64), 0, s, a);
-            else hipLaunchKernelGGL((k_unique_rows<kAcks, 8, 1>), dim3(lgrid), dim3(64), 0, s, a);
-        } else {
-            if (bl.n_rows <= 2) hipLaunchKernelGGL((k_unique_rows<kAcks, 2, 4>), dim3(lgrid), dim3(64), 0, s, a);
-            else hipLaunchKernelGGL((k_unique_rows<kAcks, 8, 4>), dim3(lgrid), dim3(64), 0, s, a);
-        }
+#define HKV_ROWS(T, CH)                                                                                           \
+    do {                                                                                                         \
+        if (il && bl.n_rows <= 2) hipLaunchKernelGGL((k_unique_rows<T, 2, CH, kLookupPair, true>), dim3(lgrid), dim3(64), 0, s, a); \
+        else if (il) hipLaunchKernelGGL((k_unique_rows<T, 8, CH, kLookupPair, true>), dim3(lgrid), dim3(64), 0, s, a); \
+        else if (bl.n_rows <= 2) hipLaunchKernelGGL((k_unique_rows<T, 2, CH>), dim3(lgrid), dim3(64), 0, s, a);  \
+        else hipLaunchKernelGGL((k_unique_rows<T, 8, CH>), dim3(lgrid), dim3(64), 0, s, a);                      \
+    } while (0)
+        if (bl.type == kInvs) HKV_ROWS(kInvs, 4);
+        else if (bl.esz <= 16) HKV_ROWS(kAcks, 1);
+        else HKV_ROWS(kAcks, 4);
+#undef HKV_ROWS
     } else if (bl.unique && (bl.type == kInvs || bl.type == kAcks)) {
         const unsigned ugrid1 = (unsigned)((n + 63) / 64);
 #define HKV_UNIQUE(T)                                                                                  \
@@ -3436,7 +3553,9 @@
         if (a.ack_out && !(lds64 || lds_big)) return -1;
         if (lds64) {
             const unsigned g1 = (unsigned)((n + 15) / 16);
-            if (bl.type == kInvs) hipLaunchKernelGGL((k_unique_lds<kInvs, 1>), dim3(g1), dim3(64), 0, s, a);
+            if (il && bl.type == kInvs) hipLaunchKernelGGL((k_unique_lds<kInvs, 1, true>), dim3(g1), dim3(64), 0, s, a);
+            else if (il) hipLaunchKernelGGL((k_unique_lds<kAcks, 1, true>), dim3(g1), dim3(64), 0, s, a);
+            else if (bl.type == kInvs) hipLaunchKernelGGL((k_unique_lds<kInvs, 1>), dim3(g1), dim3(64), 0, s, a);
             else hipLaunchKernelGGL((k_unique_lds<kAcks, 1>), dim3(g1), dim3(64), 0, s, a);
         } else if (lds_big) {
             hipLaunchKernelGGL(k_unique_big<kInvs>, dim3((unsigned)((n + kUbElems - 1) / kUbElems)), dim3(64), 0, s, a);
@@ -3444,7 +3563,8 @@
         else HKV_UNIQUE(kAcks);
 #undef HKV_UNIQUE
     } else if (bl.type == kVals) {
-        hipLaunchKernelGGL(k_lookup<1>, dim3((unsigned)((n + 63) / 64)), dim3(256), 0, s, a, (int64_t)0, n);
+        if (il) hipLaunchKernelGGL((k_lookup<1, true>), dim3((unsigned)((n + 63) / 64)), dim3(256), 0, s, a, (int64_t)0, n);
+        else hipLaunchKernelGGL(k_lookup<1>, dim3((unsigned)((n + 63) / 64)), dim3(256), 0, s, a, (int64_t)0, n);
         return hipGetLastError() == hipSuccess ? 0 : -3;
     } else {
     const bool split = bl.type == kLocal || bl.type == kLocalAfterMemb;
diff --git a/hermes_amd/csrc/hkv_internal.h b/hermes_amd/csrc/hkv_internal.h
--- a/hermes_amd/csrc/hkv_internal.h
+++ b/hermes_amd/csrc/hkv_internal.h
@@ -20,6 +20,7 @@
     uint8_t *rw_state;
     const uint8_t *index;
     uint8_t *log;
+    uint8_t *line;
     uint8_t *rw;
     int64_t rw_stride;
     int32_t *ns_idx;
@@ -142,11 +143,21 @@
     Geometry g;
     const uint8_t *index;
     const uint8_t *log;
+    const uint8_t *line;
 };
-int table_view(const hkv_table *t, TableView *out);
+enum : int32_t { kViewLog = 0, kViewLive = 1, kViewStatic = 2 };
+int table_view(hkv_table *t, TableView *out, hipStream_t stream, int32_t mode);
 
+constexpr uint64_t kInlineSlotBit = 1ull << 63;
+constexpr uint64_t kInlineOffBit = 1ull << 39;
+constexpr uint64_t kInlineMaxLog = 1ull << 36;
+constexpr uint64_t kPhysInline = 1ull << 62;
+int launch_layout_convert(const uint8_t *index, uint8_t *log, uint8_t *line, uint64_t num_bkts, uint64_t log_mask,
+                          bool to_inline, hipStream_t s);
+bool batch_inline_capable(const BatchLaunch &bl);
+
+constexpr int64_t kSmallMaxElems = 4096;
 int launch_batch(BatchLaunch &bl, hipStream_t s);
-constexpr int64_t kSmallMaxElems = 4096;
 int launch_populate(const PopulateLaunch &pl, hipStream_t s);
 int launch_hash_ids(const uint32_t *ids, uint64_t *out, int64_t n, hipStream_t s);
 size_t sort_temp_bytes(int64_t n, int key_bits);
diff --git a/hermes_amd/csrc/hkv_runtime.hip b/hermes_amd/csrc/hkv_runtime.hip
--- a/hermes_amd/csrc/hkv_runtime.hip
+++ b/hermes_amd/csrc/hkv_runtime.hip
@@ -94,6 +94,10 @@
     hipStream_t stream = nullptr;
     uint8_t *d_index = nullptr;
     uint8_t *d_log = nullptr;
+    uint8_t *d_line = nullptr;
+    int layout_pref = HKV_LAYOUT_LOG, layout_state = HKV_LAYOUT_LOG;
+    uint64_t conversions = 0, inline_launches = 0;
+    hipStream_t last_stream = nullptr;
     unsigned long long *d_evictions = nullptr;
     int64_t inserted = 0;
     uint32_t skip_key = 0;
@@ -259,13 +263,59 @@
     final_head = (n < k) ? h0 + n * e : hw + (n - k) * e;
 }
 
+static bool layout_eligible(const hkv_table *t)
+{
+    return t->geo.entry_size == 64 && !t->cfg.big_objects && t->geo.log_head <= t->geo.log_cap &&
+           t->geo.log_cap <= kInlineMaxLog;
+}
+
+static int layout_set(hkv_table *t, int want, hipStream_t s)
+{
+    if (t->layout_state == want) {
+        t->last_stream = s;
+        return 0;
+    }
+    if (t->last_stream != s) HIP_TRY(hipStreamSynchronize(t->last_stream));
+    if (launch_layout_convert(t->d_index, t->d_log, t->d_line, t->cfg.num_bkts, t->geo.log_mask,
+                              want == HKV_LAYOUT_INLINE, s))
+        return fail(-3, "layout conversion launch failed: %s", hipGetErrorString(hipGetLastError()));
+    TRACE("layout -> %s", want == HKV_LAYOUT_INLINE ? "INLINE" : "LOG");
+    t->layout_state = want;
+    t->last_stream = s;
+    ++t->conversions;
+    return 0;
+}
+
+static int layout_for_launch(hkv_table *t, bool capable, hipStream_t s, uint8_t **line)
+{
+    const bool inl = capable && t->layout_pref == HKV_LAYOUT_INLINE && t->d_line && layout_eligible(t);
+    if (int rc = layout_set(t, inl ? HKV_LAYOUT_INLINE : HKV_LAYOUT_LOG, s)) return rc;
+    if (inl) ++t->inline_launches;
+    *line = inl ? t->d_line : nullptr;
+    return 0;
+}
+
+static int layout_export(hkv_table *t)
+{
+    if (t->layout_state == HKV_LAYOUT_LOG) return 0;
+    hipStream_t s = t->last_stream;
+    HIP_TRY(hipStreamSynchronize(t->stream));
+    HIP_TRY(hipStreamSynchronize(s));
+    if (int rc = layout_set(t, HKV_LAYOUT_LOG, s)) return rc;
+    HIP_TRY(hipStreamSynchronize(s));
+    return 0;
+}
+
 namespace hkv {
-int table_view(const hkv_table *t, TableView *out)
+int table_view(hkv_table *t, TableView *out, hipStream_t stream, int32_t mode)
 {
     if (!t || !out) return -1;
+    uint8_t *line = nullptr;
+    if (mode != kViewStatic && layout_for_launch(t, mode == kViewLive, stream, &line)) return -1;
     out->g = t->geo;
     out->index = t->d_index;
     out->log = t->d_log;
+    out->line = line;
     return 0;
 }
 }
@@ -337,6 +387,7 @@
     if (t->stream) hipStreamSynchronize(t->stream);
     hipFree(t->d_index);
     hipFree(t->d_log);
+    hipFree(t->d_line);
     hipFree(t->d_evictions);
     hipFree(t->d_batch);
     hipFree(t->d_fw);
@@ -394,6 +445,7 @@
     if (n > 0x7FFFFFFFll) return fail(-1, "populate: at most 2^31-1 keys (32-bit key ids)");
     std::lock_guard<std::mutex> lk(t->mu);
     HIP_TRY(hipSetDevice(t->cfg.device));
+    if (int rc = layout_export(t)) return rc;
     int bbits = bit_width(t->cfg.num_bkts - 1);
     if (bbits == 0) bbits = 1;
     uint64_t *d_first = nullptr, *d_second = nullptr;
@@ -560,7 +612,8 @@
         bl.row_stride = d->row_stride;
         bl.path = kPathEngine;
     }
-    TRACE("batch_async type=%d n=%lld", d->type, (long long)n);
+    if (int lrc = layout_for_launch(t, batch_inline_capable(bl), s, &bl.line)) return lrc;
+    TRACE("batch_async type=%d n=%lld%s", d->type, (long long)n, bl.line ? " (inline)" : "");
     rc = launch_batch(bl, s);
     if (rc) return fail(rc, "batch launch failed (%d): %s", rc, hipGetErrorString(hipGetLastError()));
     return 0;
@@ -596,6 +649,7 @@
     if (!t || !dst) return fail(-1, "null argument");
     if (off + bytes > t->cfg.num_bkts * 64) return fail(-1, "index range out of bounds");
     srv_stop(t);
+    if (int rc = layout_export(t)) return rc;
     HIP_TRY(hipStreamSynchronize(t->stream));
     HIP_TRY(hipMemcpy(dst, t->d_index + off, bytes, hipMemcpyDeviceToHost));
     return 0;
@@ -606,6 +660,7 @@
     if (!t || !dst) return fail(-1, "null argument");
     if (off + bytes > t->cfg.log_cap + t->geo.entry_size) return fail(-1, "log range out of bounds");
     srv_stop(t);
+    if (int rc = layout_export(t)) return rc;
     HIP_TRY(hipStreamSynchronize(t->stream));
     HIP_TRY(hipMemcpy(dst, t->d_log + off, bytes, hipMemcpyDeviceToHost));
     return 0;
@@ -621,7 +676,11 @@
     return (int64_t)v;
 }
 
-void *hkv_device_index(hkv_table *t) { return t ? t->d_index : nullptr; }
+void *hkv_device_index(hkv_table *t)
+{
+    if (!t || layout_export(t)) return nullptr;
+    return t->d_index;
+}
 
 int hkv_take_error_flags(hkv_table *t, uint32_t *out)
 {
@@ -633,7 +692,73 @@
     HIP_TRY(hipDeviceSynchronize());
     return 0;
 }
-void *hkv_device_log(hkv_table *t) { return t ? t->d_log : nullptr; }
+void *hkv_device_log(hkv_table *t)
+{
+    if (!t || layout_export(t)) return nullptr;
+    return t->d_log;
+}
+
+static bool layout_room(const hkv_table *t)
+{
+    const size_t bytes = (size_t)t->cfg.num_bkts * 128;
+    size_t free_b = 0, total_b = 0;
+    if (hipSetDevice(t->cfg.device) != hipSuccess || hipMemGetInfo(&free_b, &total_b) != hipSuccess) return false;
+    return free_b >= bytes + bytes / 4 + ((size_t)1 << 30);
+}
+
+int hkv_table_prefer_layout(hkv_table *t, int layout)
+{
+    if (!t) return fail(-1, "null table");
+    if (layout != HKV_LAYOUT_LOG && layout != HKV_LAYOUT_INLINE) return fail(-1, "unknown layout %d", layout);
+    std::lock_guard<std::mutex> lk(t->mu);
+    t->layout_pref = layout;
+    if (layout == HKV_LAYOUT_LOG || !layout_eligible(t)) return 0;
+    if (!t->d_line) {
+        const size_t bytes = (size_t)t->cfg.num_bkts * 128;
+        if (!layout_room(t)) return 0;
+        if (hipMalloc(&t->d_line, bytes) != hipSuccess) {
+            (void)hipGetLastError();
+            t->d_line = nullptr;
+            return 0;
+        }
+    }
+    return 1;
+}
+
+int hkv_table_layout(hkv_table *t, hkv_layout_info *out)
+{
+    if (!t || !out) return fail(-1, "null argument");
+    memset(out, 0, sizeof *out);
+    out->state = t->layout_state;
+    out->preferred = t->layout_pref;
+    out->eligible = layout_eligible(t) && (t->d_line || layout_room(t));
+    out->conversions = t->conversions;
+    out->inline_launches = t->inline_launches;
+    out->line_bytes = t->d_line ? (uint64_t)t->cfg.num_bkts * 128 : 0;
+    return 0;
+}
+
+int hkv_table_apply_layout(hkv_table *t, void *stream)
+{
+    if (!t) return fail(-1, "null table");
+    srv_stop(t);
+    uint8_t *line;
+    if (int rc = layout_for_launch(t, true, (hipStream_t)stream, &line)) return rc;
+    if (line) --t->inline_launches;
+    return 0;
+}
+
+int hkv_copy_lines(hkv_table *t, void *dst, uint64_t off, uint64_t bytes)
+{
+    if (!t || !dst) return fail(-1, "null argument");
+    if (!t->d_line) return fail(-1, "the inline residency is not allocated");
+    if (off + bytes > t->cfg.num_bkts * 128) return fail(-1, "line range out of bounds");
+    srv_stop(t);
+    HIP_TRY(hipStreamSynchronize(t->stream));
+    HIP_TRY(hipStreamSynchronize(t->last_stream));
+    HIP_TRY(hipMemcpy(dst, t->d_line + off, bytes, hipMemcpyDeviceToHost));
+    return 0;
+}
 
 int hkv_hash_ids(const uint32_t *d_ids, uint64_t *d_keys_second, int64_t n, void *stream)
 {
@@ -797,6 +922,7 @@
     }
     BatchLaunch bl;
     memset(&bl, 0, sizeof bl);
+    if (layout_export(t)) die("hermes_batch_ops_to_KVS (layout)");
     bl.g = t->geo;
     bl.index = t->d_index;
     bl.log = t->d_log;
@@ -888,6 +1014,7 @@
         std::lock_guard<std::mutex> tl(t->mu);
         sl.c.g = t->geo;
     }
+    if (layout_export(t)) die("hermes_batch_ops_to_KVS (layout)");
     sl.c.index = t->d_index;
     sl.c.log = t->d_log;
     sl.c.error_flags = t->d_error_flags;
@@ -1010,6 +1137,7 @@
         h.w_ack_init = (uint8_t)(r->mb >> 16);
         for (int g = 0; g <= kPartG; ++g) pl.part[g][b] = r->poff[g];
     }
+    if (layout_export(t)) die("hermes_batch_ops_to_KVS (layout)");
     pl.c.index = t->d_index;
     pl.c.log = t->d_log;
     pl.c.error_flags = t->d_error_flags;
diff --git a/hermes_amd/csrc/hkv_workload.hip b/hermes_amd/csrc/hkv_workload.hip
--- a/hermes_amd/csrc/hkv_workload.hip
+++ b/hermes_amd/csrc/hkv_workload.hip
@@ -1231,20 +1231,31 @@
     }
 }
 
+template <bool FLAG = false>
 __device__ __forceinline__ uint64_t find_entry(const TableView &t, uint64_t key)
 {
     const uint64_t *b = reinterpret_cast<const uint64_t *>(t.index + ((key & 0xFFFFFFFFFFFFULL) & t.g.bkt_mask) * 64u);
     const uint32_t tag = (uint32_t)(key >> 48);
+    bool lowest = true;
     for (int s = 0; s < 8; ++s) {
         const uint64_t slot = b[s];
         if ((slot & 1u) && ((uint32_t)(slot >> 1) & 0x7FFFFFu) == tag) {
             const uint64_t off = slot >> 24;
             if (t.g.log_head - off >= t.g.log_cap) return ~0ull;
             const uint64_t phys = off & t.g.log_mask;
-            return *reinterpret_cast<const uint64_t *>(t.log + phys + 8) == key ? phys : ~0ull;
-        }
+            if (*reinterpret_cast<const uint64_t *>(t.log + phys + 8) != key) return ~0ull;
+            return phys | (FLAG && lowest && t.g.log_cap <= kInlineMaxLog ? kPhysInline : 0ull);
+        }
+        if (slot & 1u) lowest = false;
     }
     return ~0ull;
+}
+
+template <bool IL>
+__device__ __forceinline__ const uint8_t *located_entry(const TableView &t, uint64_t loc, uint64_t key)
+{
+    if (IL && (loc & kPhysInline)) return t.line + ((key & 0xFFFFFFFFFFFFULL) & t.g.bkt_mask) * 128u + 64u;
+    return t.log + (loc & ~kPhysInline);
 }
 
 __device__ __forceinline__ uint64_t peer_slot(const TableView &t, uint64_t phys) { return phys / t.g.entry_size; }
@@ -1537,7 +1548,7 @@
 {
     const int64_t g = (int64_t)blockIdx.x * 256 + threadIdx.x;
     if (g >= total) return;
-    phys_out[g] = find_entry(t, *reinterpret_cast<const uint64_t *>(invs + g * op_size));
+    phys_out[g] = find_entry<true>(t, *reinterpret_cast<const uint64_t *>(invs + g * op_size));
 }
 
 struct PeerTsArgs {
@@ -1549,6 +1560,7 @@
     unsigned long long *peer_ts;
     uint32_t round;
 };
+template <bool IL>
 __device__ __forceinline__ void peer_ts_at_body(const PeerTsArgs &pt, int bx)
 {
     const TableView &t = pt.t;
@@ -1570,7 +1582,7 @@
     uint32_t cur = 0;
     bool ok = false;
     if (phys != ~0ull) {
-        const U64x2w *e = reinterpret_cast<const U64x2w *>(t.log + phys);
+        const U64x2w *e = reinterpret_cast<const U64x2w *>(located_entry<IL>(t, phys, key));
         const U64x2w l0 = e[0], l1 = e[1];
         if (l0.b == key) {
             ok = true;
@@ -1578,12 +1590,13 @@
         }
     }
     if (!ok) {
-        phys = find_entry(t, key);
+        phys = find_entry<true>(t, key);
         if (phys != ~0ull) {
             ok = true;
-            cur = *reinterpret_cast<const uint32_t *>(t.log + phys + 24);
-        }
-    }
+            cur = *reinterpret_cast<const uint32_t *>(located_entry<IL>(t, phys, key) + 24);
+        }
+    }
+    phys &= ~kPhysInline;
     uint32_t ver = 2;
     if (ok) {
         ver = cur + ((!t.g.rmw_enabled || rmw) ? 2u : 4u);
@@ -1597,12 +1610,14 @@
     *reinterpret_cast<uint64_t *>(vv + 8) = (vh & 0xFFFFFF00ull & 0xFFFFFFFFull) | kOpVal | ((uint64_t)ver << 32);
 }
 
-__global__ __launch_bounds__(256) void k_peer_ts_at(PeerTsArgs pt) { peer_ts_at_body(pt, blockIdx.x); }
-
+template <bool IL>
+__global__ __launch_bounds__(256) void k_peer_ts_at(PeerTsArgs pt) { peer_ts_at_body<IL>(pt, blockIdx.x); }
+
+template <bool IL>
 __global__ __launch_bounds__(256) HKV_PLAN_SGPR_ATTR void k_plan_peer_ts(PlanArgs pa, PeerTsArgs pt, int plan_blocks)
 {
     if ((int)blockIdx.x < plan_blocks) refill_plan_body<2>(pa, blockIdx.x);
-    else peer_ts_at_body(pt, (int)blockIdx.x - plan_blocks);
+    else peer_ts_at_body<IL>(pt, (int)blockIdx.x - plan_blocks);
 }
 
 }
@@ -1727,7 +1742,7 @@
     if (n_peers <= 0 || n_workers <= 0 || ack_size < kOpMetaSize || ack_size % 8 || !inv_off) return -1;
     if (max_invs <= 0 || max_invs > inv_stride) return -1;
     TableView tv{};
-    if (peer_ts && table_view(t, &tv)) return -1;
+    if (peer_ts && table_view(t, &tv, (hipStream_t)stream, kViewStatic)) return -1;
     const int32_t out_stride = max_invs * n_peers;
     int64_t total = (int64_t)n_workers * out_stride;
     hipLaunchKernelGGL(k_peer_acks, dim3(blocks_for(total)), dim3(256), 0, (hipStream_t)stream, inv_out, inv_count,
@@ -1744,7 +1759,7 @@
     if (n_peers <= 0 || n_workers <= 0 || ack_size < kOpMetaSize || ack_size % 8) return -1;
     if (out_stride % n_peers || out_stride > inv_stride * n_peers || out_stride <= 0) return -1;
     TableView tv{};
-    if (peer_ts && table_view(t, &tv)) return -1;
+    if (peer_ts && table_view(t, &tv, (hipStream_t)stream, kViewStatic)) return -1;
     int64_t total = (int64_t)n_workers * out_stride;
     hipLaunchKernelGGL(k_peer_acks, dim3(blocks_for(total)), dim3(256), 0, (hipStream_t)stream, inv_out, inv_count,
                        inv_stride, op_size, acks, ack_size, out_stride, ack_count, peer_ids, n_peers, total, tv,
@@ -1799,7 +1814,7 @@
                    int32_t stride, uint32_t op_size, unsigned long long *peer_ts, uint32_t round, void *stream)
 {
     TableView tv;
-    if (table_view(t, &tv) || n_workers <= 0 || stride <= 0 || op_size % 8) return -1;
+    if (table_view(t, &tv, (hipStream_t)stream, kViewLog) || n_workers <= 0 || stride <= 0 || op_size % 8) return -1;
     const int64_t total = (int64_t)n_workers * stride;
     const int64_t per_block = 64 * kPeerTsPair;
     hipLaunchKernelGGL(k_peer_ts, dim3((unsigned)((total + per_block - 1) / per_block)), dim3(256), 0,
@@ -1810,7 +1825,7 @@
 uint64_t hkv_wl_peer_ts_words(const hkv_table *t)
 {
     TableView tv;
-    if (table_view(t, &tv)) return 0;
+    if (table_view(const_cast<hkv_table *>(t), &tv, nullptr, kViewStatic)) return 0;
     return (tv.g.log_cap / tv.g.entry_size + 1) * 8;
 }
 
@@ -1991,7 +2006,7 @@
 {
     if (n_peers <= 0 || n_workers <= 0 || ack_size < kOpMetaSize || ack_size % 8 || q_stride <= 0) return -1;
     TableView tv{};
-    if (peer_ts && table_view(t, &tv)) return -1;
+    if (peer_ts && table_view(t, &tv, (hipStream_t)stream, kViewStatic)) return -1;
     hipLaunchKernelGGL(k_peer_acks_q, dim3(n_workers), dim3(256), 0, (hipStream_t)stream, inv_out, inv_count, inv_stride,
                        op_size, aq, ack_size, q_stride, aq_n, vq_n, acnt, peer_ids, n_peers, tv, peer_ts, round);
     return ok();
@@ -2015,7 +2030,7 @@
 int hkv_wl_peer_locate(hkv_table *t, const uint8_t *invs, int64_t n, uint32_t op_size, uint64_t *phys_out, void *stream)
 {
     TableView tv;
-    if (table_view(t, &tv) || n < 0 || op_size % 8) return -1;
+    if (table_view(t, &tv, (hipStream_t)stream, kViewStatic) || n < 0 || op_size % 8) return -1;
     if (n == 0) return 0;
     hipLaunchKernelGGL(k_peer_locate, dim3(blocks_for(n)), dim3(256), 0, (hipStream_t)stream, tv, invs, op_size, n,
                        phys_out);
@@ -2026,10 +2041,12 @@
                       unsigned long long *peer_ts, uint32_t round, void *stream)
 {
     TableView tv;
-    if (table_view(t, &tv) || n < 0 || op_size % 8) return -1;
+    if (n < 0 || op_size % 8) return -1;
     if (n == 0) return 0;
+    if (table_view(t, &tv, (hipStream_t)stream, kViewLive)) return -1;
     const PeerTsArgs pt{tv, invs, vals, phys, n, op_size, peer_ts, round};
-    hipLaunchKernelGGL(k_peer_ts_at, dim3(blocks_for(n)), dim3(256), 0, (hipStream_t)stream, pt);
+    if (tv.line) hipLaunchKernelGGL(k_peer_ts_at<true>, dim3(blocks_for(n)), dim3(256), 0, (hipStream_t)stream, pt);
+    else hipLaunchKernelGGL(k_peer_ts_at<false>, dim3(blocks_for(n)), dim3(256), 0, (hipStream_t)stream, pt);
     return ok();
 }
 
@@ -2043,17 +2060,23 @@
     if (flags & ~(uint32_t)(HKV_WL_REFILL_ALL | HKV_WL_READ_TS_RESET)) return -1;
     if (((uintptr_t)patch & 15) || (st_value >> shift) > 255) return -1;
     TableView tv;
-    if (table_view(t, &tv) || n < 0 || op_size % 8) return -1;
+    if (n < 0 || op_size % 8) return -1;
+    if (table_view(t, &tv, (hipStream_t)stream, n ? kViewLive : kViewStatic)) return -1;
     const PlanArgs pa{states, n_workers, stride, st_value, shift, tkey, top, tlen, cursor, machine_id, flags, counters, opc,
                       patch};
     const PeerTsArgs pt{tv, invs, vals, phys, n, op_size, peer_ts, round};
     const int plan_blocks = (n_workers + 7) / 8;
 #ifdef HKV_PLAN_PTS_SPLIT
     hipLaunchKernelGGL(k_refill_plan_w<2>, dim3((unsigned)plan_blocks), dim3(256), 0, (hipStream_t)stream, pa);
-    if (n) hipLaunchKernelGGL(k_peer_ts_at, dim3(blocks_for(n)), dim3(256), 0, (hipStream_t)stream, pt);
+    if (n && tv.line) hipLaunchKernelGGL(k_peer_ts_at<true>, dim3(blocks_for(n)), dim3(256), 0, (hipStream_t)stream, pt);
+    else if (n) hipLaunchKernelGGL(k_peer_ts_at<false>, dim3(blocks_for(n)), dim3(256), 0, (hipStream_t)stream, pt);
 #else
-    hipLaunchKernelGGL(k_plan_peer_ts, dim3((unsigned)plan_blocks + blocks_for(n)), dim3(256), 0, (hipStream_t)stream, pa,
-                       pt, plan_blocks);
+    if (tv.line)
+        hipLaunchKernelGGL(k_plan_peer_ts<true>, dim3((unsigned)plan_blocks + blocks_for(n)), dim3(256), 0,
+                           (hipStream_t)stream, pa, pt, plan_blocks);
+    else
+        hipLaunchKernelGGL(k_plan_peer_ts<false>, dim3((unsigned)plan_blocks + blocks_for(n)), dim3(256), 0,
+                           (hipStream_t)stream, pa, pt, plan_blocks);
 #endif
     return ok();
 }
diff --git a/hermes_amd/kvs.py b/hermes_amd/kvs.py
--- a/hermes_amd/kvs.py
+++ b/hermes_amd/kvs.py
@@ -6,7 +6,7 @@
 import torch
 
 from . import layout as L
-from .lib import ABI_VERSION, HkvBatchDesc, HkvConfig, Membership, check, raw
+from .lib import ABI_VERSION, HkvBatchDesc, HkvConfig, HkvLayoutInfo, Membership, check, raw
 
 _L = raw()
 
@@ -59,6 +59,9 @@
     cap = 1 << max(16, (need - 1).bit_length())
     return min(bkts, 1 << (27 if num_keys <= 1 << 28 else 29)), cap
 
+
+LAYOUT_LOG = 0
+LAYOUT_INLINE = 1
 
 BATCH_ENGINE = 1
 BATCH_SMALL = 2
@@ -288,6 +291,28 @@
             return None
         return self.log_bytes(off, self.sizes.entry).view(L.entry_dtype(self.sizes))[0]
 
+    def prefer_layout(self, layout: int) -> bool:
+        rc = _L.hkv_table_prefer_layout(self.h, int(layout))
+        if rc < 0:
+            check(rc, "hkv_table_prefer_layout")
+        return rc == 1
+
+    def layout(self) -> dict:
+        v = HkvLayoutInfo()
+        check(_L.hkv_table_layout(self.h, ctypes.byref(v)), "hkv_table_layout")
+        return {"state": v.state, "preferred": v.preferred, "eligible": bool(v.eligible), "conversions": v.conversions,
+                "inline_launches": v.inline_launches, "line_bytes": v.line_bytes}
+
+    def apply_layout(self, stream: torch.cuda.Stream | None = None) -> None:
+        s = (stream or torch.cuda.current_stream(self.device)).cuda_stream
+        check(_L.hkv_table_apply_layout(self.h, ctypes.c_void_p(s)), "hkv_table_apply_layout")
+
+    def line_bytes(self, offset: int = 0, nbytes: int | None = None) -> np.ndarray:
+        nbytes = self.cfg.num_bkts * 128 - offset if nbytes is None else nbytes
+        out = np.empty(nbytes, dtype=np.uint8)
+        check(_L.hkv_copy_lines(self.h, out.ctypes.data_as(ctypes.c_void_p), offset, nbytes), "hkv_copy_lines")
+        return out
+
     def device_index(self) -> int:
         return _L.hkv_device_index(self.h)
 
diff --git a/hermes_amd/lib.py b/hermes_amd/lib.py
--- a/hermes_amd/lib.py
+++ b/hermes_amd/lib.py
@@ -7,7 +7,7 @@
 
 HERE = os.path.dirname(os.path.abspath(__file__))
 LIB_PATH = os.environ.get("HKV_LIB") or os.path.join(HERE, "libhermeskv.so")
-ABI_VERSION = 8
+ABI_VERSION = 9
 
 if not os.path.exists(LIB_PATH):
     raise ImportError(f"{LIB_PATH} is missing: run __graft_entry__.build() (hipcc --offload-arch=gfx950)")
@@ -36,6 +36,12 @@
                 ("d_phys", ctypes.c_void_p)]
 
 
+class HkvLayoutInfo(ctypes.Structure):
+    _fields_ = [("state", ctypes.c_int32), ("preferred", ctypes.c_int32), ("eligible", ctypes.c_int32),
+                ("reserved", ctypes.c_int32), ("conversions", ctypes.c_uint64), ("inline_launches", ctypes.c_uint64),
+                ("line_bytes", ctypes.c_uint64)]
+
+
 class Membership(ctypes.Structure):
     _fields_ = [("bits", ctypes.c_uint64)]
 
@@ -62,6 +68,10 @@
 _L.hkv_take_error_flags.argtypes = [_P, ctypes.POINTER(ctypes.c_uint32)]
 _L.hkv_device_log.restype = _P
 _L.hkv_device_log.argtypes = [_P]
+_L.hkv_table_prefer_layout.argtypes = [_P, ctypes.c_int]
+_L.hkv_table_layout.argtypes = [_P, ctypes.POINTER(HkvLayoutInfo)]
+_L.hkv_table_apply_layout.argtypes = [_P, _P]
+_L.hkv_copy_lines.argtypes = [_P, _P, ctypes.c_uint64, ctypes.c_uint64]
 _L.hkv_set_default_config.argtypes = [ctypes.POINTER(HkvConfig)]
 _L.hkv_default_table.restype = _P
 _L.hkv_hash_ids.argtypes = [_P, _P, ctypes.c_int64, _P]
diff --git a/hermes_amd/workload.py b/hermes_amd/workload.py
--- a/hermes_amd/workload.py
+++ b/hermes_amd/workload.py
@@ -2,12 +2,13 @@
 
 import ctypes
 import math
+import os
 
 import numpy as np
 import torch
 
 from . import layout as L
-from .kvs import HermesKV
+from .kvs import LAYOUT_INLINE, HermesKV
 from .lib import check, raw
 
 _L = raw()
@@ -290,6 +291,9 @@
         self.remote_packed = []
         self.fused_acks = (self.pack_remote and ((kvs.sizes.entry == 64 and self.op <= 64) or
                                                  (kvs.sizes.entry == 320 and self.op <= 320)))
+        all_capable = (not kvs.rmw and kvs.sizes.entry == 64 and self.op == 56 and val_credits is None and
+                       (self.R == 0 or (self.pack_remote and self.fit and self.ack_rows)))
+        self.inline = all_capable and os.environ.get("HKV_INLINE", "1") != "0" and kvs.prefer_layout(LAYOUT_INLINE)
         self.drops = []
         self.alive = self.R
         self._counts = {}
diff --git a/include/hermeskv.h b/include/hermeskv.h
--- a/include/hermeskv.h
+++ b/include/hermeskv.h
@@ -8,7 +8,7 @@
 extern "C" {
 #endif
 
-#define HKV_ABI_VERSION 8
+#define HKV_ABI_VERSION 9
 
 #ifndef HERMES_SPACETIME_H
 enum hermes_batch_type_t {
@@ -116,6 +116,22 @@
 int  hkv_take_error_flags(hkv_table *t, uint32_t *out);
 void *hkv_device_log(hkv_table *t);
 
+#define HKV_LAYOUT_LOG 0
+#define HKV_LAYOUT_INLINE 1
+typedef struct hkv_layout_info {
+    int32_t state;
+    int32_t preferred;
+    int32_t eligible;
+    int32_t reserved;
+    uint64_t conversions;
+    uint64_t inline_launches;
+    uint64_t line_bytes;
+} hkv_layout_info;
+int  hkv_table_prefer_layout(hkv_table *t, int layout);
+int  hkv_table_layout(hkv_table *t, hkv_layout_info *out);
+int  hkv_table_apply_layout(hkv_table *t, void *stream);
+int  hkv_copy_lines(hkv_table *t, void *host_dst, uint64_t offset, uint64_t bytes);
+
 int  hkv_set_default_config(const hkv_config *cfg);
 hkv_table *hkv_default_table(void);
 
```
